# worm-privacy/proof-of-burn

Measured on AMD Instinct MI355X. Metric: proof_of_burn witnesses/sec, higher is better.
Workload: dtype u64 bit-sliced lanes + BN254 Fr (8x32-bit Montgomery)

## Files before the change

### include/pob_hip.h

```cpp
#ifndef POB_HIP_H
#define POB_HIP_H
#include <stdint.h>
#ifdef __cplusplus
extern "C" {
#endif

typedef struct pob_ctx* pob_handle;

enum { POB_CIRCUIT_PROOF_OF_BURN = 0, POB_CIRCUIT_SPEND = 1, POB_CIRCUIT_GADGET = 2 };
enum { POB_OK = 0, POB_E_ARG = -1, POB_E_HIP = -2, POB_E_NOMEM = -3, POB_E_STATE = -4, POB_E_IO = -5, POB_E_RANGE = -6 };

typedef struct {
    uint64_t n_witness;
    uint64_t n_bit, n_sm, n_fr;
    uint32_t n_fr_inputs, n_sm_inputs, n_outputs;
    uint32_t n_units, n_sponges, n_perms, n_stages, max_batch;
    uint64_t group_bytes;
    uint64_t keccak_bit_wires;
    uint64_t n_derived;
    uint64_t n_alias;
    uint32_t kchk_rounds;
    uint32_t kgc_rounds;
} pob_info_t;

int pob_open(int device, int circuit, const uint64_t* params, int nparams, uint32_t max_batch, pob_handle* out);
void pob_close(pob_handle h);
int pob_get_info(pob_handle h, pob_info_t* info);
int pob_plan_info(int circuit, const uint64_t* params, int nparams, pob_info_t* info);
const char* pob_strerror(pob_handle h);
int pob_gadget_template(const char* name, int* nparams);

int pob_upload_inputs(pob_handle h, const uint8_t* fr_inputs, const int32_t* sm_inputs, uint32_t n);
int pob_upload_inputs_async(pob_handle h, const uint8_t* fr_inputs, const int32_t* sm_inputs, uint32_t n, void* stream);
int pob_pack_json(int circuit, const uint64_t* params, int nparams, const char* json, uint64_t len, uint8_t* fr_row, int32_t* sm_row,
                  uint32_t* forced, char* err, uint32_t errcap);
int pob_pack_json_batch(int circuit, const uint64_t* params, int nparams, const char* const* json, const uint64_t* len, uint32_t n, int threads,
                        uint8_t* fr, int32_t* sm, uint32_t* forced, char* err, uint32_t errcap);
#define POB_EXC_CAP 32
#define POB_EXC_NONE 0xFFFFFFFFu
typedef struct { uint32_t k; int32_t v; } pob_sm_exc_t;
int pob_upload_inputs8(pob_handle h, const uint8_t* fr_inputs, const uint8_t* sm8, const pob_sm_exc_t* exc, uint32_t n);
int pob_upload_inputs8_async(pob_handle h, const uint8_t* fr_inputs, const uint8_t* sm8, const pob_sm_exc_t* exc, uint32_t n, void* stream);
int pob_narrow_inputs(const int32_t* sm, uint32_t n, uint32_t n_sm_inputs, uint8_t* sm8, pob_sm_exc_t* exc);
int pob_pack_json_batch8(int circuit, const uint64_t* params, int nparams, const char* const* json, const uint64_t* len, uint32_t n, int threads,
                         uint8_t* fr, uint8_t* sm8, pob_sm_exc_t* exc, uint32_t* forced, char* err, uint32_t errcap);
int pob_host_alloc(void** p, uint64_t bytes);
void pob_host_free(void* p);

int pob_generate(pob_handle h, void* stream);
int pob_constraint_check(pob_handle h, void* stream);
int pob_sync(pob_handle h);
int pob_set_partner(pob_handle h, pob_handle partner);

int pob_set_inorder(pob_handle h, int on);
int pob_set_audit(pob_handle h, uint32_t groups, uint32_t period);
int pob_audit_last(pob_handle h, uint32_t* first_group, uint32_t* n_groups, uint64_t* audited_batches, uint64_t* audited_groups);

int pob_results(pob_handle h, uint32_t* status, uint8_t* outputs, uint32_t* check_status, uint32_t* bad_wire);
int pob_results_device(pob_handle h, void** d_status, void** d_outputs);
#define POB_RECORD_BYTES 44
#define POB_NOT_EVALUATED 0xFFFFFFFEu
int pob_results_records_device(pob_handle h, void** d_records);
int pob_gather_records(pob_handle h, void* comm, void* stream, void* d_out, uint32_t n_per_rank);
int pob_results_fetch(pob_handle h);
int pob_results_wait(pob_handle h, const uint8_t** records, uint32_t* n);

int pob_emit_witness(pob_handle h, uint32_t idx, uint8_t* dst, uint64_t cap);
int pob_write_wtns(pob_handle h, uint32_t idx, const char* path);
int pob_write_wtns_reduced(pob_handle h, uint32_t idx, const uint32_t* keep, uint64_t n_keep, const char* path);
int pob_emit_begin(pob_handle h, uint32_t idx, uint64_t window_wires);
int pob_emit_begin_reduced(pob_handle h, uint32_t idx, const uint32_t* keep, uint64_t n_keep, uint64_t window_wires);
int pob_reduced_map_pin(pob_handle h, const uint32_t* keep, uint64_t n_keep);
int pob_emit_next(pob_handle h, const uint8_t** data, uint64_t* first_wire, uint64_t* n_wires);
int pob_emit_queue(pob_handle h, uint32_t next_idx);
int pob_emit_selfcheck(pob_handle h, int enable);
int pob_emit_selfcheck_alias(pob_handle h, const int32_t* alias, uint64_t n_wires);
int pob_emit_selfcheck_result(pob_handle h, uint64_t* checked, uint64_t* skipped, uint32_t* first_bad_wire);
int pob_emit_measure(pob_handle h, uint32_t first_idx, uint32_t count, uint64_t window_wires, double* seconds, uint64_t* bytes);
int pob_emit_measure_ex(pob_handle h, uint32_t first_idx, uint32_t count, uint64_t window_wires, const uint32_t* keep, uint64_t n_keep, double* seconds, uint64_t* bytes);

int pob_emit_begin_packed(pob_handle h, uint32_t idx, const uint32_t* keep, uint64_t n_keep, uint64_t window_wires);
int pob_emit_next_packed(pob_handle h, const uint8_t** data, uint64_t* bytes, uint64_t* first_wire, uint64_t* n_wires);
int pob_unpack_window(const uint8_t* packed, uint64_t packed_bytes, uint8_t* dst, uint64_t dst_cap, int threads);
int pob_write_wtns_packed(pob_handle h, uint32_t idx, const uint32_t* keep, uint64_t n_keep, const char* path);
int pob_emit_measure_packed(pob_handle h, uint32_t first_idx, uint32_t count, uint64_t window_wires, const uint32_t* keep, uint64_t n_keep, uint8_t* dst, uint64_t dst_cap, int threads,
                            double* seconds_pinned, double* seconds_expanded, uint64_t* d2h_bytes);

int pob_emit_begin_group_packed(pob_handle h, uint32_t group, uint64_t lanes, const uint32_t* keep, uint64_t n_keep, uint64_t window_wires, uint64_t* lanes_out);
int pob_emit_next_group_packed(pob_handle h, const uint8_t* data[64], uint64_t bytes[64], uint64_t* first_wire, uint64_t* n_wires);
int pob_write_wtns_group(pob_handle h, uint32_t group, uint64_t lanes, const uint32_t* keep, uint64_t n_keep, const char* const paths[64]);
int pob_emit_measure_group(pob_handle h, uint32_t first_group, uint32_t count, uint64_t lanes, uint64_t window_wires, const uint32_t* keep, uint64_t n_keep, uint8_t* dst, uint64_t dst_cap, int threads,
                           double* seconds_pinned, double* seconds_expanded, uint64_t* d2h_bytes);
int pob_emit_group_selfcheck(pob_handle h, int enable);
int pob_emit_group_selfcheck_result(pob_handle h, uint64_t* lanes, uint64_t* checked, uint64_t* skipped, uint32_t first_bad_wire[64]);

int pob_time_kernel(pob_handle h, int which, int iters, void* stream, float* avg_ms);
int pob_probe_check_kernel(pob_handle h, int enable, float* ms);

int pob_debug_xor_bits(pob_handle h, uint32_t group, uint64_t bit_index, uint64_t mask);
int pob_debug_store_fault(pob_handle h, int cls, uint32_t group, uint64_t index, uint64_t mask, uint32_t* wire);
int pob_debug_value_fault(pob_handle h, int cls, uint32_t group, uint64_t index, uint64_t mask, uint32_t* wire);
int pob_debug_stream_create(int device, const uint32_t* cu_mask, uint32_t words, void** stream);
void pob_debug_stream_destroy(int device, void* stream);
enum { POB_CLASS_BIT = 0, POB_CLASS_SM = 1, POB_CLASS_FR = 2 };
int pob_debug_poke(pob_handle h, int cls, uint32_t group, uint64_t index, uint32_t sub, uint32_t lane, uint32_t xor_mask);
// ... 18 lines not shown
```

### proof_of_burn_amd/csrc/circuits.hpp

```cpp
#pragma once
#include <string.h>
#include "gadgets.hpp"
#include "poseidon_consts.h"

#define KECCAKF_ROUND_WIRES 102656u
#define KECCAKF_WIRES (43200u + 24u * KECCAKF_ROUND_WIRES)
#define ABSORB_OWN 5888u
#define ABSORB_WIRES (ABSORB_OWN + 17u * 384u + KECCAKF_WIRES)
#define KR_STORED 76u
#define KR_BITS (KR_STORED * 64u)
#define AB_ROUNDS_W (ABSORB_OWN + 17u * 384u + 43200u)
#define AB_MID 0u
#define AB_DIRECT (25u * 1600u)
#define ABSORB_BITS (AB_DIRECT + 24u * KR_BITS)
#define ABSORB_ALIAS (ABSORB_WIRES - ABSORB_BITS)

enum UnitKind : uint32_t {
    U_POB_INPUT = 1, U_POB_RANGE, U_POB_LAYER_ASSERT, U_POB_HDR_ASSERT, U_POB_POSEIDONS, U_BAH_PRE, U_BAH_POST,
    U_KB_HEAD, U_KB_RANGE, U_KB_SELROW, U_KB_POST, U_POB_N2B, U_PC_PRE, U_PC_POST, U_POB_LASTLAYER, U_POB_LASTLAYER_RANGE,
    U_POB_LASTLEN, U_POB_LEAF, U_POB_LAYER_POST, U_SC_M, U_SC_RANGE, U_SC_SUMS, U_POB_LASTLEAF,
    U_RL_A, U_RL_SLROW, U_RL_ACC, U_RL_B, U_POW_PRE, U_POW_POST, U_POB_FINAL, U_ABS_RANGE, U_LD_HEAD, U_LD_SELR, U_LD_TAIL, U_POB_INPUT_FR, U_RL_ACC_B, U_RL_ACC_C,
    U_SP_INPUT, U_SP_HEAD,
    U_SC_MI,
    CK_POS_SEG,
// ... 14 lines not shown
#define FAM_LIGHT (FAM_BIT(F_MISC) | FAM_BIT(F_RANGE) | FAM_BIT(F_SELROW) | FAM_BIT(F_LD) | FAM_BIT(F_RL))
#define FAM_HEAVY (FAM_BIT(F_POS) | FAM_BIT(F_N2B))
#define FAM_ALL ((1u << F_COUNT) - 1)
HD constexpr uint32_t fam_of(uint32_t k) {
    return (k == U_KB_RANGE || k == U_ABS_RANGE) ? F_RANGE
         : k == U_KB_SELROW ? F_SELROW
         : (k == U_LD_HEAD || k == U_LD_SELR || k == U_LD_TAIL || k == U_LD_COPY || k == U_POB_LASTLAYER_RANGE || k == U_SC_SUMS) ? F_LD
         : (k == U_RL_A || k == U_RL_SLROW || k == U_RL_ACC_B || k == U_RL_ACC_C || k == U_RL_B || k == CK_SR_COLS || k == CK_SL_ROWS || k == CK_RL_B2 || k == CK_RL_B3 || k == CK_CAT) ? F_RL
         : (k == U_POB_LAYER_POST || k == U_SC_M || k == U_SC_RANGE) ? F_SC
         : (k == U_POB_POSEIDONS || k == U_BAH_PRE || k == U_SP_HEAD || k == CK_POS_SEG || k == U_POS_WIDE) ? F_POS
         : (k == U_GM || k == U_GM_INPUT) ? F_GM
         : (k == U_POB_INPUT_FR || k == U_POB_RANGE || k == U_POB_N2B || k == U_PC_POST || k == U_RL_ACC || k == U_POW_PRE || k == U_SP_INPUT || k == CK_N2BE) ? F_N2B
         : F_MISC;
}
HD constexpr uint32_t gen_fam_of(uint32_t k) { return k == U_PC_PRE ? (uint32_t)F_N2B : fam_of(k); }
HD constexpr bool ride_keeps_evaluation(uint32_t kind) { return fam_of(kind) == F_RL; }
#define UCASE(K) case K: if constexpr ((((MASK) >> (P::is_gen ? gen_fam_of(K) : fam_of(K))) & 1u) && !(P::ride && ride_keeps_evaluation(K)))

struct PobParams { int L, NB, HB, minNib, amountBytes, powZero; Fr maxIntended, maxActual; };
struct SpendParams { int maxAmountBytes; };

#define FP_ISEQ_S (Cur{6, 2, 0, 0, 4})
#define FP_ISEQ_F (Cur{6, 2, 0, 0, 4})
#define FP_N2B8 (Cur{9, 0, 0, 0, 9})
#define FP_ISEQ_D (Cur{6, 0, 0, 0, 6})

struct PobMain {
    FrRef commitment, burnKey, actualBalance, intendedBalance, revealAmount, burnExtraCommitment;
    SmRef numLeafAddressNibbles, layers, layerLens, numLayers, blockHeader, blockHeaderLen, byteSecurityRelax;
    FrRef proofExtraCommitment, remainingCoin, nullifier;
    SmRef addressHashNibbles, blockRoot, stateRoot, nullifierBytes, remainingCoinBytes, revealAmountBytes, burnExtraCommitmentBytes,
        extraCommitmentBytes, lastLayer, lastLayerLen;
    BitRef layerExists, substringCheckers;
    SmRef layerKeccaks, reducedLayerKeccaks;
    BitRef isLeaf, isLastLayerLeaf;
    SmRef leaf, leafLen;
};
struct SpendMain {
    FrRef commitment, burnKey, balance, withdrawnBalance, extraCommitment, coin, remainingCoin;
    SmRef coinBytes, withdrawnBalanceBytes, remainingCoinBytes, extraCommitmentBytes;
};
struct KBRefs {
    SmRef out, in, inLen, numBlocks; BitRef inBitsArray, inBits, inBlocks, outBits, outBytes;
    uint32_t padded_w, pad_o_w, pad_in_w;
    SmRef pad_nb, pad_il, pad_dv, pad_rm; BitRef pad_flt, pad_isEq, pad_isLast;
    Cur c_loop;
    Cur c_div;
    BitRef k_out, k_in; SmRef k_blocks; BitRef k_finalState, f_out, f_in; SmRef f_blocks; BitRef f_s;
    uint32_t abs_w, abs_b;
    BitRef sel_out, sel_arrays; SmRef sel_select; BitRef sel_T;
    Cur c_post;
    SmRef dst; uint32_t has_dst;
    uint32_t mb, index;
};
struct ScRefs {
    BitRef out; uint32_t mi_w; SmRef ml, si; FrRef num; uint32_t M_w; BitRef ex, isl, alw; SmRef sums; BitRef dne;
    Cur c_abs_sub, c_abs_main, c_after_abs, c_loop, c_tail;
    SmRef abs_main_in;
};
struct RlRefs {
    SmRef o, ol, in, inl; FrRef bal; SmRef key, keyLen, acc, accLen, pk, pkLen, val, valLen;
    SmRef t_o, t_ol, t_in, t_il, t_dv, t_rm, t_shf, t_on, t_tmp;
    SmRef s_o, s_in, s_cn; BitRef s_isEq; SmRef s_temp;
    Cur c_sl_iseq, c_mux, c_age, c_acc, c_concat;
};
struct LdRefs {
    BitRef isLeaf; SmRef layer, ll;
    BitRef leafPrefixIsF8; SmRef totalLength; BitRef isConsistentWithLayerLen; SmRef keyPrefix; BitRef keyPrefixIsValid, keyIsMultiByte;
    SmRef keyExtraLen, keyLen, valueWrapperPrefix; BitRef valueWrapperPrefixIsB8; SmRef valueWrapperLen, valuePrefix; BitRef valuePrefixIsF8;
    SmRef valueLen; BitRef isValueWrapperLenConsistent, isKeyValueLenEqualWithLayerLen;
    Cur c_sel[4], c_eq[4], c_mand, c_end;
    SmRef src, len_src; BitRef dst;
};
struct RaRefs {
    SmRef ea_o, ea_ol; FrRef ea_ib; SmRef pn, pnl, br, brl, nbl, sc;
    SmRef ri_o, ri_ol; FrRef ri_i; SmRef by, len, be; BitRef isb, isz; SmRef frb;
    Cur c_cb, c_sl, c_lt, c_concat, c_end;
};
struct SpongeDesc { uint32_t n, stage, src_b, abs_b, kin_w, fin_w, fs_w, abs_w, src_w; };
struct UnitDesc { uint32_t kind, stage; Cur cur; uint32_t a[8]; uint32_t cost, flags; };

#define SC_RANGE_POS 32
#define MAX_KB 72
#define MAX_SC 64
struct CircuitLayout {
    int circuit;
    struct { uint32_t tid, nfr_in, nsm_in, nout; } gm;
    uint32_t decl_order;
    PobParams pob; SpendParams spend;
    PobMain pm; SpendMain sm;
    Fr prefix[3];
    struct { SmRef nibbles; FrRef in; SmRef addressBytes, block, hash; uint32_t kb; } bah;
    struct { FrRef out; SmRef in, flat, block, hash, reduced; uint32_t kb; int N, nb; SmRef fl_o, fl_i, fit_o, fit_i; Cur c_abs; } pc;
    struct { FrRef in; SmRef mzb, keyBytes, raBytes, becBytes, eip, hin, block, keccak; BitRef sbz; uint32_t kb; } pw;
    struct { SmRef out; uint32_t arr_w, sel_w, T_w; Cur c_sel0; } ll;
    RlRefs rl;
    RaRefs ra;
    uint32_t kb_hdr, kb_layer0, nkb, nsc;
    Cur fp_n2be32, fp_n2beN;
    KBRefs kbs[MAX_KB];
    ScRefs scs[MAX_SC];
    LdRefs lds[MAX_SC + 1];
};

HD PosOff pos_off(int t) {
    PosOff k;
    if (t == 3) { k.C = POS_OFF_C_3; k.S = POS_OFF_S_3; k.M = POS_OFF_M_3; k.Pm = POS_OFF_P_3; k.rp = POS_RP_3; }
    else if (t == 4) { k.C = POS_OFF_C_4; k.S = POS_OFF_S_4; k.M = POS_OFF_M_4; k.Pm = POS_OFF_P_4; k.rp = POS_RP_4; }
    else { k.C = POS_OFF_C_5; k.S = POS_OFF_S_5; k.M = POS_OFF_M_5; k.Pm = POS_OFF_P_5; k.rp = POS_RP_5; }
    return k;
}

HD bool posw_value_fault_covers(int T, uint32_t rel) {
    const uint32_t t = (uint32_t)T, rp = (uint32_t)pos_off(T).rp, full = 8 * t, part = 4 + 2 * t;
    if (rel < 4 * t + 1) return rel >= 2 * t + 1 && rel <= 3 * t;
    rel -= 4 * t + 1;
    if (rel >= 4 * full && rel < 4 * full + rp * part) { const uint32_t q = (rel - 4 * full) % part; return q >= 4 && q < 4 + t; }
    if (rel >= 4 * full) rel -= rp * part;
    if (rel >= 7 * full) return false;
    const uint32_t q = rel % full;
    return (q >= 4 * t && q < 5 * t) || (q >= 6 * t && q < 7 * t);
}

#define NO_RANK 0xFFFFFFFFu
template <class P> HD BitRef dbits(P& p, uint32_t n) { BitRef r = {p.dvs(n), NO_RANK}; return r; }
template <class P> GD void kb_head(P& p, int mb, S inLen, KBRefs& r) {
    const uint32_t m = 136 * mb;
    r.mb = mb;
    r.out = p.sms(32); r.in = p.sms(m); r.inLen = p.sms(1); r.padded_w = p.dvs(m); r.numBlocks = p.sms(1);
    r.inBitsArray = dbits(p, 8 * m); r.inBits = dbits(p, 8 * m); r.inBlocks = p.bits(8 * m); r.outBits = dbits(p, 256); r.outBytes = dbits(p, 256);
    inLen = p.put(r.inLen, inLen);
    gAssertLessThanS(p, 16, inLen, (S)m);
    r.pad_o_w = p.dvs(m); r.pad_nb = p.sms(1); r.pad_in_w = p.dvs(m); r.pad_il = p.sms(1); r.pad_dv = p.sms(1); r.pad_rm = p.sms(1);
    r.pad_flt = p.bits(m + 1); r.pad_isEq = p.bits(m); r.pad_isLast = p.bits(m);
    inLen = p.put(r.pad_il, inLen);
    S q, rem;
    r.c_div = p.cur;
    gDivide(p, 16, inLen, (S)136, q, rem);
    q = p.put(r.pad_dv, q); p.put(r.pad_rm, rem);
    S nb = p.put(r.pad_nb, q + 1);
    gAssertLessEqThanS(p, 16, nb, (S)mb);
    p.put(r.numBlocks, nb);
    p.put(r.pad_flt, ~(B)0);
    r.c_loop = p.cur;
    p.cur = cur_add(cur_add(cur_add(p.cur, FP_ISEQ_D, 2 * m), FP_N2B8, m), Cur{16u * m, 0, 0, 0, 16u * m}, 1);
}
template <class P> HD void iseq_derived(P& p, Cur c, S a, S b) {
    p.derived(c.w + 1, a); p.derived(c.w + 2, b);
    const S x = (S)((uint32_t)b - (uint32_t)a);
    p.derived(c.w + 4, x); p.derived_inv(c.w + 5, x, true);
}
template <class P> GD void kb_range(P& p, const KBRefs& r, SmRef src, uint32_t lo, uint32_t hi, bool assert_src = false, SmRef also = SmRef{0, 0}) {
    const uint32_t m = 136 * r.mb, cnt = hi - lo, ln = p.lane_id();
    const S inLen = p.get(r.inLen), nb = p.get(r.numBlocks);
    const S last = (S)((uint32_t)nb * 136u - 1u);
    const Cur cE = r.c_loop, cL = cur_add(cE, FP_ISEQ_D, m), cN = cur_add(cL, FP_ISEQ_D, m), cF = cur_add(cN, FP_N2B8, m);
    const uint32_t flat_o_w = cF.w, flat_i_w = cF.w + 8 * m;
    bool fl = P::is_gen ? ((uint32_t)inLen >= lo) : p.bit(p.get(r.pad_flt + lo));
    uint32_t wE = 0, wL = 0, wF = 0, wPE = 0, wPL = 0;
    B wb0 = 0, wb1 = 0;
    S vs[16];
    if constexpr (P::is_count) { for (uint32_t t = 0; t < cnt; t++) p.put(r.in + (lo + t), (S)0); for (int q = 0; q < 16; q++) vs[q] = 0; }
    else {
        SmRef rr[16]; S sv[16];
#pragma unroll
        for (int q = 0; q < 16; q++) rr[q] = r.in + (lo + ((uint32_t)q < cnt ? (uint32_t)q : cnt - 1));
        const SmLoaded<16> h = sm_load(p, rr);
#pragma unroll
        for (int q = 0; q < 16; q++) sv[q] = p.get(src + (lo + ((uint32_t)q < cnt ? (uint32_t)q : cnt - 1)));
        sm_commit(p, rr, h, sv);
#pragma unroll
        for (int q = 0; q < 16; q++) vs[q] = P::is_check ? h.s[q] : sv[q];
        if (assert_src) {
#pragma unroll
            for (int q = 0; q < 16; q++) p.require_lane((uint32_t)sv[q] < 256u, FAILCODE(T_NUM2BITS, 38));
        }
        if (also.w) {
            SmRef ar[16];
#pragma unroll
            for (int q = 0; q < 16; q++) ar[q] = also + (lo + ((uint32_t)q < cnt ? (uint32_t)q : cnt - 1));
            const SmLoaded<16> ha = sm_load(p, ar);
            sm_commit(p, ar, ha, sv);
        }
    }
#pragma unroll
    for (uint32_t t = 0; t < 16; t++) if (t < cnt) {
        const uint32_t i = lo + t;
        const Cur ce = cur_add(cE, FP_ISEQ_D, i), cl = cur_add(cL, FP_ISEQ_D, i);
        const S v = vs[t];
        iseq_derived(p, ce, (S)i, inLen); iseq_derived(p, cl, (S)i, last);
        const bool e = (uint32_t)inLen == i, l = (uint32_t)last == i;
        fl = fl && !e;
        const S pv = (fl ? v : 0) + (S)e + (l ? 0x80 : 0);
        p.derived(r.pad_in_w + i, v); p.derived(r.pad_o_w + i, pv); p.derived(r.padded_w + i, pv); p.derived(cN.w + 9 * i + 8, pv);
        p.require_lane((uint32_t)pv < 256u, FAILCODE(T_NUM2BITS, 38));
        wE |= (uint32_t)e << t; wL |= (uint32_t)l << t; wF |= (uint32_t)fl << t;
        wPE |= (e ? 3u : 0u) << (2 * t); wPL |= (l ? 3u : 0u) << (2 * t);
        if (t < 8) wb0 |= (B)((uint32_t)pv & 0xffu) << (8 * t); else wb1 |= (B)((uint32_t)pv & 0xffu) << (8 * (t - 8));
    }
    const B runE = p.xpose64(wE, 0, cnt), runL = p.xpose64(wL, 0, cnt), runF = p.xpose64(wF, 0, cnt);
    const B runPairE = p.xpose64(wPE, 0, 2 * cnt), runPairL = p.xpose64(wPL, 0, 2 * cnt);
    const B bits0 = p.xpose(wb0, 64), bits1 = cnt > 8 ? p.xpose(wb1, 64) : 0;
    p.run_put(cnt, r.pad_isEq.w + lo + ln, r.pad_isEq.i + lo + ln, runE);
    p.run_put(cnt, r.pad_flt.w + lo + 1 + ln, r.pad_flt.i + lo + 1 + ln, runF);
    p.run_put(cnt, r.pad_isLast.w + lo + ln, r.pad_isLast.i + lo + ln, runL);
    {
        const uint32_t i = lo + (ln >> 1), wh = ln & 1;
        p.run_derived(2 * cnt, cE.w + 6 * i + 3 * wh, runPairE);
        p.run_derived(2 * cnt, cL.w + 6 * i + 3 * wh, runPairL);
        if constexpr (P::is_emit) { if (ln < 2 * cnt) { p.site_c(cE.w + 6 * i + 3 * wh, r.pad_isEq.w + i); p.site_c(cL.w + 6 * i + 3 * wh, r.pad_isLast.w + i); } }
    }
    for (uint32_t h2 = 0; h2 < 2 && 8 * h2 < cnt; h2++) {
        const uint32_t n = (cnt - 8 * h2 < 8 ? cnt - 8 * h2 : 8) * 8;
        const B x = h2 ? bits1 : bits0;
        const uint32_t j = 8 * (lo + 8 * h2) + ln, i = lo + 8 * h2 + (ln >> 3);
        p.run_put(n, r.inBlocks.w + j, r.inBlocks.i + j, x);
        p.run_derived(n, cN.w + 9 * i + (ln & 7), x);
        p.run_derived(n, r.inBitsArray.w + j, x);
        p.run_derived(n, flat_i_w + j, x);
        p.run_derived(n, flat_o_w + j, x);
        p.run_derived(n, r.inBits.w + j, x);
    }
}
template <class P> GD void kb_declare_keccak(P& p, KBRefs& r) {
    const uint32_t n = r.mb;
    r.k_out = dbits(p, 256); r.k_in = dbits(p, n * 1088); r.k_blocks = p.sms(1); r.k_finalState = dbits(p, 1600);
    r.f_out = dbits(p, 1600); r.f_in = dbits(p, n * 1088); r.f_blocks = p.sms(1); r.f_s = dbits(p, (n + 1) * 1600);
    r.abs_w = p.cur.w; r.abs_b = p.cur.b;
    p.skip_alias(n * ABSORB_WIRES, n * ABSORB_BITS);
    r.sel_out = dbits(p, 1600); r.sel_arrays = dbits(p, (n + 1) * 1600); r.sel_select = p.sms(1); r.sel_T = dbits(p, 1600 * (n + 1));
}
template <class P, int N1> GD void kb_selrow_n(P& p, const KBRefs& r, uint32_t row, uint32_t j0, uint32_t j1) {
    const uint32_t n1 = N1 ? (uint32_t)N1 : r.mb + 1, n = j1 - j0, ln = p.lane_id();
    const uint32_t fw = 9 * n1 + 3, fb = 1, fq = 9 * n1 + 2;
    const Cur c0 = p.cur;
    const uint32_t idx = row * 64 + j0 + ln;
    const S blocks = p.get(r.numBlocks);
    p.require(p.ballot((uint32_t)blocks < n1), FAILCODE(T_SELECTOR, 43));
    const uint32_t bw = c0.w + ln * fw, bb = c0.b + ln * fb;
    B acc = 0;
    p.run_derived(n, bw + 2 * n1 + 2, 0);
#pragma unroll
    for (uint32_t k = 0; k < n1; k++) {
        const B v = k == 0 ? (B)0 : p.run_get(n, r.abs_b + (k - 1) * ABSORB_BITS + AB_MID + 24u * 1600u + idx);
        const B e = p.ballot((uint32_t)blocks == k);
        acc |= e & v;
        if constexpr (P::is_emit) {
            p.run_derived(n, r.sel_arrays.w + k * 1600 + idx, v);
            p.run_derived(n, r.sel_T.w + idx * n1 + k, v);
            p.run_derived(n, bw + 1 + k, v);
            p.run_derived(n, bw + n1 + 2 + k, e);
            p.run_derived(n, bw + 2 * n1 + 3 + k, acc);
            const uint32_t cw = bw + 3 * n1 + 3 + 6 * k;
            p.run_derived(n, cw, e);
            p.run_derived(n, cw + 3, e);
        }
    }
    p.run_put(n, bw, bb, acc);
    p.run_derived(n, r.sel_out.w + idx, acc);
    p.run_derived(n, r.f_out.w + idx, acc);
    p.run_derived(n, r.k_finalState.w + idx, acc);
    if (row < 4) {
        const uint32_t pw = r.c_post.w;
        p.run_derived(n, r.k_out.w + idx, acc);
        p.run_derived(n, r.outBits.w + idx, acc);
        p.run_derived(n, pw + 256 + idx, acc);
        p.run_derived(n, pw + idx, acc);
        p.run_derived(n, r.outBytes.w + idx, acc);
        p.run_derived(n, pw + 512 + 9 * (idx >> 3) + 1 + (idx & 7), acc);
        for (uint32_t jj = 0; jj < n; jj += 8) {
            S by = 0;
#pragma unroll
            for (uint32_t b = 0; b < 8; b++) by |= (S)p.bit(p.run_bcast(acc, jj + b)) << b;
            const uint32_t i = (row * 64 + j0 + jj) >> 3;
            const SmRef b2n_o = {pw + 512 + 9 * i, r.c_post.s + i};
            const S o = p.put(r.out + i, p.put(b2n_o, by));
            if (r.has_dst) p.put(r.dst + i, o);
        }
    }
    derived_rows_same(p, c0.w + n1 + 1, fw, n, blocks);
    for (uint32_t k = 0; k < n1; k++) {
        const uint32_t cw = c0.w + 3 * n1 + 3 + 6 * k;
        const S x = (S)(k - (uint32_t)blocks);
        derived_rows_same(p, cw + 1, fw, n, blocks);
        derived_rows_same(p, cw + 2, fw, n, (S)k);
        derived_rows_same(p, cw + 4, fw, n, x);
        derived_rows_same(p, cw + 5, fw, n, x, true);
    }
    p.cur = cur_add(c0, Cur{fw, fb, 0, 0, fq}, n);
}
template <class P> GD void kb_selrow(P& p, const KBRefs& r, uint32_t row, uint32_t j0, uint32_t j1) { kb_selrow_n<P, 0>(p, r, row, j0, j1); }
template <class P> GD void kb_post(P& p, const KBRefs& r) {
    S nb = p.get(r.numBlocks);
    p.put(r.k_blocks, nb); p.put(r.f_blocks, nb); p.put(r.sel_select, nb);
    p.cur = cur_add(r.c_post, Cur{512 + 32 * 9, 0, 32, 0, 512 + 32 * 8}, 1);
}

#include "gadget_mains.hpp"

template <class P> GD void rl_b_prefixes(P& p, const RlRefs& R, const PobParams& prm, S kl, S& pl, S& vl) {
    const int ab = 32, bb = prm.amountBytes, maxAcc = 4 + bb + 66, maxKey = 1 + ab;
    const S al = p.get(R.accLen);
    p.put(R.val, 0xb8); p.put(R.val + 1, al);
    copy_n(p, R.val + 2, R.acc, maxAcc);
    vl = p.put(R.valLen, 2 + al);
    p.put(R.pk, 0xf8); p.put(R.pk + 1, (kl + 1) + vl); p.put(R.pk + 2, 0x80 + kl);
    copy_n(p, R.pk + 3, R.key, maxKey);
    pl = p.put(R.pkLen, 3 + kl);
}
template <class P, class MR> GD void rl_b_concat(P& p, const RlRefs& R, const MR& M, const PobParams& prm, S pl, S vl) {
// ... 537 lines not shown
        for (uint32_t k = lo; k < hi; k++) {
            Fr b1 = {{(uint32_t)p.get(src + k), 0, 0, 0, 0, 0, 0, 0}};
            acc = fr_add(fr_mul(b1, p.k256r(k)), acc);
            p.derived_fr(sc.M_w + k + 1, acc);
            p.site_m(sc.M_w + k + 1, sc.mi_w + k, k);
        }
    } break;
    UCASE(U_SC_RANGE) {
        const ScRefs& sc = L.scs[d.a[0]];
        const uint32_t lo = d.a[1], hi = d.a[2], sl = 31;
        const S mainLen = p.get(sc.ml);
        const F subNum = p.get(sc.num);
        const Fr subC = fr_from_mont(subNum);
        const SmRef src = M.layers + ((d.a[0] - 1) * LB);
        const uint32_t lastIdx = (uint32_t)(mainLen - (S)sl + 1);
        const uint32_t ln = p.lane_id(), cnt = hi - lo;
        bool allowed = P::is_gen ? (lastIdx >= lo) : p.bit(p.get(sc.alw + lo));
        uint32_t wIsl = 0, wAlw = 0, wEx = 0;
        B wC0 = 0, wC1 = 0;
        F ddL = fr_zero();
        Fr win = sc_window(p, src, lo, sl);
        for (uint32_t t = 0; t < cnt; t++) {
            const uint32_t i = lo + t;
            const S nxt = i + sl < (uint32_t)LB ? p.get(src + (i + sl)) : 0;
            const bool e = fr_eq(win, subC), last = i == lastIdx;
            allowed = allowed && !last;
            wIsl |= (uint32_t)last << t; wAlw |= (uint32_t)allowed << t; wEx |= (uint32_t)e << t;
            const B four = (B)((last ? 3u : 0u) | (e ? 12u : 0u)) << (4 * (t & 15));
            if (t < 16) wC0 |= four; else wC1 |= four;
            if constexpr (P::is_emit) {
                const Cur c = cur_add(cur_add(sc.c_loop, FP_ISEQ_S, i), FP_ISEQ_F, i);
                iseq_derived(p, c, (S)i, (S)lastIdx);
                const F t1 = fr_mul(subNum, p.k256(i)), t2 = fr_mul(fr_to_mont(win), p.k256(i)), dd = fr_sub(t2, t1);
                p.derived_fr(c.w + 7, t1); p.derived_fr(c.w + 8, t2); p.derived_fr(c.w + 10, dd);
                if constexpr (P::is_group) p.derived_fr_inv(c.w + 11, dd, true);
                else { const F ds = p.bcast_sel(dd); if (ln == t) ddL = ds; }
            }
            sc_window_step(win, sl, (uint32_t)nxt);
        }
        if constexpr (P::is_emit) if constexpr (!P::is_group) {
            const F inv = fr_is_zero(ddL) ? fr_zero() : fr_inv(ddL);
            if (ln < cnt) p.w32(cur_add(cur_add(sc.c_loop, FP_ISEQ_S, lo + ln), FP_ISEQ_F, lo + ln).w + 11, fr_from_mont(inv), (fr_is_zero(ddL) ? 3 : 2) | 4);
        }
        const B runIsl = p.xpose64(wIsl, 0, cnt), runAlw = p.xpose64(wAlw, 0, cnt), runEx = p.xpose64(wEx, 0, cnt);
        const B runC0 = p.xpose(wC0, 64), runC1 = cnt > 16 ? p.xpose(wC1, 64) : 0;
        p.run_put(cnt, sc.isl.w + lo + ln, sc.isl.i + lo + ln, runIsl);
        p.run_put(cnt, sc.alw.w + lo + 1 + ln, sc.alw.i + lo + 1 + ln, runAlw);
        p.run_put(cnt, sc.ex.w + lo + ln, sc.ex.i + lo + ln, runEx);
        for (uint32_t h2 = 0; h2 < 2 && 16 * h2 < cnt; h2++) {
            const uint32_t n = (cnt - 16 * h2 < 16 ? cnt - 16 * h2 : 16) * 4, i = lo + 16 * h2 + (ln >> 2), wh = ln & 3;
            p.run_put(n, sc.c_loop.w + 12 * i + 3 * wh, sc.c_loop.b + 4 * i + wh, h2 ? runC1 : runC0);
        }
    } break;
    UCASE(CK_POS_SEG) {
        if constexpr (!(P::is_check || P::is_count)) { (void)d; }
        else if (d.a[0] == 3) gPoseidonSegStored<P, 3>(p, pos_off(3), d.cur, d.a[1]);
        else if (d.a[0] == 4) gPoseidonSegStored<P, 4>(p, pos_off(4), d.cur, d.a[1]);
        else gPoseidonSegStored<P, 5>(p, pos_off(5), d.cur, d.a[1]);
    } break;
    UCASE(CK_SL_ROWS) {
        if constexpr (P::is_check || P::is_count) gShiftLeftRows(p, (int)d.a[0], d.cur, Cur{d.a[3], d.a[4], d.a[5], d.cur.f, d.cur.q}, d.a[1], d.a[2]);
    } break;
    UCASE(CK_N2BE) {
        if constexpr (P::is_check || P::is_count || P::is_gen) {
            const FrRef src = P::is_gen ? FrRef{d.a[6], d.a[7]} : FrRef{d.a[1], d.a[2]}; const SmRef also = {d.a[3], d.a[4]};
            gNum2BigEndianBytesFv(p, (int)d.a[0], p.get(src), also, d.a[5] != 0);
        }
    } break;
    default: break;
    }
}
template <class P> GD void unit_run_all(P& p, const UnitDesc& d, CircuitLayout& L) { unit_run<P, FAM_ALL>(p, d, L); }

#include <stdlib.h>
#include <algorithm>
#include <stdexcept>
#include <string>
#include <vector>
struct Plan {
    CircuitLayout L;
    std::vector<UnitDesc> units;
    std::vector<SpongeDesc> sponges;
    Cur total;
    uint32_t nfr_in, nsm_in, max_stage;
    enum { TRACK_STRIDE = 32, MAX_TRACKS = 7 };
    uint32_t ntracks, track_fork[MAX_TRACKS], track_join[MAX_TRACKS];
    uint32_t wide_tracks = 0;
    CountP p;

    static bool same(Cur a, Cur b) { return a.w == b.w && a.b == b.b && a.s == b.s && a.f == b.f && a.q == b.q; }
    void expect_cursor(const char* what, Cur got, Cur want) {
        if (!same(got, want)) throw std::runtime_error(std::string("layout planner: split units disagree with the monolithic template: ") + what);
    }
    void record(uint32_t kind, uint32_t stage, Cur cur, uint32_t a0 = 0, uint32_t a1 = 0, uint32_t a2 = 0, uint32_t a3 = 0, uint32_t a4 = 0, uint32_t a5 = 0, uint32_t a6 = 0, uint32_t a7 = 0) {
        UnitDesc d; d.kind = kind; d.stage = stage; d.cur = cur; d.cost = 0; d.a[0] = a0; d.a[1] = a1; d.a[2] = a2; d.a[3] = a3; d.a[4] = a4; d.a[5] = a5; d.a[6] = a6; d.a[7] = a7;
        d.flags = (kind == CK_POS_SEG || kind == CK_SR_COLS || kind == CK_SL_ROWS || kind == CK_RL_B2 || kind == CK_RL_B3 || kind == CK_CAT) ? UNIT_CHECK
                : kind == CK_N2BE ? (UNIT_GEN | UNIT_CHECK)
                : kind == U_POS_WIDE ? UNIT_GEN
                : kind == U_SC_M ? UNIT_EMIT
                : kind == U_POB_POSEIDONS ? (UNIT_CHECK | UNIT_EMIT)
                : kind == U_GM_INPUT ? (UNIT_GEN | UNIT_CHECK)
                : kind == U_POB_INPUT ? UNIT_EMIT
                : (UNIT_GEN | UNIT_CHECK | UNIT_EMIT);
        units.push_back(d);
        if (stage > max_stage) max_stage = stage;
    }
    void unit(uint32_t kind, uint32_t stage, uint32_t a0 = 0, uint32_t a1 = 0, uint32_t a2 = 0, uint32_t a3 = 0, uint32_t a4 = 0) {
        record(kind, stage, p.cur, a0, a1, a2, a3, a4);
        const UnitDesc d = units.back();
        p.nnotes = 0;
        unit_run_all(p, d, L);
        take_notes(p, stage);
    }
    void take_notes(CountP& q, uint32_t stage) {
        if (q.notes_overflow) throw std::runtime_error("layout planner: a composite unit has more split sub-blocks than PLAN_MAX_NOTES");
        for (uint32_t k = 0; k < q.nnotes; k++) {
            const PlanNote& nt = q.notes[k];
            if (nt.what == NOTE_POSEIDON) {
                const uint32_t ns = pos_nseg(pos_off((int)nt.n).rp);
                for (uint32_t seg = 1; seg < ns; seg++) record(CK_POS_SEG, stage, nt.cur, nt.n, seg);
                if (stage % TRACK_STRIDE == 0) throw std::runtime_error("layout planner: a Poseidon composite needs a stage before it");
                record(U_POS_WIDE, stage - 1, nt.cur, nt.n, nt.a[0], nt.a[1], nt.a[2], nt.a[3], nt.a[4], nt.a[5]);
            } else if (nt.what == NOTE_N2BE) record(CK_N2BE, stage, nt.cur, nt.n, nt.a[0], nt.a[1], nt.a[2], nt.a[3], nt.a[4], nt.a[5], nt.a[6]);
            else if (nt.what == NOTE_SHIFTLEFT) { for (uint32_t i = 0; i < nt.n; i += 2) record(CK_SL_ROWS, stage, nt.cur, nt.n, i, std::min(i + 2, nt.n), nt.a[0], nt.a[1], nt.a[2]); }
        }
        q.nnotes = 0;
    }
    void record_composite(uint32_t kind, uint32_t stage, Cur cur) {
        record(kind, stage, cur);
        const UnitDesc d = units.back();
        CountP q; q.nnotes = 0;
        unit_run_all(q, d, L);
        take_notes(q, stage);
    }
    void cat_units(uint32_t stage, Cur c0, int La, int Lb) {
        Cur cc[3]; concat_cursors(p, c0, La, Lb, cc);
        for (uint32_t part = 0; part < 4; part++) record(CK_CAT, stage, cc[part < 3 ? part : 2], part, (uint32_t)La, (uint32_t)Lb, c0.w, c0.s);
    }
    void abs_units(uint32_t stage, uint32_t N, SmRef src, uint32_t chunk = 32, bool emit_only = false) {
        CountP chk; chk.cur = p.cur; gAssertByteString(chk, (int)N, src);
        const uint32_t own_w = p.dvs(N);
        const Cur c0 = p.cur;
        for (uint32_t lo = 0; lo < N; lo += chunk) { record(U_ABS_RANGE, stage, c0, own_w, 0, src.w, src.i, lo, std::min(lo + chunk, N)); if (emit_only) units.back().flags = UNIT_EMIT; }
        p.cur = cur_add(c0, FP_ABITS8, N);
        expect_cursor("AssertByteString", p.cur, chk.cur);
    }
    void keccak_tail(uint32_t kb, uint32_t range_stage, SmRef dst, bool has_dst) {
        KBRefs& r = L.kbs[kb];
        r.index = kb;
        kb_declare_keccak(p, r);
        SpongeDesc s; s.n = r.mb; s.stage = range_stage + 1; s.src_b = r.inBlocks.i; s.src_w = r.inBlocks.w;
        s.kin_w = r.k_in.w; s.fin_w = r.f_in.w; s.fs_w = r.f_s.w; s.abs_b = r.abs_b; s.abs_w = r.abs_w;
        sponges.push_back(s);
        r.dst = dst; r.has_dst = has_dst ? 1 : 0;
        {
            CountP q; q.cur = p.cur; r.c_post = Cur{0, 0, 0, 0}; r.has_dst = 0; kb_selrow(q, r, 24, 0, 1);
            const Cur fp1 = {q.cur.w - p.cur.w, q.cur.b - p.cur.b, q.cur.s - p.cur.s, 0, q.cur.q - p.cur.q};
            r.c_post = cur_add(p.cur, fp1, 1600); r.has_dst = has_dst ? 1 : 0;
        }
        const uint32_t split = r.mb >= 8 ? 4 : r.mb >= 3 ? 2 : 1;
        for (uint32_t row = 0; row < 25; row++) {
            const Cur c0 = p.cur;
            CountP q; q.cur = c0; kb_selrow(q, r, row, 0, 64);
            const Cur fp = {(q.cur.w - c0.w) / 64, (q.cur.b - c0.b) / 64, (q.cur.s - c0.s) / 64, 0, (q.cur.q - c0.q) / 64};
            for (uint32_t k = 0; k < split; k++) record(U_KB_SELROW, range_stage + 2, cur_add(c0, fp, k * (64 / split)), kb, row, k * (64 / split), (k + 1) * (64 / split));
            p.cur = q.cur;
        }
        if (!same(p.cur, r.c_post)) throw std::runtime_error("layout planner: selector footprint");
        unit(U_KB_POST, range_stage + 2, kb);
        if (range_stage + 1 > max_stage) max_stage = range_stage + 1;
    }
    void keccak_bytes(uint32_t kb, int mb, uint32_t stage, SmRef src, SmRef len, SmRef dst, uint32_t len_input = 0, bool has_dst = true, bool assert_src = false, SmRef also = SmRef{0, 0}) {
        L.kbs[kb].mb = mb;
        const Cur start = p.cur;
        unit(U_KB_HEAD, stage, kb, len.w, len.i, len_input);
        const uint32_t m = 136 * mb;
        for (uint32_t lo = 0; lo < m; lo += 16) record(U_KB_RANGE, stage + 1, start, kb, src.w, src.i, lo, std::min(lo + 16, m), assert_src ? 1u : 0u, also.w, also.i);
        keccak_tail(kb, stage + 1, dst, has_dst);
    }
    void kb_ranges(uint32_t kb, uint32_t stage, SmRef src) {
        const uint32_t m = 136 * L.kbs[kb].mb;
        for (uint32_t lo = 0; lo < m; lo += 16) record(U_KB_RANGE, stage, p.cur, kb, src.w, src.i, lo, std::min(lo + 16, m));
    }
    void leaf_detector(uint32_t inst, uint32_t stage, SmRef src, SmRef len, BitRef dst, bool copy_units = true) {
        const uint32_t N = 136 * L.pob.NB;
        CountP chk; chk.cur = p.cur; gLeafDetector(chk, (int)N, src, 0);
        L.lds[inst].src = src; L.lds[inst].len_src = len; L.lds[inst].dst = dst;
        unit(U_LD_HEAD, stage, inst);
        expect_cursor("LeafDetector", p.cur, chk.cur);
        if (copy_units) for (uint32_t lo = 0; lo < N; lo += 32) record(U_LD_COPY, stage, p.cur, inst, lo, std::min(lo + 32, N));
        for (uint32_t k = 0; k < 4; k++) for (uint32_t lo = 0; lo < N; lo += 34) record(U_LD_SELR, stage + 1, p.cur, inst, k, lo, std::min(lo + 34, N));
        record(U_LD_TAIL, stage + 2, p.cur, inst);
    }
    void burn_address_hash(uint32_t pre_stage) {
        L.bah.nibbles = p.sms(64); L.bah.in = p.frs(3); L.bah.addressBytes = p.sms(20); L.bah.block = p.sms(136); L.bah.hash = p.sms(32);
        L.bah.kb = L.nkb++;
        if (L.circuit == 2) { L.pm.burnKey = L.bah.in; L.pm.revealAmount = L.bah.in + 1; L.pm.burnExtraCommitment = L.bah.in + 2; L.pm.addressHashNibbles = L.bah.nibbles; }
        unit(U_BAH_PRE, pre_stage);
        kb_ranges(L.bah.kb, pre_stage + 1, L.bah.block);
        keccak_tail(L.bah.kb, pre_stage + 1, L.bah.hash, true);
        unit(U_BAH_POST, pre_stage + 4);
    }
    void proof_of_work_checker(uint32_t pre_stage) {
        L.pw.in = p.frs(3); L.pw.mzb = p.sms(1); L.pw.keyBytes = p.sms(32); L.pw.raBytes = p.sms(32); L.pw.becBytes = p.sms(32); L.pw.eip = p.sms(8);
        L.pw.hin = p.sms(104); L.pw.block = p.sms(136); L.pw.keccak = p.sms(32); L.pw.sbz = p.bits(32);
        L.pw.kb = L.nkb++;
        if (L.circuit == 2) { L.pm.burnKey = L.pw.in; L.pm.revealAmount = L.pw.in + 1; L.pm.burnExtraCommitment = L.pw.in + 2; L.pm.byteSecurityRelax = L.pw.mzb; }
        unit(U_POW_PRE, pre_stage);
        kb_ranges(L.pw.kb, pre_stage + 1, L.pw.block);
        keccak_tail(L.pw.kb, pre_stage + 1, L.pw.keccak, true);
        unit(U_POW_POST, pre_stage + 4);
    }
    void public_commitment(int N, uint32_t pre_stage) {
        L.pc.N = N; L.pc.nb = N * 32 / 136 + ((N * 32) % 136 != 0);
        L.pc.out = p.frs(1); L.pc.in = p.sms(32 * N); L.pc.flat = p.sms(32 * N); L.pc.block = p.sms(136 * L.pc.nb); L.pc.hash = p.sms(32); L.pc.reduced = p.sms(31);
        L.pc.kb = L.nkb++; L.kbs[L.pc.kb].mb = L.pc.nb;
        {
            CountP chk; chk.cur = p.cur; chk.decl_order = p.decl_order;
            for (int j = 0; j < N; j++) gAssertByteString(chk, 32, L.pc.in + 32 * j);
            gFlattenS(chk, 32 * N, L.pc.in); gFitS(chk, 32 * N, 136 * L.pc.nb, L.pc.flat);
            unit(U_PC_PRE, pre_stage);
            for (int j = 0; j <= N; j++) record(U_PC_COPY, pre_stage, p.cur, (uint32_t)j);
            KBRefs r2 = L.kbs[L.pc.kb]; kb_head(chk, L.pc.nb, (S)(32 * N), r2);
            expect_cursor("PublicCommitment", p.cur, chk.cur);
        }
        kb_ranges(L.pc.kb, pre_stage + 1, L.pc.block);
        keccak_tail(L.pc.kb, pre_stage + 1, L.pc.hash, true);
        unit(U_PC_POST, pre_stage + 4);
    }

    void estimate_costs() {
        for (UnitDesc& d : units) {
            if (d.kind == U_POS_WIDE) { d.cost = 8 * pos_wires((int)d.a[0], pos_off((int)d.a[0]).rp); continue; }
            CountP q; const UnitDesc dd = d; unit_run_all(q, dd, L); d.cost = q.nput * (unit_is_heavy(d.kind) ? 4 : 1);
        }
    }
    void plan_pob(const PobParams& prm) {
        memset(&L, 0, sizeof L);
        L.circuit = 0; L.pob = prm; L.nkb = 0; max_stage = 0; L.decl_order = p.decl_order;
        L.fp_n2be32 = n2be_footprint(32); L.fp_n2beN = n2be_footprint(prm.amountBytes);
        const uint32_t TB = TRACK_STRIDE, TR = 2 * TRACK_STRIDE, TC = 3 * TRACK_STRIDE, TN = 4 * TRACK_STRIDE;
        ntracks = 6; track_fork[1] = 0; track_join[1] = 5; track_fork[2] = TB + 6; track_join[2] = 10; track_fork[3] = 0; track_join[3] = TR + 2;
        track_fork[4] = TB + 1; track_join[4] = 4;
        const uint32_t TP = 5 * TRACK_STRIDE;
        track_fork[5] = 0; track_join[5] = 5; wide_tracks = 1u << 5;
        const uint32_t TQ = 6 * TRACK_STRIDE;
        ntracks = 7; track_fork[6] = 4; track_join[6] = 10;
        PobMain& M = L.pm;
        const int Ln = prm.L, LB = 136 * prm.NB, HBy = 136 * prm.HB;
        p.cur = Cur{1, 0, 0, 0};
        M.commitment = p.frs(1);
        M.burnKey = p.frs(1); M.actualBalance = p.frs(1); M.intendedBalance = p.frs(1); M.revealAmount = p.frs(1); M.burnExtraCommitment = p.frs(1);
        M.numLeafAddressNibbles = p.sms(1); M.layers = p.sms(Ln * LB); M.layerLens = p.sms(Ln); M.numLayers = p.sms(1);
        M.blockHeader = p.sms(HBy); M.blockHeaderLen = p.sms(1); M.byteSecurityRelax = p.sms(1); M.proofExtraCommitment = p.frs(1);
        M.remainingCoin = p.frs(1); M.nullifier = p.frs(1); M.addressHashNibbles = p.sms(64); M.blockRoot = p.sms(32); M.stateRoot = p.sms(32);
        M.nullifierBytes = p.sms(32); M.remainingCoinBytes = p.sms(32); M.revealAmountBytes = p.sms(32); M.burnExtraCommitmentBytes = p.sms(32);
        M.extraCommitmentBytes = p.sms(32); M.lastLayer = p.sms(LB); M.lastLayerLen = p.sms(1); M.layerExists = p.bits(Ln);
        M.substringCheckers = p.bits(Ln - 1); M.layerKeccaks = p.sms(32 * Ln); M.reducedLayerKeccaks = p.sms(31 * Ln); M.isLeaf = p.bits(Ln);
        M.isLastLayerLeaf = p.bits(1); M.leaf = p.sms(139); M.leafLen = p.sms(1);
        nfr_in = 6; nsm_in = 1 + Ln * LB + Ln + 1 + HBy + 2;

        unit(U_POB_INPUT_FR, 0);
        for (uint32_t k = 0; k < nsm_in; k += 256) unit(U_POB_INPUT, 0, k, std::min(k + 256, nsm_in));
        for (int k = 0; k < 5; k++) unit(U_POB_RANGE, TB + 1, k);
        for (int i = 0; i < Ln; i++) { unit(U_POB_LAYER_ASSERT, TP + 1, i); abs_units(TP + 1, LB, M.layers + i * LB, 32, true); }
        unit(U_POB_HDR_ASSERT, TP + 1); abs_units(TP + 1, HBy, M.blockHeader, 32, true);
        unit(U_POB_POSEIDONS, TB + 2, 0);
        unit(U_POB_POSEIDONS, TB + 2, 1);
        burn_address_hash(TB + 2);
        L.kb_hdr = L.nkb++;
        keccak_bytes(L.kb_hdr, prm.HB, 0, M.blockHeader, M.blockHeaderLen, M.blockRoot, 0, true, true);
        for (int j = 0; j < 5; j++) unit(U_POB_N2B, TN + 1, j);
        public_commitment(6, TQ + 1);
        {
            CountP chk; chk.cur = p.cur; gSelectorArray1D(chk, Ln, LB, M.layers, 0);
            L.ll.out = p.sms(LB); L.ll.arr_w = p.dvs(Ln * LB); L.ll.sel_w = p.dvs(1); L.ll.T_w = p.dvs(LB * Ln);
            unit(U_POB_LASTLAYER, TP + 1);
            L.ll.c_sel0 = p.cur;
            const Cur fp = sel_fp((uint32_t)Ln);
            for (uint32_t j = 0; j < (uint32_t)LB; j += 4) record(U_POB_LASTLAYER_RANGE, TP + 1, p.cur, j, std::min<uint32_t>(j + 4, LB));
            p.cur = cur_add(p.cur, fp, LB);
            expect_cursor("SelectorArray1D", p.cur, chk.cur);
        }
        unit(U_POB_LASTLEN, TP + 1);
        L.kb_layer0 = L.nkb; L.nkb += Ln;
        L.nsc = Ln;
        for (int i = 0; i < Ln; i++) {
            leaf_detector(i, TP + 1, M.layers + i * LB, M.layerLens + i, M.isLeaf + i, false);
            keccak_bytes(L.kb_layer0 + i, prm.NB, 0, M.layers + i * LB, M.layerLens + i, M.layerKeccaks + 32 * i, 0, true, true, L.lds[i].layer);
            const Cur start = p.cur;
            unit(U_POB_LAYER_POST, 5, i);
            if (i > 0) {
                const ScRefs sc = L.scs[i];
                CountP chk; chk.cur = start; { gFitS(chk, 32, 31, M.layerKeccaks); gSubstringCheck(chk, LB, 31, M.layers, 0, M.reducedLayerKeccaks); }
                expect_cursor("SubstringCheck", p.cur, chk.cur);
                const SmRef src = M.layers + (i - 1) * LB;
                for (uint32_t lo = 0; lo < (uint32_t)LB; lo += 32) {
                    record(U_ABS_RANGE, TP + 1, sc.c_abs_main, sc.abs_main_in.w, sc.abs_main_in.i, src.w, src.i, lo, std::min<uint32_t>(lo + 32, LB));
                    units.back().flags = UNIT_EMIT;
                }
                for (uint32_t lo = 0; lo < (uint32_t)LB; lo += 32) record(U_SC_M, TP + 1, start, i, lo, std::min<uint32_t>(lo + 32, LB));
                const uint32_t kk = LB - 31 + 1;
                record(U_SC_MI, TP + 1, start, i);
                for (uint32_t lo = 0; lo < kk; lo += SC_RANGE_POS) record(U_SC_RANGE, 6, sc.c_loop, i, lo, std::min<uint32_t>(lo + SC_RANGE_POS, kk));
                const uint32_t sums_step = 64;
                for (uint32_t lo = 0; lo < kk; lo += sums_step) record(U_SC_SUMS, 7, sc.c_tail, i, lo, std::min<uint32_t>(lo + sums_step, kk));
            }
        }
        leaf_detector(Ln, TP + 2, M.lastLayer, M.lastLayerLen, M.isLastLayerLeaf);
        {
            const Cur start = p.cur;
            CountP chk; chk.cur = start; { S ll; gRlpMptLeaf(chk, 32, prm.amountBytes, M.addressHashNibbles, 0, fr_zero(), ll); }
            unit(U_RL_A, TR + 1);
            RlRefs& R = L.rl;
            for (uint32_t i = 0; i < 64; i += 4) record(U_RL_SLROW, TR + 1, R.c_sl_iseq, i, i + 4);
            CountP q; q.cur = R.c_mux;
            for (int i = 0; i < 63; i++) gMux1S(q, 0, 0, 0);
            gNibbles2Bytes(q, 33, R.t_on);
            R.c_age = q.cur;
            gAssertGreaterEqThanS(q, 16, 0, 2);
            R.c_acc = q.cur;
            { S al; gRlpEmptyAccount(q, prm.amountBytes, fr_zero(), al); }
            R.c_concat = q.cur;
            { S cl; gConcat(q, 2 + 1 + 33, 2 + 4 + prm.amountBytes + 66, R.pk, 0, R.val, 0, cl); }
            expect_cursor("RlpMerklePatriciaTrieLeaf", q.cur, chk.cur);
            {
                const Cur keep = p.cur;
                p.cur = R.c_acc;
                CountP qa; qa.cur = R.c_acc; { S al; gRlpEmptyAccount(qa, prm.amountBytes, fr_zero(), al); }
                unit(U_RL_ACC, TC + 1);
                expect_cursor("RlpEmptyAccount", p.cur, qa.cur);
                p.cur = keep;
                record_composite(U_RL_ACC_B, TC + 2, L.ra.c_cb);
                record_composite(U_RL_ACC_C, TC + 3, L.ra.c_concat);
                cat_units(TC + 3, L.ra.c_concat, 4 + prm.amountBytes, 66);
            }
            record_composite(U_RL_B, TR + 2, R.c_mux);
            record(CK_RL_B2, TR + 2, R.c_mux); record(CK_RL_B3, TR + 2, R.c_concat);
            cat_units(TR + 2, R.c_concat, 2 + 1 + 33, 2 + 4 + prm.amountBytes + 66);
            p.cur = chk.cur;
        }
        proof_of_work_checker(TB + 2);
        unit(U_POB_FINAL, 10);
        total = p.cur;
        estimate_costs();
    }
    const char* plan_gadget(uint32_t tid, const int* prm, int nprm) {
        memset(&L, 0, sizeof L);
        L.circuit = 2; L.nkb = 0; max_stage = 0; ntracks = 1; L.decl_order = p.decl_order;
        L.pob = PobParams{1, 1, 1, 0, 31, 0, fr_zero(), fr_zero()};
        L.fp_n2be32 = n2be_footprint(32); L.fp_n2beN = n2be_footprint(31);
        L.gm.tid = tid;
        const GmName* nm = nullptr;
        for (const GmName& g : GM_NAMES) if (g.id == tid) nm = &g;
        if (!nm) return "unknown gadget template";
        if (nprm != nm->nparams) return "wrong number of template parameters";
        const int a = nprm > 0 ? prm[0] : 0, b = nprm > 1 ? prm[1] : 0, c = nprm > 2 ? prm[2] : 0, d = nprm > 3 ? prm[3] : 0;
        auto in = [](long v, long lo, long hi) { return v >= lo && v <= hi; };
        bool ok = true;
        switch (tid) {
        case GM_CONCAT_FIXED4: ok = in(a, 0, 4096) && in(b, 0, 4096) && in(c, 0, 4096) && in(d, 0, 4096) && a + b + c + d >= 1; break;
        case GM_PUBLIC_COMMITMENT: ok = in(a, 1, 16); break;
        case GM_POSEIDON: ok = in(a, 2, 4); break;
        case GM_DIVIDE: case GM_ASSERT_LESS_EQ_THAN: case GM_ASSERT_LESS_THAN: case GM_ASSERT_GREATER_EQ_THAN: case GM_IS_IN_RANGE: ok = in(a, 1, 30); break;
        case GM_SUBSTRING_CHECK: ok = in(b, 1, 31) && in(a, b, 4096); break;
        case GM_SHIFT_LEFT: ok = in(a, 1, 256); break;
        case GM_SHIFT_RIGHT: ok = in(a, 1, 4096) && in(b, 0, 4096) && in((long)a * (b + 1), 1, 1 << 20); break;
        case GM_MASK: case GM_SELECTOR: case GM_BYTES2NIBBLES: case GM_NIBBLES2BYTES: case GM_ASSERT_BYTE_STRING: case GM_FILTER: case GM_REVERSE:
        case GM_COUNT_BYTES: ok = in(a, 1, 4096); break;
        case GM_CONCAT: ok = in(a, 1, 2048) && in(b, 1, 2048); break;
        case GM_SELECTOR_ARRAY_1D: ok = in(a, 1, 4096) && in(b, 1, 4096) && in((long)a * b, 1, 1 << 16); break;
        case GM_SELECTOR_ARRAY_2D: ok = in(a, 1, 4096) && in(b, 1, 4096) && in(c, 1, 4096) && in((long)a * b * c, 1, 1 << 16); break;
        case GM_BIG_ENDIAN_BYTES2NUM: case GM_LITTLE_ENDIAN_BYTES2NUM: case GM_RLP_INTEGER: case GM_RLP_EMPTY_ACCOUNT: ok = in(a, 1, 31); break;
        case GM_NUM2BIG_ENDIAN_BYTES: case GM_NUM2LITTLE_ENDIAN_BYTES: ok = in(a, 1, 32); break;
        case GM_NUM2BITS_SAFE: ok = in(a, 1, 256); break;
        case GM_PAD: ok = in(a, 1, 4096) && in(b, 1, 4096) && in((long)a * b, 1, 4096); break;
        case GM_KECCAK_BYTES: ok = in(a, 1, 32); break;
        case GM_ASSERT_BITS: ok = in(a, 1, 253); break;
        case GM_FIT: ok = in(a, 1, 4096) && in(b, 1, 4096); break;
        case GM_FLATTEN: case GM_RESHAPE: ok = in(a, 1, 4096) && in(b, 1, 4096) && in((long)a * b, 1, 1 << 16); break;
        case GM_TRUNCATED_ADDRESS_HASH: ok = in(a, 1, 32); break;
        case GM_LEAF_DETECTOR: ok = in(a, 3, 4096); break;
        case GM_RLP_MPT_LEAF: ok = in(a, 1, 32) && in(b, 1, 31); break;
        default: break;
        }
        if (!ok) return "template parameters outside the range the gadget-main path supports";
        p.cur = Cur{1, 0, 0, 0, 0};
        nfr_in = nsm_in = 0;
        if (tid == GM_KECCAK_BYTES) {
            const uint32_t m = 136u * (uint32_t)a;
            const SmRef own_in = {1 + 32, 32}, own_len = own_in + m;
            L.nkb = 1;
            keccak_bytes(0, a, 1, own_in, own_len, SmRef{0, 0}, m + 1, false);
            const KBRefs& r = L.kbs[0];
            if (r.in.w != own_in.w || r.in.i != own_in.i || r.inLen.w != own_len.w || r.inLen.i != own_len.i) throw std::runtime_error("layout planner: KeccakBytes main inputs");
            record(U_GM_INPUT, 1, Cur{1, 0, 0, 0, 0}, 0, 0, 0, own_in.w, own_in.i, m + 1);
            L.gm.nfr_in = 0; L.gm.nsm_in = m + 1; L.gm.nout = 32;
        } else if (tid == GM_PUBLIC_COMMITMENT) {
            public_commitment(a, 2);
            record(U_GM_INPUT, 1, Cur{1, 0, 0, 0, 0}, 0, 0, 0, L.pc.in.w, L.pc.in.i, 32u * (uint32_t)a);
            L.gm.nfr_in = 0; L.gm.nsm_in = 32u * (uint32_t)a; L.gm.nout = 1;
        } else if (tid == GM_BURN_ADDRESS_HASH) {
            burn_address_hash(2);
            record(U_GM_INPUT, 0, Cur{1, 0, 0, 0, 0}, L.bah.in.w, L.bah.in.i, 3, 0, 0, 0);
            L.gm.nfr_in = 3; L.gm.nsm_in = 0; L.gm.nout = 64;
        } else if (tid == GM_PROOF_OF_WORK_CHECKER) {
            proof_of_work_checker(2);
            record(U_GM_INPUT, 0, Cur{1, 0, 0, 0, 0}, L.pw.in.w, L.pw.in.i, 3, L.pw.mzb.w, L.pw.mzb.i, 1);
            L.gm.nfr_in = 3; L.gm.nsm_in = 1; L.gm.nout = 0;
        } else unit(U_GM, 1, tid, (uint32_t)a, (uint32_t)b, (uint32_t)c, (uint32_t)d);
        nfr_in = L.gm.nfr_in; nsm_in = L.gm.nsm_in;
        total = p.cur;
        estimate_costs();
        return nullptr;
    }
    void plan_spend(const SpendParams& prm) {
        memset(&L, 0, sizeof L);
        L.circuit = 1; L.spend = prm; L.nkb = 0; max_stage = 0; ntracks = 1; L.decl_order = p.decl_order;
        L.fp_n2be32 = n2be_footprint(32); L.fp_n2beN = n2be_footprint(prm.maxAmountBytes);
        L.pob = PobParams{1, 1, 1, 0, prm.maxAmountBytes, 0, fr_zero(), fr_zero()};
        SpendMain& M = L.sm;
        p.cur = Cur{1, 0, 0, 0};
        M.commitment = p.frs(1); M.burnKey = p.frs(1); M.balance = p.frs(1); M.withdrawnBalance = p.frs(1); M.extraCommitment = p.frs(1);
        M.coin = p.frs(1); M.remainingCoin = p.frs(1); M.coinBytes = p.sms(32); M.withdrawnBalanceBytes = p.sms(32); M.remainingCoinBytes = p.sms(32);
        M.extraCommitmentBytes = p.sms(32);
        nfr_in = 4; nsm_in = 0;
        unit(U_SP_INPUT, 0);
        unit(U_SP_HEAD, 2);
        public_commitment(4, 3);
        total = p.cur;
        estimate_costs();
    }
};
```

### proof_of_burn_amd/csrc/pob_emit.hip

```cpp
#include "pob_ctx.hpp"

static void group_free_device(EmitGroup& Gr) {
    for (void* p : {(void*)Gr.d_win, (void*)Gr.d_pk[0], (void*)Gr.d_pk[1], (void*)Gr.d_hdr[0], (void*)Gr.d_hdr[1], (void*)Gr.d_blk, (void*)Gr.d_tot}) if (p) (void)hipFree(p);
    for (uint8_t* p : {Gr.h_hdr[0], Gr.h_hdr[1]}) if (p) (void)hipHostFree(p);
    Gr.d_win = Gr.d_pk[0] = Gr.d_pk[1] = Gr.d_hdr[0] = Gr.d_hdr[1] = Gr.h_hdr[0] = Gr.h_hdr[1] = nullptr; Gr.d_blk = Gr.d_tot = nullptr; Gr.alloc_wires = 0;
}
void pob_detail::emit_release(pob_ctx* h) {
    EmitState& E = h->em;
    void* ptrs[] = {E.d_win[0], E.d_win[1], E.d_win[2], E.d_order, E.d_probe, E.d_rbits, E.d_rpre, E.d_sc_res, E.d_sc_zr, E.d_sc_mr, E.d_gsc_res, E.d_pk[0], E.d_pk[1], E.d_pk[2], E.d_pk_blk, E.d_pk_tot};
    for (void* p : ptrs) if (p) hipFree(p);
    E.sc.free(); E.gsc.free();
    {
        EmitGroup& Gr = E.grp;
        group_free_device(Gr);
        for (int k = 0; k < 3; k++) if (Gr.h_pin[k]) hipHostFree(Gr.h_pin[k]);
        for (hipEvent_t e : {Gr.ev_made[0], Gr.ev_made[1], Gr.ev_hdr[0], Gr.ev_hdr[1], Gr.ev_free[0], Gr.ev_free[1], Gr.ev_copied[0], Gr.ev_copied[1], Gr.ev_copied[2]}) if (e) hipEventDestroy(e);
    }
    for (int k = 0; k < EmitState::NSLOT; k++) {
        if (E.h_pin[k]) hipHostFree(E.h_pin[k]);
        for (hipEvent_t e : {E.ev_made[k], E.ev_copied[k], E.ev_free[k]}) if (e) hipEventDestroy(e);
    }
}
void pob_detail::emit_release_streams(pob_ctx* h) {
    if (h->em.s_copy) hipStreamDestroy(h->em.s_copy);
    if (h->em.s_val) hipStreamDestroy(h->em.s_val);
}

#define EMIT_ALL_UNITS (~0ull)
static void emit_units(pob_ctx* h, GArgs A, uint64_t k, void (*launch)(const GArgs&, uint32_t, uint32_t, hipStream_t)) {
    const EmitState& E = h->em;
    hipStream_t st = own_stream(h);
    if (E.probe_win == E.win_wires && E.probe_map == E.map_id && k < E.wsegs.size()) {
        A.order = E.d_order;
        for (const EmitState::WSeg& sg : E.wsegs[k]) { A.first = sg.first; launch(A, sg.cls, sg.count, st); }
    } else {
        for (const pob_ctx::Seg& sg : h->emit_segs) { A.first = sg.first; launch(A, sg.lds, sg.count, st); }
    }
}
template <class F> static void for_each_run_piece(const EmitState& E, uint64_t w0, uint64_t wn, F f) {
    const uint64_t wire_lo = E.red ? E.keep[w0] : w0, wire_hi = E.red ? (uint64_t)E.keep[w0 + wn - 1] + 1 : w0 + wn;
    for (const EmitState::Run& r : E.runs) {
        uint64_t lo = std::max<uint64_t>(r.w, wire_lo), hi = std::min<uint64_t>((uint64_t)r.w + r.n, wire_hi);
        if (lo >= hi) continue;
        if (E.red) {
            const auto a = std::lower_bound(E.keep.begin() + w0, E.keep.begin() + w0 + wn, (uint32_t)lo), b = std::lower_bound(a, E.keep.begin() + w0 + wn, (uint32_t)hi);
            if (a == b) continue;
            lo = *a; hi = (uint64_t)*(b - 1) + 1;
        }
        f(r, lo, hi);
    }
}
hipError_t SiteTables::upload(const std::vector<std::array<uint32_t, 3>>& ms, const std::vector<std::array<uint32_t, 2>>& cs) {
    m_next.resize(ms.size()); c_hi.resize(cs.size());
    for (size_t i = 0; i < ms.size(); i++) m_next[i] = ms[i][0];
    for (size_t i = 0; i < cs.size(); i++) c_hi[i] = cs[i][0];
    hipError_t e = hipMalloc(&d_z, std::max<size_t>(z.size(), 1) * 4);
    if (e == hipSuccess) e = hipMalloc(&d_m, std::max<size_t>(ms.size(), 1) * 12);
    if (e == hipSuccess) e = hipMalloc(&d_c, std::max<size_t>(cs.size(), 1) * 8);
    if (e == hipSuccess && !z.empty()) e = hipMemcpy(d_z, z.data(), z.size() * 4, hipMemcpyHostToDevice);
    if (e == hipSuccess && !ms.empty()) e = hipMemcpy(d_m, ms.data(), ms.size() * 12, hipMemcpyHostToDevice);
    if (e == hipSuccess && !cs.empty()) e = hipMemcpy(d_c, cs.data(), cs.size() * 8, hipMemcpyHostToDevice);
    return e;
}
void SiteTables::free() {
    for (uint32_t** q : {&d_z, &d_m, &d_c}) { if (*q) (void)hipFree(*q); *q = nullptr; }
}
SiteTables::Window SiteTables::window(uint64_t wire_lo, uint64_t wire_hi) const {
    const auto zless = [](uint32_t s, uint32_t v) { return (s & 0x7FFFFFFFu) < v; };
    const auto za = std::lower_bound(z.begin(), z.end(), (uint32_t)wire_lo, zless), zb = std::lower_bound(za, z.end(), (uint32_t)wire_hi, zless);
    const auto ma = std::lower_bound(m_next.begin(), m_next.end(), (uint32_t)wire_lo), mb = std::lower_bound(ma, m_next.end(), (uint32_t)wire_hi);
    const auto ca = std::lower_bound(c_hi.begin(), c_hi.end(), (uint32_t)wire_lo), cb = std::lower_bound(ca, c_hi.end(), (uint32_t)wire_hi);
    return {{d_z + (za - z.begin()), (uint32_t)(zb - za)}, {d_m + 3 * (ma - m_next.begin()), (uint32_t)(mb - ma)}, {d_c + 2 * (ca - c_hi.begin()), (uint32_t)(cb - ca)}};
}

extern "C" {

static int emit_make_window(pob_ctx* h, uint32_t idx, uint64_t k, int slot) {
    EmitState& E = h->em;
    const uint64_t w0 = k * E.win_wires, wn = std::min(E.win_wires, E.total - w0);
    hipStream_t st = own_stream(h);
    HIPC(hipStreamWaitEvent(st, E.ev_free[slot], 0));
    hipLaunchKernelGGL(k_fill_ee, dim3(2048), dim3(256), 0, st, (uint4*)E.d_win[slot], wn * 2);
    if (w0 == 0) { const uint32_t one[8] = {1, 0, 0, 0, 0, 0, 0, 0}; HIPC(hipMemcpyAsync(E.d_win[slot], one, 32, hipMemcpyHostToDevice, st)); }
    GArgs A = gargs(h);
    A.emit_out = E.d_win[slot]; A.emit_sel = idx % 64; A.emit_group = idx / 64; A.emit_w0 = (uint32_t)w0; A.emit_wn = (uint32_t)wn;
    if (E.red) { A.emit_rbits = E.d_rbits; A.emit_rpre = E.d_rpre; }
    emit_units(h, A, k, launch_g_emit);
    const u64* Gp = (const u64*)h->d_bits + (uint64_t)(idx / 64) * h->plan.total.b;
    for_each_run_piece(E, w0, wn, [&](const EmitState::Run& r, uint64_t lo, uint64_t hi) {
        if (!E.red) {
            if (r.absorb) launch_k_emit_absorb(Gp, E.d_win[slot] + (lo - w0) * 32, AbsorbRef{r.b, r.prev, r.src}, r.o + (uint32_t)(lo - r.w), (uint32_t)(hi - lo), idx % 64, h->d_ktab, st);
            else launch_k_emit_bits(Gp, E.d_win[slot] + (lo - w0) * 32, 0, (uint32_t)(r.b + (lo - r.w)), (uint32_t)(hi - lo), idx % 64, st);
        } else {
            if (r.absorb) launch_k_emit_absorb_red(Gp, E.d_win[slot], (uint32_t)lo, AbsorbRef{r.b, r.prev, r.src}, r.o + (uint32_t)(lo - r.w), (uint32_t)(hi - lo), idx % 64, h->d_ktab, E.d_rbits, E.d_rpre, (uint32_t)w0, (uint32_t)wn, st);
            else launch_k_emit_bits_red(Gp, E.d_win[slot], (uint32_t)lo, (uint32_t)(r.b + (lo - r.w)), (uint32_t)(hi - lo), idx % 64, E.d_rbits, E.d_rpre, (uint32_t)w0, (uint32_t)wn, st);
        }
    });
    if (E.sc_on && E.red) {
        const ScWin W{E.d_win[slot], (uint32_t)w0, (uint32_t)wn, E.d_rbits, E.d_rpre};
        uint32_t* res = E.d_sc_res; const uint32_t* zr = E.d_sc_zr; const uint32_t* mr = E.d_sc_mr; const uint32_t* pw = h->d_pow256; const uint32_t nz = E.sc_red_nz, nm = E.sc_red_nm;
        if (nz) hipLaunchKernelGGL(k_selfcheck_zr, dim3((nz + 63) / 64), dim3(64), 0, st, W, zr, nz, res);
        if (nm) hipLaunchKernelGGL(k_selfcheck_mr, dim3((nm + 63) / 64), dim3(64), 0, st, W, mr, nm, pw, res);
    }
    if (E.sc_on && !E.red) {
        const ScWin W{E.d_win[slot], (uint32_t)w0, (uint32_t)wn, nullptr, nullptr};
        uint32_t* res = E.d_sc_res;
        const SiteTables::Window S = E.sc.window(w0, w0 + wn);
        const uint32_t nz = S.z.n, nm = S.m.n, ncs = S.c.n;
        const uint32_t *zs = S.z.p, *msites = S.m.p, *csites = S.c.p, *pw = h->d_pow256;
        if (nz) hipLaunchKernelGGL(k_selfcheck_z, dim3((nz + 63) / 64), dim3(64), 0, st, W, zs, nz, res);
        if (nm) hipLaunchKernelGGL(k_selfcheck_m, dim3((nm + 63) / 64), dim3(64), 0, st, W, msites, nm, pw, res);
        if (ncs) hipLaunchKernelGGL(k_selfcheck_c, dim3((ncs + 63) / 64), dim3(64), 0, st, W, csites, ncs, res);
        E.sc_checked += S.total();
    }
    HIPC(hipGetLastError());
    if (E.packed) {
        launch_pack_window(E.d_win[slot], w0, (uint32_t)wn, E.d_pk[slot], E.d_pk_blk, E.d_pk_tot, st);
        HIPC(hipGetLastError());
    }
    HIPC(hipEventRecord(E.ev_made[slot], st));
    HIPC(hipStreamWaitEvent(E.s_copy, E.ev_made[slot], 0));
    if (E.packed) { HIPC(hipMemcpyAsync(E.h_pin[slot], E.d_pk[slot], pack_fixed_bytes(wn), hipMemcpyDeviceToHost, E.s_copy)); E.pk_d2h += pack_fixed_bytes(wn); }
    else HIPC(hipMemcpyAsync(E.h_pin[slot], E.d_win[slot], wn * 32, hipMemcpyDeviceToHost, E.s_copy));
    HIPC(hipEventRecord(E.ev_copied[slot], E.s_copy));
    HIPC(hipEventRecord(E.ev_free[slot], E.s_copy));
    return POB_OK;
}

static uint64_t fnv64(const void* p, size_t n) {
    const uint8_t* q = (const uint8_t*)p; uint64_t hsh = 1469598103934665603ull;
    size_t i = 0;
    for (; i + 8 <= n; i += 8) { uint64_t v; memcpy(&v, q + i, 8); hsh = (hsh ^ v) * 1099511628211ull; }
    for (; i < n; i++) hsh = (hsh ^ q[i]) * 1099511628211ull;
    return hsh ? hsh : 1;
}

static int emit_statuses(pob_ctx* h) {
    EmitState& E = h->em;
    if (E.status_gen == h->gen_count && E.status_host.size() == h->n) return POB_OK;
    HIPC(hipEventSynchronize(h->ev_gen_done));
    E.status_host.resize(h->n);
    HIPC(hipMemcpyAsync(E.status_host.data(), h->d_status, (size_t)h->n * 4, hipMemcpyDeviceToHost, own_stream(h)));
    HIPC(hipStreamSynchronize(own_stream(h)));
    E.status_gen = h->gen_count;
    return POB_OK;
}

static int emit_prepare(pob_ctx* h, uint64_t total, uint64_t default_window, uint64_t* window_wires, uint64_t* nwin) {
    HIPC(hipEventSynchronize(h->ev_gen_done));
    if (h->evaluated) HIPC(hipEventSynchronize(h->ev_check_done));
    { int rc = emit_statuses(h); if (rc) return rc; }
    if (*window_wires == 0) *window_wires = default_window;
    *window_wires = std::min<uint64_t>(*window_wires, total);
    *nwin = (total + *window_wires - 1) / *window_wires;
    return POB_OK;
}

static int emit_streams_and_runs(pob_ctx* h) {
    EmitState& E = h->em;
    const int NS = EmitState::NSLOT;
    if (E.s_copy) HIPC(hipStreamSynchronize(E.s_copy));
    if (!E.s_copy) {
        HIPC(hipStreamCreateWithPriority(&E.s_copy, hipStreamNonBlocking, 0));
        for (int k = 0; k < NS; k++) {
            HIPC(hipEventCreateWithFlags(&E.ev_made[k], hipEventDisableTiming)); HIPC(hipEventCreateWithFlags(&E.ev_copied[k], hipEventDisableTiming));
            HIPC(hipEventCreateWithFlags(&E.ev_free[k], hipEventDisableTiming));
        }
        for (const SpongeDesc& sp : h->plan.sponges) {
            E.runs.push_back({sp.kin_w, sp.src_b, sp.n * 1088, 0, 0, 0, 0}); E.runs.push_back({sp.fin_w, sp.src_b, sp.n * 1088, 0, 0, 0, 0});
            E.runs.push_back({sp.fs_w, sp.abs_b, 1600, 1, 1600, NO_RANK, sp.src_b});
            for (uint32_t b = 0; b < sp.n; b++) {
// ... 227 lines not shown
        std::vector<unsigned long long> bits(nwords, 0); std::vector<uint32_t> pre(nwords, 0);
        for (uint64_t i = 0; i < n_keep; i++) {
            if (i && keep[i] <= keep[i - 1]) { h->err = "reduced map: wire indices must be strictly increasing"; return POB_E_ARG; }
            if (keep[i] >= W) { h->err = "reduced map: every index must be < nWitness"; return POB_E_ARG; }
            bits[keep[i] >> 6] |= 1ull << (keep[i] & 63);
        }
        uint32_t acc = 0;
        for (uint64_t i = 0; i < nwords; i++) { pre[i] = acc; acc += (uint32_t)__builtin_popcountll(bits[i]); }
        if (E.s_copy) HIPC(hipStreamSynchronize(E.s_copy));
        HIPC(hipStreamSynchronize(own_stream(h)));
        if (E.d_rbits) { HIPC(hipFree(E.d_rbits)); E.d_rbits = nullptr; }
        if (E.d_rpre) { HIPC(hipFree(E.d_rpre)); E.d_rpre = nullptr; }
        HIPC(hipMalloc(&E.d_rbits, nwords * 8)); HIPC(hipMalloc(&E.d_rpre, nwords * 4));
        HIPC(hipMemcpy(E.d_rbits, bits.data(), nwords * 8, hipMemcpyHostToDevice));
        HIPC(hipMemcpy(E.d_rpre, pre.data(), nwords * 4, hipMemcpyHostToDevice));
        E.keep.assign(keep, keep + n_keep);
        E.queued_idx = -1; E.pre_made = false;
    }
    E.red = true; E.map_id = id; E.total = n_keep;
    return POB_OK;
}

int pob_reduced_map_pin(pob_handle h, const uint32_t* keep, uint64_t n_keep) {
    if (!h) return POB_E_ARG;
    EmitState& E = h->em;
    if (!keep || n_keep == 0) { E.pin_ptr = nullptr; E.pin_n = 0; E.pin_id = 0; return POB_OK; }
    E.pin_ptr = keep; E.pin_n = n_keep; E.pin_id = fnv64(keep, n_keep * 4) ^ (n_keep << 1);
    return POB_OK;
}

static bool packed_counts_ok(const uint8_t* hdr, uint64_t wn, pob_ctx* h, uint32_t cnt[2]) {
    memcpy(cnt, hdr + 20, 8);
    if ((uint64_t)cnt[0] + cnt[1] > wn) { h->err = "internal: packed window counts more values than wires"; return false; }
    return true;
}
static int emit_next(pob_handle h, bool packed, const uint8_t** data, uint64_t* bytes, uint64_t* first_wire, uint64_t* n_wires) {
    if (!h || !data || !first_wire || !n_wires) return POB_E_ARG;
    EmitState& E = h->em;
    if (!E.active) { h->err = "pob_emit_next without pob_emit_begin"; return POB_E_STATE; }
    if (E.grp.on) { h->err = "pob_emit_next / pob_emit_next_packed: the emission was begun with pob_emit_begin_group_packed"; return POB_E_STATE; }
    if (E.packed != packed) { h->err = packed ? "pob_emit_next_packed: the emission was not begun with pob_emit_begin_packed" : "pob_emit_next: the emission was begun with pob_emit_begin_packed"; return POB_E_STATE; }
    if (E.next_take == E.nwin) { E.active = false; *data = nullptr; *first_wire = E.total; *n_wires = 0; return POB_OK; }
    HIPC(hipSetDevice(h->device));
    const int NS = EmitState::NSLOT;
    while (E.next_make < E.nwin && E.next_make <= E.next_take + 2) {
        int rc = emit_make_window(h, E.idx, E.next_make, (int)((E.first_slot + E.next_make) % NS)); if (rc) return rc;
        E.next_make++;
    }
    if (E.next_make == E.nwin && E.nwin - E.next_take <= 2 && E.queued_idx >= 0 && !E.pre_made) {
        int rc = emit_make_window(h, (uint32_t)E.queued_idx, 0, (int)((E.first_slot + E.nwin) % NS)); if (rc) return rc;
        E.pre_made = true; E.pre_made_gen = h->gen_count; E.pre_made_packed = E.packed;
    }
    const uint64_t k = E.next_take++;
    const int slot = (int)((E.first_slot + k) % NS);
    HIPC(hipEventSynchronize(E.ev_copied[slot]));
    *data = E.h_pin[slot]; *first_wire = k * E.win_wires; *n_wires = std::min(E.win_wires, E.total - k * E.win_wires);
    if (packed) {
        uint32_t cnt[2];
        if (!packed_counts_ok(E.h_pin[slot], *n_wires, h, cnt)) return POB_E_STATE;
        const uint64_t fixed = pack_fixed_bytes(*n_wires), vb = pack_value_bytes(cnt[0], cnt[1]);
        if (vb) {
            HIPC(hipMemcpyAsync(E.h_pin[slot] + fixed, E.d_pk[slot] + fixed, vb, hipMemcpyDeviceToHost, E.s_val));
            HIPC(hipStreamSynchronize(E.s_val));
            E.pk_d2h += vb;
        }
        if (bytes) *bytes = fixed + vb;
    }
    return POB_OK;
}
int pob_emit_next(pob_handle h, const uint8_t** data, uint64_t* first_wire, uint64_t* n_wires) { return emit_next(h, false, data, nullptr, first_wire, n_wires); }
int pob_emit_next_packed(pob_handle h, const uint8_t** data, uint64_t* bytes, uint64_t* first_wire, uint64_t* n_wires) {
    if (!bytes) return POB_E_ARG;
    return emit_next(h, true, data, bytes, first_wire, n_wires);
}

#define GROUP_DEFAULT_WINDOW (4ull << 20)
static int group_make_window(pob_ctx* h, uint64_t k) {
    EmitState& E = h->em; EmitGroup& Gr = E.grp;
    const int ps = (int)(k % 2);
    const uint64_t w0 = k * E.win_wires, wn = std::min(E.win_wires, E.total - w0);
    const uint32_t nblk = (uint32_t)((wn + 63) / 64);
    hipStream_t st = own_stream(h);
    HIPC(hipStreamWaitEvent(st, Gr.ev_free[ps], 0));
    const u64* Gp = (const u64*)h->d_bits + (uint64_t)Gr.group * h->plan.total.b;
    const GroupWin GW{Gr.d_win, Gr.plane, Gr.lanes, (uint32_t)w0, (uint32_t)wn, E.red ? E.d_rbits : nullptr, E.red ? E.d_rpre : nullptr};
    struct Piece { const EmitState::Run* r; uint64_t lo, hi; };
    std::vector<Piece> canon;
    std::vector<std::pair<uint32_t, uint32_t>> ranges;
    uint32_t covered = 0;
    for_each_run_piece(E, w0, wn, [&](const EmitState::Run& r, uint64_t lo, uint64_t hi) {
        if (E.red) { canon.push_back({&r, lo, hi}); return; }
        const uint64_t bA = (lo - w0 + 63) / 64, bB = (hi - w0) / 64;
        if (bB > bA) {
            const uint64_t wa = w0 + 64 * bA, wb = w0 + 64 * bB;
            if ((uint32_t)bA > covered) ranges.push_back({covered, (uint32_t)bA});
            covered = (uint32_t)bB;
            launch_k_emit_group_direct(Gp, Gr.d_pk[ps], Gr.pk_stride, Gr.lanes, (uint32_t)bA, (uint32_t)(bB - bA), AbsorbRef{r.b, r.prev, r.src},
                                       (r.absorb ? r.o : r.b) + (uint32_t)(wa - r.w), r.absorb ? h->d_ktab : nullptr, st);
            if (lo < wa) canon.push_back({&r, lo, wa});
            if (wb < hi) canon.push_back({&r, wb, hi});
        } else canon.push_back({&r, lo, hi});
    });
    if (covered < nblk) ranges.push_back({covered, nblk});
    const PackGroup PG{Gr.d_win, Gr.plane, Gr.d_pk[ps], Gr.pk_stride, Gr.lanes, Gr.d_blk, Gr.d_tot, Gr.d_hdr[ps]};
    launch_group_fill(PG, (uint32_t)wn, w0 == 0, ranges, st);
    GArgs A = gargs(h);
    A.emit_out = Gr.d_win; A.emit_plane = Gr.plane; A.emit_lanes = Gr.lanes; A.emit_sel = 0; A.emit_group = Gr.group; A.emit_w0 = (uint32_t)w0; A.emit_wn = (uint32_t)wn;
    if (E.red) { A.emit_rbits = E.d_rbits; A.emit_rpre = E.d_rpre; }
    emit_units(h, A, k, launch_g_emit_group);
    for (const Piece& c : canon) {
        const EmitState::Run& r = *c.r;
        launch_k_emit_group_canon(Gp, GW, (uint32_t)c.lo, AbsorbRef{r.b, r.prev, r.src}, (r.absorb ? r.o : r.b) + (uint32_t)(c.lo - r.w), (uint32_t)(c.hi - c.lo), r.absorb ? h->d_ktab : nullptr, st);
    }
    for (const EmitState::GXor& x : E.xor_now) {
        if (!((Gr.lanes >> x.lane) & 1)) continue;
        uint64_t pos = x.wire;
        if (E.red) { const auto it = std::lower_bound(E.keep.begin(), E.keep.end(), x.wire); if (it == E.keep.end() || *it != x.wire) continue; pos = (uint64_t)(it - E.keep.begin()); }
        if (pos < w0 || pos >= w0 + wn) continue;
        launch_group_xor_byte(Gr.d_win + (uint64_t)x.lane * Gr.plane + (pos - w0) * 32 + x.byte, x.mask, st);
    }
    if (Gr.checked) {
        const ScGroup SG{Gr.d_win, Gr.plane, Gr.lanes, (uint32_t)w0, (uint32_t)wn, E.red ? E.d_rbits : nullptr, E.red ? E.d_rpre : nullptr, E.d_gsc_res, E.d_gsc_res + 64};
        if (E.red) {
            launch_selfcheck_group_zr(SG, E.d_sc_zr, E.sc_red_nz, st);
            launch_selfcheck_group_mr(SG, E.d_sc_mr, E.sc_red_nm, h->d_pow256, st);
        } else {
            const SiteTables::Window S = E.gsc.window(w0, w0 + wn);
            launch_selfcheck_group_z(SG, S.z.p, S.z.n, st);
            launch_selfcheck_group_m(SG, S.m.p, S.m.n, h->d_pow256, st);
            launch_selfcheck_group_c(SG, S.c.p, S.c.n, st);
            E.gsc_launched += S.total();
        }
    }
    launch_pack_group(PG, w0, (uint32_t)wn, ranges, st);
    HIPC(hipGetLastError());
    HIPC(hipEventRecord(Gr.ev_made[ps], st));
    HIPC(hipStreamWaitEvent(E.s_copy, Gr.ev_made[ps], 0));
    HIPC(hipMemcpyAsync(Gr.h_hdr[ps], Gr.d_hdr[ps], (size_t)Gr.nsel * 32, hipMemcpyDeviceToHost, E.s_copy));
    HIPC(hipEventRecord(Gr.ev_hdr[ps], E.s_copy));
    return POB_OK;
}

static int group_copy_window(pob_ctx* h, uint64_t k) {
    EmitState& E = h->em; EmitGroup& Gr = E.grp;
    const int ps = (int)(k % 2), hs = (int)(k % 3);
    const uint64_t wn = std::min(E.win_wires, E.total - k * E.win_wires), fixed = pack_fixed_bytes(wn);
    HIPC(hipEventSynchronize(Gr.ev_hdr[ps]));
    uint64_t total = 0; uint32_t r = 0;
    for (uint32_t l = 0; l < 64; l++) {
        Gr.off[hs][l] = Gr.len[hs][l] = 0;
        if (!((Gr.lanes >> l) & 1)) continue;
        uint32_t cnt[2];
        if (!packed_counts_ok(Gr.h_hdr[ps] + 32 * (size_t)r++, wn, h, cnt)) return POB_E_STATE;
        Gr.off[hs][l] = total; Gr.len[hs][l] = fixed + pack_value_bytes(cnt[0], cnt[1]); total += Gr.len[hs][l];
    }
    if (Gr.pin_cap[hs] < total) {
        if (Gr.h_pin[hs]) { HIPC(hipHostFree(Gr.h_pin[hs])); Gr.h_pin[hs] = nullptr; Gr.pin_cap[hs] = 0; }
        const uint64_t cap = total + total / 8 + 4096;
        if (hipHostMalloc((void**)&Gr.h_pin[hs], cap, hipHostMallocDefault) != hipSuccess) { Gr.h_pin[hs] = nullptr; (void)hipGetLastError(); h->err = "group emission: out of pinned host memory"; E.active = false; return POB_E_NOMEM; }
        Gr.pin_cap[hs] = cap;
    }
    r = 0;
    for (uint32_t l = 0; l < 64; l++) {
        if (!Gr.len[hs][l]) continue;
        uint8_t* dst = Gr.h_pin[hs] + Gr.off[hs][l];
        memcpy(dst, Gr.h_hdr[ps] + 32 * (size_t)r++, 32);
        HIPC(hipMemcpyAsync(dst + 32, Gr.d_pk[ps] + (uint64_t)l * Gr.pk_stride + 32, Gr.len[hs][l] - 32, hipMemcpyDeviceToHost, E.s_copy));
// ... 387 lines not shown
```

### proof_of_burn_amd/csrc/pob_host.hip

```cpp
#include "pob_ctx.hpp"


__global__ void k_init_invlut(uint32_t* lut) {
    int t = blockIdx.x * blockDim.x + threadIdx.x;
    if (t > 8192) return;
    Fr c = fr_from_mont(fr_inv(fr_from_i64((int64_t)t - 4096)));
    for (int j = 0; j < 8; j++) lut[t * 8 + j] = c.l[j];
}
__global__ void k_collect(const uint32_t* fr, uint64_t fr_stride, uint32_t out_idx, uint32_t* status_raw, uint32_t* status, uint8_t* outputs, uint32_t* records,
                          uint32_t* host_records, uint32_t* chk, uint32_t* bad, uint32_t n) {
    uint32_t w = blockIdx.x * blockDim.x + threadIdx.x;
    if (w >= n) return;
    const uint32_t g = w / 64, lane = w % 64;
    Fr m = fr_zero();
    if (out_idx != 0xFFFFFFFFu) for (int k = 0; k < 8; k++) m.l[k] = fr[(uint64_t)g * fr_stride + (uint64_t)out_idx * 512 + k * 64 + lane];
    Fr c = fr_from_mont(m);
    uint32_t s, cs = POB_NOT_EVALUATED, bw = POB_NOT_EVALUATED;
    if (!chk) {
        s = status_raw[w]; status_raw[w] = 0xFFFFFFFFu;
        s = s == 0xFFFFFFFFu ? 0 : s;
        status[w] = s;
        for (int k = 0; k < 8; k++) ((uint32_t*)(outputs + (uint64_t)w * 32))[k] = c.l[k];
    } else {
        s = status[w];
// ... 190 lines not shown
            for (int x = 0; x < 5; x++) a[y + x] = b[y + x] ^ (~b[y + (x + 1) % 5] & b[y + (x + 2) % 5]);
        a[0] ^= RC[r];
    }
    if ((a[0] & mask) == 0) atomicMin(found, (unsigned long long)off);
}


hipStream_t pob_detail::own_stream(pob_ctx* h) {
    if (!h->stream) {
        int lo = 0, hi = 0;
        hipSetDevice(h->device);
        if (hipDeviceGetStreamPriorityRange(&lo, &hi) != hipSuccess) hi = 0;
        if (hipStreamCreateWithPriority(&h->stream, hipStreamNonBlocking, hi) != hipSuccess) h->stream = nullptr;
    }
    return h->stream;
}

struct StreamPool { int device = 0, refs = 0; hipStream_t stream2 = nullptr, stream_k = nullptr, track1 = nullptr, track2 = nullptr, chk1 = nullptr, chk2 = nullptr, s_in = nullptr; };
static std::mutex g_pool_mu;
static std::vector<StreamPool*> g_pools;

#define POB_PIPELINE_HW_QUEUES 12
static int hw_queues_env() { const char* e = getenv("GPU_MAX_HW_QUEUES"); return e ? atoi(e) : 4; }
__attribute__((constructor)) static void pob_default_hw_queues() { setenv("GPU_MAX_HW_QUEUES", "16", 0); }


#define N_GEN_CLASSES 6
#define CLS_ALL 6
static uint32_t unit_class(uint32_t kind, bool gen = false) { return fam_of(kind) == F_GM ? 5 : kind == U_POS_WIDE ? 4 : fam_of(kind) == F_SC ? 3 : (gen ? unit_gen_is_heavy(kind) : unit_is_heavy(kind)) ? 1 : 0; }
static void launch_g_gen(const GArgs& A, uint32_t cls, uint32_t nunits, uint32_t ngroups, hipStream_t st, bool ride = false, bool fault = false) {
    if (cls == 5) launch_g_gen_gm(A, nunits, ngroups, st);
    else if (cls == 4) launch_pos_wide(A, nunits, ngroups, st, ride, fault);
    else if (cls == CLS_ALL && ride && fault) launch_g_gen_all_ride_fault(A, nunits, ngroups, st);
    else if (cls == CLS_ALL && ride) launch_g_gen_all_ride(A, nunits, ngroups, st);
    else if (cls == 3) launch_g_gen_sc(A, nunits, ngroups, st);
    else if (cls == 1) launch_g_gen_n2b(A, nunits, ngroups, st);
    else if (cls == CLS_ALL) launch_g_gen_all(A, nunits, ngroups, st);
    else launch_g_gen_light(A, nunits, ngroups, st);
}
static void launch_g_check(const GArgs& A, uint32_t fam, uint32_t nunits, uint32_t ngroups, hipStream_t st) {
    switch (fam) {
    case F_MISC: launch_g_check_misc(A, nunits, ngroups, st); break;
    case F_RANGE: launch_g_check_range(A, nunits, ngroups, st); break;
    case F_SELROW: launch_g_check_selrow(A, nunits, ngroups, st); break;
    case F_LD: launch_g_check_ld(A, nunits, ngroups, st); break;
    case F_RL: launch_g_check_rl(A, nunits, ngroups, st); break;
    case F_SC: launch_g_check_sc(A, nunits, ngroups, st); break;
    case F_POS: launch_g_check_pos(A, nunits, ngroups, st); break;
    case F_GM: launch_g_check_gm(A, nunits, ngroups, st); break;
    default: launch_g_check_n2b(A, nunits, ngroups, st); break;
    }
}
void pob_detail::launch_g_emit_group(const GArgs& A, uint32_t cls, uint32_t nunits, hipStream_t st) {
    if (cls == 3) launch_g_emit_group_sc(A, nunits, 1, st); else if (cls) launch_g_emit_group_heavy(A, nunits, 1, st); else launch_g_emit_group_light(A, nunits, 1, st);
}
void pob_detail::launch_g_emit(const GArgs& A, uint32_t cls, uint32_t nunits, hipStream_t st) {
    if (cls == 5) launch_g_emit_gm(A, nunits, 1, st); else if (cls == 3) launch_g_emit_sc(A, nunits, 1, st); else if (cls) launch_g_emit_heavy(A, nunits, 1, st); else launch_g_emit_light(A, nunits, 1, st);
}

static void launch_inputs(pob_ctx* h, int mode, uint32_t G, hipStream_t st, uint32_t group0) {
    if (h->circuit != POB_CIRCUIT_PROOF_OF_BURN || !h->plan.nsm_in) return;
    const SmRef r0 = h->plan.L.pm.numLeafAddressNibbles;
    const uint32_t fk = (mode == 2 && h->fault_armed && !h->fault_g && h->fault_cls == POB_CLASS_SM) ? (uint32_t)h->fault_word - r0.i : 0xFFFFFFFFu;
    if (h->in_bytes[h->in_cur]) {
        const dim3 grid8((h->plan.nsm_in + IN8_K - 1) / IN8_K, G);
        const size_t lds = 64 * (IN8_K + 1) * 4;
        auto go = [&](auto kern) { hipLaunchKernelGGL(kern, grid8, dim3(256), lds, st, h->d_in_sm8[h->in_cur], h->d_in_exc[h->in_cur], h->plan.nsm_in, h->n, h->d_sm, (uint64_t)h->plan.total.s * 64, r0.i, r0.w, h->d_bad, fk, h->fault_group, h->fault_mask, mode == 1 ? group0 : 0u); };
        if (mode == 1) go(k_inputs8<1>); else if (mode == 2) go(k_inputs8<2>); else go(k_inputs8<0>);
        return;
    }
    const dim3 grid((h->plan.nsm_in + 63) / 64, G);
    auto go = [&](auto kern) { hipLaunchKernelGGL(kern, grid, dim3(64), 64 * 65 * 4, st, h->d_in_sm[h->in_cur], h->plan.nsm_in, h->d_sm, (uint64_t)h->plan.total.s * 64, r0.i, r0.w, h->d_bad, fk, h->fault_group, h->fault_mask, mode == 1 ? group0 : 0u); };
    if (mode == 1) go(k_inputs<1>); else if (mode == 2) go(k_inputs<2>); else go(k_inputs<0>);
}
static Fr limbs_to_mont(const uint64_t* l) {
    Fr c; for (int i = 0; i < 4; i++) { c.l[2 * i] = (uint32_t)l[i]; c.l[2 * i + 1] = (uint32_t)(l[i] >> 32); }
    return fr_to_mont(c);
}

GArgs pob_detail::gargs(pob_ctx* h) {
    GArgs A; memset(&A, 0, sizeof A);
    A.units = h->d_units; A.order = h->d_order; A.L = h->d_L;
    A.bits = h->d_bits; A.sm = h->d_sm; A.fr = h->d_fr;
    A.bits_stride = h->plan.total.b; A.sm_stride = (uint64_t)h->plan.total.s * 64; A.fr_stride = (uint64_t)h->plan.total.f * 512;
    A.pos_tab = h->d_pos; A.inv_lut = h->d_inv; A.pow256 = h->d_pow256; A.npow256 = h->npow256; A.in_fr = h->d_in_fr[h->in_cur]; A.in_sm = h->d_in_sm[h->in_cur];
    A.nfr_in = h->plan.nfr_in; A.nsm_in = h->plan.nsm_in;
    A.status = h->d_status_raw; A.chk_status = h->d_chk; A.bad_wire = h->d_bad; A.emit_counters = h->d_emit_ctr;
    A.fault_cls = 0xFFFFFFFFu;
    return A;
}
static KArgs kargs(pob_ctx* h) {
    KArgs K; memset(&K, 0, sizeof K);
    K.bits = (u64*)h->d_bits; K.group_stride = h->plan.total.b; K.sponges = h->d_sponges;
    K.perm_sponge = h->d_perm_sponge; K.perm_block = h->d_perm_block; K.bad_wire = h->d_bad;
    return K;
}

static bool small_param(const uint64_t* l, uint64_t lo, uint64_t hi, int* out) {
    if (l[1] | l[2] | l[3]) return false;
    if (l[0] < lo || l[0] > hi) return false;
    *out = (int)l[0];
    return true;
}
static Fr field_param(const uint64_t* l) {
    Fr c; for (int i = 0; i < 4; i++) { c.l[2 * i] = (uint32_t)l[i]; c.l[2 * i + 1] = (uint32_t)(l[i] >> 32); }
    for (int k = 0; k < 6 && fr_geq_p(c); k++) c = fr_sub_p(c);
    return fr_to_mont(c);
}
static int make_plan(Plan& plan, std::string& err, int circuit, const uint64_t* params, int nparams) {
    if (circuit == POB_CIRCUIT_PROOF_OF_BURN) {
        if (nparams != 8) { err = "ProofOfBurn takes 8 template parameters"; return POB_E_ARG; }
        PobParams prm;
        if (!small_param(params + 0, 2, 64, &prm.L) || !small_param(params + 4, 1, 16, &prm.NB) || !small_param(params + 8, 1, 32, &prm.HB) ||
            !small_param(params + 12, 0, 64, &prm.minNib) || !small_param(params + 16, 1, 31, &prm.amountBytes) || !small_param(params + 20, 0, 32, &prm.powZero) ||
            4 + prm.L > MAX_KB || prm.L > MAX_SC) {
            err = "unsupported ProofOfBurn parameters (maxNumLayers 2..64, maxNodeBlocks 1..16, maxHeaderBlocks 1..32, minLeafAddressNibbles 0..64, "
                  "amountBytes 1..31, powMinimumZeroBytes 0..32)";
            return POB_E_ARG;
        }
        prm.maxIntended = field_param(params + 24); prm.maxActual = field_param(params + 28);
        const uint64_t perms = (uint64_t)prm.L * prm.NB + prm.HB + 2 + 1 + 1;
        if (perms * 2600000ull >= (1ull << 29)) { err = "instantiation too large for the 32-bit layout offsets (more than 206 Keccak-f permutations)"; return POB_E_ARG; }
        plan.plan_pob(prm);
    } else if (circuit == POB_CIRCUIT_SPEND) {
        int mab = 0;
        if (nparams != 1 || !small_param(params, 1, 31, &mab)) { err = "Spend takes maxAmountBytes in 1..31"; return POB_E_ARG; }
        SpendParams sp; sp.maxAmountBytes = mab;
        plan.plan_spend(sp);
    } else if (circuit == POB_CIRCUIT_GADGET) {
        int tid = 0, prm[4] = {0, 0, 0, 0};
        if (nparams < 1 || nparams > 5 || !small_param(params, 1, GM_TEMPLATE_COUNT - 1, &tid)) { err = "gadget main: params[0] must be a template id (pob_gadget_template)"; return POB_E_ARG; }
        for (int k = 1; k < nparams; k++) if (!small_param(params + 4 * k, 0, 1 << 20, &prm[k - 1])) { err = "gadget main: template parameter out of range"; return POB_E_ARG; }
        const char* why = plan.plan_gadget((uint32_t)tid, prm, nparams - 1);
        if (why) { err = std::string("gadget main: ") + why; return POB_E_ARG; }
    } else { err = "unknown circuit"; return POB_E_ARG; }
    const Cur t = plan.total;
    if (t.b >= (1u << 29) || t.s >= (1u << 24) || t.f >= (1u << 21) || t.q >= (1u << 30)) {
        err = "instantiation exceeds the layout's offset limits (BIT < 2^29, SM < 2^24, FR < 2^21 wires)"; return POB_E_ARG;
    }
    return POB_OK;
}
static void fill_info(const Plan& pl, uint32_t nperms, uint32_t max_batch, pob_info_t* info) {
    info->n_witness = pl.total.w; info->n_bit = pl.total.b; info->n_sm = pl.total.s; info->n_fr = pl.total.f;
    info->n_fr_inputs = pl.nfr_in; info->n_sm_inputs = pl.nsm_in; info->n_outputs = pl.L.circuit == 2 ? pl.L.gm.nout : 1;
    info->n_units = (uint32_t)pl.units.size(); info->n_sponges = (uint32_t)pl.sponges.size(); info->n_perms = nperms;
    { std::vector<char> used(pl.max_stage + 1, 0); for (const UnitDesc& u : pl.units) if (u.flags & UNIT_GEN) used[u.stage] = 1; for (const SpongeDesc& s : pl.sponges) used[s.stage] = 1;
      info->n_stages = 0; for (char c : used) info->n_stages += c; }
    info->max_batch = max_batch;
    info->group_bytes = (uint64_t)pl.total.b * 8 + (uint64_t)pl.total.s * 256 + (uint64_t)pl.total.f * 2048;
    info->n_derived = pl.total.q;
    info->n_alias = (uint64_t)nperms * ABSORB_ALIAS;
    info->kchk_rounds = (uint32_t)pob_kchk_rounds(); info->kgc_rounds = (uint32_t)pob_kgc_rounds();
    info->keccak_bit_wires = 0;
    for (const SpongeDesc& s : pl.sponges) info->keccak_bit_wires += (uint64_t)s.n * (ABSORB_WIRES + 2 * 1088) + (uint64_t)(s.n + 1) * 1600;
}

extern "C" {

int pob_plan_info(int circuit, const uint64_t* params, int nparams, pob_info_t* info) {
    if (!info) return POB_E_ARG;
    Plan* plan = new Plan(); std::string err;
    int rc;
    try { rc = make_plan(*plan, err, circuit, params, nparams); } catch (const std::exception& e) { fprintf(stderr, "%s\n", e.what()); rc = POB_E_STATE; }
    if (rc == POB_OK) { uint32_t np = 0; for (const SpongeDesc& sd : plan->sponges) np += sd.n; fill_info(*plan, np, 0, info); }
    delete plan;
    return rc;
}

int pob_gadget_template(const char* name, int* nparams) {
    if (!name) return -1;
    for (const GmName& g : GM_NAMES) if (!strcmp(g.name, name)) { if (nparams) *nparams = g.nparams; return (int)g.id; }
    return -1;
}

const char* pob_strerror(pob_handle h) { return h ? h->err.c_str() : "null handle"; }

int pob_open(int device, int circuit, const uint64_t* params, int nparams, uint32_t max_batch, pob_handle* out) {
    if (!out || max_batch == 0) return POB_E_ARG;
    pob_ctx* h = new pob_ctx();
    *out = h;
    h->device = device; h->circuit = circuit; h->max_batch = max_batch; h->groups = (max_batch + 63) / 64;
    try { int prc = make_plan(h->plan, h->err, circuit, params, nparams); if (prc) return prc; }
    catch (const std::exception& e) { h->err = e.what(); return POB_E_STATE; }
    Plan& pl = h->plan;
    {
        const uint64_t pre[4] = {0xf0363f983d892f7eULL, 0xd115b780980a6b46ULL, 0x007d2482cd46cec2ULL, 0x0ba44186ee7876b8ULL};
        Fr base = limbs_to_mont(pre);
        pl.L.prefix[0] = base; pl.L.prefix[1] = fr_add(base, fr_one_mont()); pl.L.prefix[2] = fr_add(pl.L.prefix[1], fr_one_mont());
    }
    std::stable_sort(pl.sponges.begin(), pl.sponges.end(), [&](const SpongeDesc& a, const SpongeDesc& b) { return a.stage < b.stage; });
    std::vector<uint32_t> perm_sponge, perm_block;
    for (uint32_t s = 0; s <= pl.max_stage; s++) {
        for (uint32_t lds = N_GEN_CLASSES; lds-- > 0;) {
            pob_ctx::Seg sg{s, lds, (uint32_t)h->order.size(), 0};
            for (uint32_t u = 0; u < pl.units.size(); u++) {
                if (!(pl.units[u].flags & UNIT_GEN)) continue;
                if (pl.units[u].stage == s && unit_class(pl.units[u].kind, true) == lds) h->order.push_back(u);
            }
            sg.count = (uint32_t)h->order.size() - sg.first;
            std::stable_sort(h->order.begin() + sg.first, h->order.end(), [&](uint32_t a, uint32_t b) { return pl.units[a].cost > pl.units[b].cost; });
            if (sg.count) h->segs.push_back(sg);
        }
        {
            pob_ctx::KSeg ks{s, 0, 0, (uint32_t)perm_sponge.size(), 0, nullptr};
            bool first = true;
            for (uint32_t i = 0; i < pl.sponges.size(); i++) if (pl.sponges[i].stage == s) {
                if (first) { ks.sp_first = i; first = false; }
                ks.sp_count++;
                for (uint32_t b = 0; b < pl.sponges[i].n; b++) { perm_sponge.push_back(i); perm_block.push_back(b); }
            }
            ks.perm_count = (uint32_t)perm_sponge.size() - ks.perm_first;
            if (ks.sp_count) h->ksegs.push_back(ks);
        }
    }
    h->nperms = (uint32_t)perm_sponge.size();
    for (uint32_t cls = 0; cls < N_GEN_CLASSES; cls++) {
        pob_ctx::Seg sg{0, cls, (uint32_t)h->order.size(), 0};
        for (uint32_t u = 0; u < pl.units.size(); u++) if ((pl.units[u].flags & UNIT_EMIT) && unit_class(pl.units[u].kind) == cls) h->order.push_back(u);
        sg.count = (uint32_t)h->order.size() - sg.first;
        if (sg.count) h->emit_segs.push_back(sg);
    }
    for (uint32_t fam = 0; fam < F_COUNT; fam++) {
        pob_ctx::Seg sg{0, fam, (uint32_t)h->order.size(), 0};
        for (uint32_t u = 0; u < pl.units.size(); u++) if ((pl.units[u].flags & UNIT_CHECK) && fam_of(pl.units[u].kind) == fam) h->order.push_back(u);
        sg.count = (uint32_t)h->order.size() - sg.first;
        std::stable_sort(h->order.begin() + sg.first, h->order.end(), [&](uint32_t a, uint32_t b) { return pl.units[a].cost > pl.units[b].cost; });
        if (sg.count) h->chk_segs.push_back(sg);
    }

    for (int variant = 0; variant < 2; variant++) {
        const bool fused = variant == 1;
        const uint32_t NS = (pl.max_stage / Plan::TRACK_STRIDE + 1) * Plan::TRACK_STRIDE;
// ... 31 lines not shown
                pob_ctx::GenLaunch gl{pob_ctx::GL_UNITS, cls, (uint32_t)h->order.size(), 0, 0, 0};
                for (const pob_ctx::Seg& sg : h->segs) if ((cls == CLS_ALL ? (sg.lds == 0 || sg.lds == 1 || sg.lds == 3) : sg.lds == cls) && has_g[sg.stage] && lvl_g[sg.stage] == lv)
                    for (uint32_t j2 = 0; j2 < sg.count; j2++) h->order.push_back(h->order[sg.first + j2]);
                gl.count = (uint32_t)h->order.size() - gl.first;
                std::stable_sort(h->order.begin() + gl.first, h->order.end(), [&](uint32_t a, uint32_t b) { return pl.units[a].cost > pl.units[b].cost; });
                if (!gl.count) continue;
                if (cls == 4 && fused) pos = gl;
                else plan.push_back(gl);
            }
            for (const pob_ctx::KSeg& ks : h->ksegs) if (lvl_end[ks.stage] == lv) {
                if (pos.count) { plan.push_back({pob_ctx::GL_POS_CHAIN, 4, pos.first, pos.count, ks.sp_first, ks.sp_count}); pos.count = 0; }
                else plan.push_back({pob_ctx::GL_CHAIN, 0, 0, 0, ks.sp_first, ks.sp_count});
            }
            if (pos.count) plan.push_back(pos);
        }
        if (h->nperms) plan.push_back({pob_ctx::GL_ROUNDS, 0, 0, 0, 0, h->nperms});
        if (getenv("POB_DEBUG_LEVELS")) {
            fprintf(stderr, "---- in-order launch plan %d (%s), %d levels\n", variant, fused ? "fused" : "one launch per kernel", nlev);
            for (const pob_ctx::GenLaunch& gl : plan) {
                fprintf(stderr, "kind %u class %u: %5u units, sponges / permutations [%u, +%u)", gl.kind, gl.cls, gl.count, gl.k_first, gl.k_count);
                if (gl.count && gl.kind != pob_ctx::GL_CHAIN && gl.kind != pob_ctx::GL_ROUNDS) {
                    fprintf(stderr, " longest unit cost %u:", pl.units[h->order[gl.first]].cost);
                    std::vector<uint32_t> kinds(U_KIND_COUNT, 0);
                    for (uint32_t j2 = 0; j2 < gl.count; j2++) kinds[pl.units[h->order[gl.first + j2]].kind]++;
                    for (uint32_t k = 0; k < U_KIND_COUNT; k++) if (kinds[k]) fprintf(stderr, " %u x kind %u", kinds[k], k);
                }
                fprintf(stderr, "\n");
            }
        }
    }

    {
        h->chk_narrow = pob_ctx::Seg{0, 0, (uint32_t)h->order.size(), 0};
        for (uint32_t u = 0; u < pl.units.size(); u++) {
            const uint32_t f = fam_of(pl.units[u].kind);
            if ((pl.units[u].flags & UNIT_CHECK) && (f == F_MISC || f == F_RL || f == F_POS || f == F_N2B)) h->order.push_back(u);
        }
        h->chk_narrow.count = (uint32_t)h->order.size() - h->chk_narrow.first;
        std::stable_sort(h->order.begin() + h->chk_narrow.first, h->order.end(), [&](uint32_t a, uint32_t b) { return pl.units[a].cost > pl.units[b].cost; });
        h->chk_ride_kept.first = (uint32_t)h->order.size();
        for (uint32_t u = 0; u < pl.units.size(); u++) if ((pl.units[u].flags & UNIT_CHECK) && ride_keeps_evaluation(pl.units[u].kind)) h->order.push_back(u);
        h->chk_ride_kept.count = (uint32_t)h->order.size() - h->chk_ride_kept.first;
    }

    HIPC(hipSetDevice(device));
    int prio_lo = 0, prio_hi = 0;
    HIPC(hipDeviceGetStreamPriorityRange(&prio_lo, &prio_hi));
    {
        std::lock_guard<std::mutex> lk(g_pool_mu);
        StreamPool* P = nullptr;
        for (StreamPool* q : g_pools) if (q->device == device) P = q;
        if (!P) {
            P = new StreamPool(); P->device = device;
            hipStream_t* want[7] = {&P->stream2, &P->stream_k, &P->track1, &P->track2, &P->chk1, &P->chk2, &P->s_in};
            hipError_t e = hipSuccess;
            for (int k = 0; k < 7 && e == hipSuccess; k++) e = hipStreamCreateWithPriority(want[k], hipStreamNonBlocking, (k == 1 || k == 4 || k == 5) ? prio_lo : prio_hi);
            if (e != hipSuccess) {
                for (hipStream_t* q : want) if (*q) hipStreamDestroy(*q);
                delete P;
                h->err = std::string("hipStreamCreateWithPriority: ") + hipGetErrorString(e);
                return POB_E_HIP;
            }
            g_pools.push_back(P);
        }
        P->refs++; h->pool = P;
    }
    h->stream2 = h->pool->stream2; h->stream_k = h->pool->stream_k;
    hipStream_t p_track1 = h->pool->track1, p_track2 = h->pool->track2;
    HIPC(hipEventCreateWithFlags(&h->ev_join3, hipEventDisableTiming));
    HIPC(hipEventCreateWithFlags(&h->ev_rounds_fork, hipEventDisableTiming));
    HIPC(hipEventCreateWithFlags(&h->ev_g_done, hipEventDisableTiming)); HIPC(hipEventCreateWithFlags(&h->ev_k_done, hipEventDisableTiming));
    HIPC(hipEventCreateWithFlags(&h->ev_gen_done, hipEventDisableTiming)); HIPC(hipEventCreateWithFlags(&h->ev_check_done, hipEventDisableTiming));
    for (pob_ctx::KSeg& ks : h->ksegs) HIPC(hipEventCreateWithFlags(&ks.ev_done, hipEventDisableTiming));
    HIPC(hipEventCreateWithFlags(&h->ev_fork, hipEventDisableTiming)); HIPC(hipEventCreateWithFlags(&h->ev_join, hipEventDisableTiming));
    for (uint32_t t = 1; t < Plan::MAX_TRACKS; t++) {
        pob_ctx::Track& T = h->tracks[t];
        T.s_main = t == 1 ? p_track1 : t == 2 ? p_track2 : t == 3 ? p_track2 : t == 6 ? p_track1 : h->stream2;
        T.s_heavy = T.s_main;
        HIPC(hipEventCreateWithFlags(&T.ev_fork, hipEventDisableTiming)); HIPC(hipEventCreateWithFlags(&T.ev_join, hipEventDisableTiming));
        HIPC(hipEventCreateWithFlags(&T.ev_start, hipEventDisableTiming)); HIPC(hipEventCreateWithFlags(&T.ev_end, hipEventDisableTiming));
    }
    h->stream3 = p_track1;
    const uint64_t G = h->groups, npad = G * 64;
    HIPC(hipMalloc(&h->d_bits, G * (uint64_t)std::max(pl.total.b, 1u) * 8));
    HIPC(hipMalloc(&h->d_sm, G * (uint64_t)std::max(pl.total.s, 1u) * 256));
    HIPC(hipMalloc(&h->d_fr, G * (uint64_t)std::max(pl.total.f, 1u) * 2048));
    HIPC(hipMalloc(&h->d_units, pl.units.size() * sizeof(UnitDesc)));
    HIPC(hipMalloc(&h->d_order, h->order.size() * sizeof(uint32_t)));
    HIPC(hipMalloc(&h->d_L, sizeof(CircuitLayout)));
    HIPC(hipMalloc(&h->d_sponges, std::max<size_t>(pl.sponges.size(), 1) * sizeof(SpongeDesc)));
    HIPC(hipMalloc(&h->d_perm_sponge, std::max<size_t>(h->nperms, 1) * 4));
    HIPC(hipMalloc(&h->d_perm_block, std::max<size_t>(h->nperms, 1) * 4));
    HIPC(hipMalloc(&h->d_pos, sizeof(POS_TABLE_MONT)));
    HIPC(hipMalloc(&h->d_inv, 8193 * 32));
    HIPC(hipMalloc(&h->d_emit_ctr, 4 * 4)); HIPC(hipMemset(h->d_emit_ctr, 0, 4 * 4));
    {
        h->npow256 = 136u * (uint32_t)std::max(pl.L.pob.NB, 1);
        std::vector<Fr> tab(2 * (size_t)h->npow256);
        const Fr c256 = fr_from_i64(256);
        Fr pw = fr_one_mont();
        for (uint32_t i = 0; i < h->npow256; i++) { tab[i] = pw; tab[h->npow256 + i] = fr_to_mont(pw); pw = fr_mul(pw, c256); }
        HIPC(hipMalloc(&h->d_pow256, tab.size() * sizeof(Fr)));
        HIPC(hipMemcpy(h->d_pow256, tab.data(), tab.size() * sizeof(Fr), hipMemcpyHostToDevice));
    }
    for (int k = 0; k < 2; k++) {
        HIPC(hipMalloc(&h->d_in_fr[k], std::max<uint64_t>(npad * (uint64_t)pl.nfr_in * 32, 32)));
        HIPC(hipMalloc(&h->d_in_sm[k], std::max<uint64_t>(npad * (uint64_t)pl.nsm_in * 4, 4)));
        HIPC(hipMemset(h->d_in_fr[k], 0, std::max<uint64_t>(npad * (uint64_t)pl.nfr_in * 32, 32)));
        HIPC(hipMemset(h->d_in_sm[k], 0, std::max<uint64_t>(npad * (uint64_t)pl.nsm_in * 4, 4)));
        if (pl.nsm_in) {
            HIPC(hipMalloc(&h->d_in_sm8[k], npad * (uint64_t)pl.nsm_in + 16));
            HIPC(hipMalloc(&h->d_in_exc[k], npad * POB_EXC_CAP * sizeof(pob_sm_exc_t)));
        }
        HIPC(hipEventCreateWithFlags(&h->ev_in_done[k], hipEventDisableTiming));
    }
    HIPC(hipMalloc(&h->d_status_raw, npad * 4)); HIPC(hipMalloc(&h->d_status, npad * 4));
    HIPC(hipMalloc(&h->d_chk, npad * 4)); HIPC(hipMalloc(&h->d_bad, npad * 4));
    HIPC(hipMalloc(&h->d_outputs, npad * 32));
    HIPC(hipMalloc(&h->d_records, npad * POB_RECORD_BYTES));
    for (int k = 0; k < 2; k++) {
        HIPC(hipHostMalloc((void**)&h->h_records[k], npad * POB_RECORD_BYTES, hipHostMallocDefault));
        HIPC(hipEventCreateWithFlags(&h->ev_rec[k], hipEventDisableTiming));
    }

    HIPC(hipMemcpy(h->d_units, pl.units.data(), pl.units.size() * sizeof(UnitDesc), hipMemcpyHostToDevice));
    HIPC(hipMemcpy(h->d_order, h->order.data(), h->order.size() * 4, hipMemcpyHostToDevice));
    HIPC(hipMemcpy(h->d_L, &pl.L, sizeof(CircuitLayout), hipMemcpyHostToDevice));
    if (!pl.sponges.empty()) HIPC(hipMemcpy(h->d_sponges, pl.sponges.data(), pl.sponges.size() * sizeof(SpongeDesc), hipMemcpyHostToDevice));
    if (h->nperms) {
        HIPC(hipMemcpy(h->d_perm_sponge, perm_sponge.data(), h->nperms * 4, hipMemcpyHostToDevice));
        HIPC(hipMemcpy(h->d_perm_block, perm_block.data(), h->nperms * 4, hipMemcpyHostToDevice));
    }
    HIPC(hipMemcpy(h->d_pos, POS_TABLE_MONT, sizeof(POS_TABLE_MONT), hipMemcpyHostToDevice));
    if (h->nperms) {
        std::vector<uint16_t> tab(KECCAKF_ROUND_WIRES);
        if (!keccak_alias_table_host(tab.data())) { h->err = "internal: the KeccakfRound walk does not name every wire of the block exactly once"; return POB_E_STATE; }
        HIPC(hipMalloc(&h->d_ktab, tab.size() * 2));
        HIPC(hipMemcpy(h->d_ktab, tab.data(), tab.size() * 2, hipMemcpyHostToDevice));
    }
    HIPC(hipMemset(h->d_status_raw, 0xFF, npad * 4)); HIPC(hipMemset(h->d_chk, 0xFF, npad * 4)); HIPC(hipMemset(h->d_bad, 0xFF, npad * 4));
    hipLaunchKernelGGL(k_init_invlut, dim3((8193 + 63) / 64), dim3(64), 0, h->stream2, h->d_inv);
    HIPC(hipGetLastError());
    HIPC(hipStreamSynchronize(h->stream2));
    return POB_OK;
}

void pob_close(pob_handle h) {
    if (!h) return;
    hipSetDevice(h->device);
    void* ptrs[] = {h->d_bits, h->d_sm, h->d_fr, h->d_units, h->d_order, h->d_L, h->d_sponges, h->d_perm_sponge, h->d_perm_block, h->d_pos,
                    h->d_inv, h->d_pow256, h->d_ktab, h->d_emit_ctr, h->d_in_fr[0], h->d_in_fr[1], h->d_in_sm[0], h->d_in_sm[1], h->d_in_sm8[0], h->d_in_sm8[1], h->d_in_exc[0], h->d_in_exc[1], h->d_status_raw, h->d_status, h->d_chk, h->d_bad, h->d_outputs, h->d_records};
    for (void* p : ptrs) if (p) hipFree(p);
    emit_release(h);
    hipDeviceSynchronize();
    for (int k = 0; k < 2; k++) { if (h->h_records[k]) hipHostFree(h->h_records[k]); if (h->ev_rec[k]) hipEventDestroy(h->ev_rec[k]); }
    if (h->ev_upload) hipEventDestroy(h->ev_upload);
    for (hipEvent_t e : h->ev_in_done) if (e) hipEventDestroy(e);
    for (auto& pr : h->ev_kchk) for (hipEvent_t e : pr) if (e) hipEventDestroy(e);
    if (h->partner && h->partner->partner == h) h->partner->partner = nullptr;
    emit_release_streams(h);
    if (h->pool) {
        std::lock_guard<std::mutex> lk(g_pool_mu);
        StreamPool* P = h->pool;
        if (--P->refs == 0) {
            for (hipStream_t q : {P->stream2, P->stream_k, P->track1, P->track2, P->chk1, P->chk2, P->s_in}) if (q) hipStreamDestroy(q);
            g_pools.erase(std::find(g_pools.begin(), g_pools.end(), P));
            delete P;
// ... 402 lines not shown
    return POB_OK;
}

int pob_results_records_device(pob_handle h, void** d_records) {
    if (!h || !d_records) return POB_E_ARG;
    *d_records = h->d_records;
    return POB_OK;
}

int pob_probe_check_kernel(pob_handle h, int enable, float* ms) {
    if (!h) return POB_E_ARG;
    HIPC(hipSetDevice(h->device));
    if (ms) {
        uint32_t sl = h->rec_slot;
        if (!h->kchk_rec[sl] || hipEventQuery(h->ev_kchk[sl][1]) != hipSuccess) sl ^= 1;
        if (!h->ev_kchk[sl][0] || !h->kchk_rec[sl]) { h->err = "no timed evaluation yet"; return POB_E_STATE; }
        HIPC(hipEventSynchronize(h->ev_kchk[sl][1]));
        HIPC(hipEventElapsedTime(ms, h->ev_kchk[sl][0], h->ev_kchk[sl][1]));
    }
    if (enable && !h->ev_kchk[0][0]) for (auto& pr : h->ev_kchk) for (hipEvent_t& e : pr) HIPC(hipEventCreate(&e));
    if (!enable) { for (auto& pr : h->ev_kchk) for (hipEvent_t& e : pr) if (e) { hipEventDestroy(e); e = nullptr; } h->kchk_rec[0] = h->kchk_rec[1] = false; }
    return POB_OK;
}

int pob_time_kernel(pob_handle h, int which, int iters, void* stream_, float* avg_ms) {
    if (!h || !h->generated || iters < 1 || !avg_ms) return POB_E_STATE;
    HIPC(hipSetDevice(h->device));
    hipStream_t st = stream_ ? (hipStream_t)stream_ : own_stream(h);
    const uint32_t G = (h->n + 63) / 64;
    hipEvent_t e0, e1;
    HIPC(hipEventCreate(&e0)); HIPC(hipEventCreate(&e1));
    KArgs K = kargs(h); K.first = 0;
    GArgs A = gargs(h);
    uint32_t* d_sel = nullptr; uint32_t nsel = 0, sel_cls = 0, sel_fam = 0;
    if (which >= 100 && which < 300) {
        const uint32_t kind = (uint32_t)which % 100, need = which >= 200 ? UNIT_GEN : UNIT_CHECK;
        std::vector<uint32_t> sel;
        for (uint32_t u = 0; u < h->plan.units.size(); u++) if (h->plan.units[u].kind == kind && (h->plan.units[u].flags & need)) sel.push_back(u);
        if (sel.empty()) { *avg_ms = 0; hipEventDestroy(e0); hipEventDestroy(e1); return POB_OK; }
        nsel = (uint32_t)sel.size(); sel_cls = unit_class(kind, which >= 200); sel_fam = fam_of(kind);
        HIPC(hipMalloc(&d_sel, nsel * 4)); HIPC(hipMemcpy(d_sel, sel.data(), nsel * 4, hipMemcpyHostToDevice));
        A.order = d_sel; A.first = 0;
    }
    HIPC(hipEventRecord(e0, st));
    for (int it = 0; it < iters; it++) {
        if (which >= 300) {
            for (const pob_ctx::Seg& sg : h->chk_segs) if (sg.lds == (uint32_t)which - 300) { A.first = sg.first; launch_g_check(A, sg.lds, sg.count, G, st); }
        } else if (which >= 200) launch_g_gen(A, sel_cls, nsel, G, st);
        else if (which >= 100) launch_g_check(A, sel_fam, nsel, G, st);
        else if (which == 0) launch_k_rounds(K, false, h->nperms, G, st);
        else if (which == 1) launch_k_rounds(K, true, h->nperms, G, st);
        else if (which == 6) launch_k_rounds_gc(K, h->nperms, G, false, st);
        else if (which == 2) {
            for (const pob_ctx::Seg& sg : h->chk_segs) {
                A.first = sg.first;
                launch_g_check(A, sg.lds, sg.count, G, st);
            }
        } else launch_k_chain(K, false, (uint32_t)h->plan.sponges.size(), G, st);
    }
    HIPC(hipEventRecord(e1, st));
    HIPC(hipEventSynchronize(e1));
    float ms = 0; HIPC(hipEventElapsedTime(&ms, e0, e1));
    *avg_ms = ms / iters;
    hipEventDestroy(e0); hipEventDestroy(e1);
    if (d_sel) hipFree(d_sel);
    return POB_OK;
}

int pob_debug_stream_create(int device, const uint32_t* cu_mask, uint32_t words, void** stream) {
    if (!cu_mask || !words || !stream) return POB_E_ARG;
    if (hipSetDevice(device) != hipSuccess) return POB_E_HIP;
    hipStream_t st = nullptr;
    if (hipExtStreamCreateWithCUMask(&st, words, cu_mask) != hipSuccess) return POB_E_HIP;
    *stream = (void*)st;
    return POB_OK;
}
void pob_debug_stream_destroy(int device, void* stream) { if (stream && hipSetDevice(device) == hipSuccess) hipStreamDestroy((hipStream_t)stream); }

int pob_debug_store_fault(pob_handle h, int cls, uint32_t group, uint64_t index, uint64_t mask, uint32_t* wire) {
    if (!h || group >= h->groups) return POB_E_ARG;
    if (!h->inorder || !h->gc) { h->err = "pob_debug_store_fault: the calculator's generation carries no evaluation (pob_set_inorder bit 2)"; return POB_E_STATE; }
    bool found = false;
    if (cls == POB_CLASS_BIT) {
        if (index >= h->plan.total.b) return POB_E_ARG;
        for (const SpongeDesc& sp : h->plan.sponges) {
            if (index < sp.abs_b || index >= sp.abs_b + (uint64_t)sp.n * ABSORB_BITS) continue;
            const uint32_t b = (uint32_t)((index - sp.abs_b) / ABSORB_BITS), o = (uint32_t)((index - sp.abs_b) % ABSORB_BITS);
            if (o < AB_DIRECT) break;
            if (wire) *wire = sp.abs_w + b * ABSORB_WIRES + AB_ROUNDS_W + (o - AB_DIRECT) / KR_BITS * KECCAKF_ROUND_WIRES;
            found = true; break;
        }
    } else if (cls == POB_CLASS_SM && h->circuit == POB_CIRCUIT_PROOF_OF_BURN) {
        const SmRef r0 = h->plan.L.pm.numLeafAddressNibbles;
        if (index >= r0.i && index < r0.i + h->plan.nsm_in) { found = true; if (wire) *wire = r0.w + (uint32_t)(index - r0.i); }
    }
    h->fault_g = !found;
    if (!found) {
        const Cur t = h->plan.total;
        if (!(h->circuit == POB_CIRCUIT_PROOF_OF_BURN || h->circuit == POB_CIRCUIT_SPEND) || (cls == POB_CLASS_BIT ? index >= t.b : cls == POB_CLASS_SM ? index >= t.s : cls == POB_CLASS_FR ? index >= t.f : true)) {
            h->err = "pob_debug_store_fault: not a stored word whose evaluation rides with its generation"; return POB_E_ARG;
        }
        if (wire) *wire = 0xFFFFFFFFu;
    }
    h->fault_armed = true; h->fault_value = false; h->fault_cls = cls; h->fault_group = group; h->fault_word = index; h->fault_mask = mask;
    return POB_OK;
}

int pob_debug_value_fault(pob_handle h, int cls, uint32_t group, uint64_t index, uint64_t mask, uint32_t* wire) {
    if (!h || group >= h->groups) return POB_E_ARG;
    if (!h->inorder || !h->gc) { h->err = "pob_debug_value_fault: the calculator's generation carries no evaluation (pob_set_inorder bit 2)"; return POB_E_STATE; }
    const Cur t = h->plan.total;
    if (!(cls == POB_CLASS_BIT ? index < t.b : cls == POB_CLASS_SM ? index < t.s : cls == POB_CLASS_FR ? index < t.f : false)) { h->err = "pob_debug_value_fault: no such word"; return POB_E_ARG; }
    auto refuse = [&](const char* why) { h->err = std::string("pob_debug_value_fault: not covered: ") + why; return POB_E_ARG; };
    if (!(h->circuit == POB_CIRCUIT_PROOF_OF_BURN || h->circuit == POB_CIRCUIT_SPEND)) return refuse("the G units of a gadget-level main do not ride");
    if (cls == POB_CLASS_BIT) return refuse("BIT words (round blocks, sponge chains, the G units' bit runs)");
    if (cls == POB_CLASS_SM && h->circuit == POB_CIRCUIT_PROOF_OF_BURN) {
        const SmRef r0 = h->plan.L.pm.numLeafAddressNibbles;
        if (index >= r0.i && index < r0.i + h->plan.nsm_in) return refuse("an input row (stored from the packed inputs, no unit computes it)");
    }
    uint32_t w = 0xFFFFFFFFu;
    bool in_block = false;
    if (cls == POB_CLASS_FR) for (const UnitDesc& d : h->plan.units) if (d.kind == U_POS_WIDE) {
        const int T = (int)d.a[0];
        if (index < d.cur.f || index >= (uint64_t)d.cur.f + pos_wires(T, pos_off(T).rp)) continue;
        if (!posw_value_fault_covers(T, (uint32_t)(index - d.cur.f))) return refuse("an element of a Poseidon block that does not carry the running state (Sigma internals, operand copies)");
        w = d.cur.w + (uint32_t)(index - d.cur.f); in_block = true;
    }
    if (!in_block) {
        uint64_t best = 0; bool any = false, rl = false;
        for (const UnitDesc& d : h->plan.units) if ((d.flags & UNIT_GEN) && d.kind != U_POS_WIDE) {
            const uint64_t s = cls == POB_CLASS_SM ? d.cur.s : d.cur.f;
            if (s > index) continue;
            if (!any || s > best) { best = s; any = true; rl = false; }
            if (s == best && ride_keeps_evaluation(d.kind)) rl = true;
        }
        if (rl) return refuse("a wire of the RLP units, which generate on the plain policy");
    }
    if (wire) *wire = w;
    if (mask == 0) { if (h->fault_value) h->fault_armed = false; return POB_OK; }
    h->fault_g = true; h->fault_armed = true; h->fault_value = true; h->fault_cls = cls; h->fault_group = group; h->fault_word = index; h->fault_mask = mask;
    return POB_OK;
}

int pob_debug_xor_bits(pob_handle h, uint32_t group, uint64_t bit_index, uint64_t mask) {
    if (!h || group >= h->groups || bit_index >= h->plan.total.b) return POB_E_ARG;
    HIPC(hipSetDevice(h->device));
    h->rode = false;
    hipLaunchKernelGGL(k_xor_word, dim3(1), dim3(1), 0, own_stream(h), h->d_bits + (uint64_t)group * h->plan.total.b + bit_index, mask);
    HIPC(hipStreamSynchronize(own_stream(h)));
    return POB_OK;
}

int pob_debug_poke(pob_handle h, int cls, uint32_t group, uint64_t index, uint32_t sub, uint32_t lane, uint32_t xor_mask) {
    if (!h || group >= h->groups || lane >= 64) return POB_E_ARG;
    HIPC(hipSetDevice(h->device));
    h->rode = false;
    const Cur t = h->plan.total;
    if (cls == POB_CLASS_BIT) {
        if (index >= t.b) return POB_E_ARG;
        hipLaunchKernelGGL(k_xor_word, dim3(1), dim3(1), 0, own_stream(h), h->d_bits + (uint64_t)group * t.b + index, (uint64_t)(xor_mask & 1u) << lane);
    } else if (cls == POB_CLASS_SM) {
        if (index >= t.s) return POB_E_ARG;
        hipLaunchKernelGGL(k_xor_u32, dim3(1), dim3(1), 0, own_stream(h), (uint32_t*)h->d_sm + ((uint64_t)group * t.s + index) * 64 + lane, xor_mask);
    } else if (cls == POB_CLASS_FR) {
        if (index >= t.f || sub >= 8) return POB_E_ARG;
        hipLaunchKernelGGL(k_xor_u32, dim3(1), dim3(1), 0, own_stream(h), h->d_fr + ((uint64_t)group * t.f + index) * 512 + sub * 64 + lane, xor_mask);
    } else return POB_E_ARG;
    HIPC(hipStreamSynchronize(own_stream(h)));
    return POB_OK;
}

int pob_debug_fr_inv(int device, const uint8_t* in, uint32_t n, uint8_t* out_kaliski, uint8_t* out_fermat) {
    if (!in || !out_kaliski || !out_fermat || n == 0) return POB_E_ARG;
    if (hipSetDevice(device) != hipSuccess) return POB_E_HIP;
    uint32_t *d_in = nullptr, *d_a = nullptr, *d_b = nullptr;
    const size_t bytes = (size_t)n * 32;
    int rc = POB_E_HIP;
    if (hipMalloc(&d_in, bytes) == hipSuccess && hipMalloc(&d_a, bytes) == hipSuccess && hipMalloc(&d_b, bytes) == hipSuccess &&
        hipMemcpy(d_in, in, bytes, hipMemcpyHostToDevice) == hipSuccess) {
        hipLaunchKernelGGL(k_fr_inv_test, dim3((n + 63) / 64), dim3(64), 0, 0, d_in, d_a, d_b, n);
        if (hipMemcpy(out_kaliski, d_a, bytes, hipMemcpyDeviceToHost) == hipSuccess && hipMemcpy(out_fermat, d_b, bytes, hipMemcpyDeviceToHost) == hipSuccess) rc = POB_OK;
    }
    if (d_in) hipFree(d_in); if (d_a) hipFree(d_a); if (d_b) hipFree(d_b);
    return rc;
}

int pob_debug_fr_sqr(int device, const uint8_t* in, uint32_t n, uint8_t* out_sqr, uint8_t* out_mul) {
    if (!in || !out_sqr || !out_mul || n == 0) return POB_E_ARG;
    if (hipSetDevice(device) != hipSuccess) return POB_E_HIP;
    uint32_t *d_in = nullptr, *d_a = nullptr, *d_b = nullptr;
    const size_t bytes = (size_t)n * 32;
    int rc = POB_E_HIP;
    if (hipMalloc(&d_in, bytes) == hipSuccess && hipMalloc(&d_a, bytes) == hipSuccess && hipMalloc(&d_b, bytes) == hipSuccess &&
        hipMemcpy(d_in, in, bytes, hipMemcpyHostToDevice) == hipSuccess) {
        hipLaunchKernelGGL(k_fr_sqr_test, dim3((n + 63) / 64), dim3(64), 0, 0, d_in, d_a, d_b, n);
        if (hipMemcpy(out_sqr, d_a, bytes, hipMemcpyDeviceToHost) == hipSuccess && hipMemcpy(out_mul, d_b, bytes, hipMemcpyDeviceToHost) == hipSuccess) rc = POB_OK;
    }
    if (d_in) hipFree(d_in); if (d_a) hipFree(d_a); if (d_b) hipFree(d_b);
    return rc;
}

int pob_debug_ref(pob_handle h, const char* name, uint32_t k, int* cls, uint64_t* index, uint64_t* wire) {
    if (!h || !name || !cls || !index || !wire) return POB_E_ARG;
    const Plan& pl = h->plan; const CircuitLayout& L = pl.L;
    const std::string n = name;
    auto set = [&](int c, uint64_t i, uint64_t w) { *cls = c; *index = i; *wire = w; return POB_OK; };
    if (n == "poseidon" || n == "poseidon.t3" || n == "poseidon.t4" || n == "poseidon.t5") {
        const uint32_t want_t = n.size() > 8 ? (uint32_t)(n[10] - '0') : 0;
        for (const UnitDesc& u : pl.units) if (u.kind == CK_POS_SEG && (want_t == 0 || u.a[0] == want_t)) {
            if (k >= pos_wires((int)u.a[0], pos_off((int)u.a[0]).rp)) return POB_E_ARG;
            return set(POB_CLASS_FR, u.cur.f + k, u.cur.w + k);
        }
        return POB_E_ARG;
    }
    if (n == "commitment") { const FrRef r = h->circuit == POB_CIRCUIT_PROOF_OF_BURN ? L.pm.commitment : L.sm.commitment; return set(POB_CLASS_FR, r.i, r.w); }
    if (n == "kb.inLen") { if (k >= L.nkb) return POB_E_ARG; return set(POB_CLASS_SM, L.kbs[k].inLen.i, L.kbs[k].inLen.w); }
    if (n == "kb.inBlocks" || n == "kb.absorb") {
        if (k >= L.nkb) return POB_E_ARG;
        const KBRefs& r = L.kbs[k];
        return n == "kb.inBlocks" ? set(POB_CLASS_BIT, r.inBlocks.i, r.inBlocks.w) : set(POB_CLASS_BIT, r.abs_b + AB_MID, r.abs_w);
    }
    if (n == "pad.div.out" || n == "pad.div.rem") {
        if (k >= L.nkb) return POB_E_ARG;
        const KBRefs& r = L.kbs[k];
        const uint32_t o = n == "pad.div.rem" ? 1 : 0;
        return set(POB_CLASS_SM, r.c_div.s + o, r.c_div.w + o);
    }
    if (h->circuit == POB_CIRCUIT_PROOF_OF_BURN && L.nsc > 1) {
        const ScRefs& sc = L.scs[1];
        const uint32_t mm = 136u * (uint32_t)L.pob.NB, kk = mm - 31 + 1;
        if (n == "sc.exists" && k < kk) return set(POB_CLASS_BIT, sc.ex.i + k, sc.ex.w + k);
    }
    return POB_E_ARG;
}

static const int KROT_H[25] = {1, 10, 7, 11, 17, 18, 3, 5, 16, 8, 21, 24, 4, 15, 23, 19, 13, 12, 2, 20, 14, 22, 9, 6, 1};
static uint64_t rotl64h(uint64_t v, int n) { return n ? (v << n) | (v >> (64 - n)) : v; }
static void keccak_f_host(uint64_t a[25]) {
    static const uint64_t RC[24] = {
        0x0000000000000001ULL, 0x0000000000008082ULL, 0x800000000000808AULL, 0x8000000080008000ULL, 0x000000000000808BULL,
        0x0000000080000001ULL, 0x8000000080008081ULL, 0x8000000000008009ULL, 0x000000000000008AULL, 0x0000000000000088ULL,
        0x0000000080008009ULL, 0x000000008000000AULL, 0x000000008000808BULL, 0x800000000000008BULL, 0x8000000000008089ULL,
        0x8000000000008003ULL, 0x8000000000008002ULL, 0x8000000000000080ULL, 0x000000000000800AULL, 0x800000008000000AULL,
        0x8000000080008081ULL, 0x8000000000008080ULL, 0x0000000080000001ULL, 0x8000000080008008ULL};
    for (int r = 0; r < 24; r++) {
        uint64_t c[5], b[25];
        for (int x = 0; x < 5; x++) c[x] = a[x] ^ a[x + 5] ^ a[x + 10] ^ a[x + 15] ^ a[x + 20];
        for (int x = 0; x < 5; x++) { uint64_t d = c[(x + 4) % 5] ^ rotl64h(c[(x + 1) % 5], 1); for (int y = 0; y < 25; y += 5) a[x + y] ^= d; }
        b[0] = a[0];
        for (int i = 0; i < 24; i++) b[KROT_H[i + 1]] = rotl64h(a[KROT_H[i]], ((i + 1) * (i + 2) / 2) % 64);
        for (int i = 0; i < 25; i++) { int y = i / 5 * 5; a[i] = b[i] ^ (~b[y + (i + 1) % 5] & b[y + (i + 2) % 5]); }
        a[0] ^= RC[r];
    }
}
void pob_keccak256(const uint8_t* msg, uint64_t len, uint8_t out[32]) {
    uint64_t st[25]; memset(st, 0, sizeof st);
    uint8_t blk[136];
    for (uint64_t off = 0;; off += 136) {
        uint64_t n = len - off < 136 ? len - off : 136;
        memset(blk, 0, 136); if (n) memcpy(blk, msg + off, n);
        const bool last = n < 136;
        if (last) { blk[n] ^= 0x01; blk[135] ^= 0x80; }
        for (int i = 0; i < 17; i++) { uint64_t v; memcpy(&v, blk + 8 * i, 8); st[i] ^= v; }
        keccak_f_host(st);
        if (last) break;
    }
    memcpy(out, st, 32);
}

int64_t pob_pow_search(const uint8_t start_key[32], const uint8_t* postfix, uint32_t postfix_len, uint32_t zero_bytes, uint64_t max_tries, uint8_t out_key[32]) {
    if (postfix_len > 100 || zero_bytes > 8) return -1;
    uint8_t msg[136];
    memcpy(msg, start_key, 32); memcpy(msg + 32, postfix, postfix_len);
    const uint32_t len = 32 + postfix_len;
    for (uint64_t t = 0; t < max_tries; t++) {
        uint8_t blk[136]; memset(blk, 0, 136); memcpy(blk, msg, len); blk[len] ^= 0x01; blk[135] ^= 0x80;
        uint64_t st[25]; memset(st, 0, sizeof st);
        for (int i = 0; i < 17; i++) { uint64_t v; memcpy(&v, blk + 8 * i, 8); st[i] = v; }
        keccak_f_host(st);
        const uint64_t mask = zero_bytes == 8 ? ~0ULL : ((1ULL << (8 * zero_bytes)) - 1);
        if ((st[0] & mask) == 0) { memcpy(out_key, msg, 32); return (int64_t)t; }
        for (int i = 31; i >= 0; i--) if (++msg[i]) break;
    }
    return -1;
}

int64_t pob_pow_search_gpu(int device, const uint8_t start_key[32], const uint8_t* postfix, uint32_t postfix_len, uint32_t zero_bytes,
                           uint64_t max_tries, uint8_t out_key[32]) {
    if (postfix_len > 100 || zero_bytes > 8 || zero_bytes == 0) return -1;
    if (hipSetDevice(device) != hipSuccess) return -2;
    uint8_t blk[136]; memset(blk, 0, 136);
    memcpy(blk + 32, postfix, postfix_len);
    const uint32_t len = 32 + postfix_len;
    blk[len] ^= 0x01; blk[135] ^= 0x80;
    uint64_t tail[13];
    for (int i = 0; i < 13; i++) memcpy(&tail[i], blk + 32 + 8 * i, 8);
    uint64_t kw[4];
    for (int i = 0; i < 4; i++) { uint64_t v = 0; for (int j = 0; j < 8; j++) v = (v << 8) | start_key[8 * i + j]; kw[i] = v; }
    uint64_t* d_tail = nullptr; unsigned long long* d_found = nullptr;
    if (hipMalloc(&d_tail, sizeof tail) != hipSuccess || hipMalloc(&d_found, 8) != hipSuccess) return -2;
    hipMemcpy(d_tail, tail, sizeof tail, hipMemcpyHostToDevice);
    const uint64_t mask = zero_bytes == 8 ? ~0ULL : ((1ULL << (8 * zero_bytes)) - 1);
    const uint64_t WIN = 1ULL << 24;
// ... 22 lines not shown
```

### proof_of_burn_amd/csrc/policy.hpp

```cpp
#pragma once
#include <stdint.h>
#include "fr_dev.hpp"

typedef uint64_t B;
typedef int32_t S;
typedef Fr F;

struct Cur { uint32_t w, b, s, f, q; };
HD Cur cur_add(Cur a, Cur d, uint32_t k) { Cur r = {a.w + d.w * k, a.b + d.b * k, a.s + d.s * k, a.f + d.f * k, a.q + d.q * k}; return r; }
struct BitRef { uint32_t w, i; HD BitRef operator+(uint32_t k) const { BitRef r = {w + k, i + k}; return r; } };
struct SmRef  { uint32_t w, i; HD SmRef  operator+(uint32_t k) const { SmRef  r = {w + k, i + k}; return r; } };
struct FrRef  { uint32_t w, i; HD FrRef  operator+(uint32_t k) const { FrRef  r = {w + k, i + k}; return r; } };

enum : uint32_t {
    T_NUM2BITS = 1, T_ISZERO, T_ALIASCHECK, T_ASSERT_LT, T_ASSERT_LE, T_ASSERT_GE, T_DIVIDE, T_SELECTOR,
    T_POW, T_POB, T_INPUT, T_COMPCONST, T_MISC
};
#define FAILCODE(tpl, line) (((uint32_t)(tpl) << 12) | (uint32_t)(line))

#if defined(__HIP_DEVICE_COMPILE__)
#define POB_DECL_ORDER_DEFAULT 0u
#else
#include <stdlib.h>
static inline uint32_t pob_decl_order_env() { static const uint32_t v = (getenv("POB_DECL_ORDER") && getenv("POB_DECL_ORDER")[0] == '1') ? 1u : 0u; return v; }
#define POB_DECL_ORDER_DEFAULT pob_decl_order_env()
#endif
struct PolBase {
    Cur cur;
    uint32_t decl_order = POB_DECL_ORDER_DEFAULT;
    HD BitRef bits(uint32_t n) { BitRef r = {cur.w, cur.b}; cur.w += n; cur.b += n; return r; }
    HD SmRef sms(uint32_t n) { SmRef r = {cur.w, cur.s}; cur.w += n; cur.s += n; return r; }
    HD uint32_t dvs(uint32_t n) { const uint32_t w = cur.w; cur.w += n; cur.q += n; return w; }
    HD FrRef frs(uint32_t n) { FrRef r = {cur.w, cur.f}; cur.w += n; cur.f += n; return r; }
    HD void skip_alias(uint32_t nw, uint32_t nb) { cur.w += nw; cur.b += nb; }
};

enum : uint32_t { NOTE_POSEIDON = 1, NOTE_N2BE = 2, NOTE_SHIFTRIGHT = 3, NOTE_SHIFTLEFT = 4 };
struct PlanNote { uint32_t what, n; Cur cur; uint32_t a[7]; };
#define PLAN_MAX_NOTES 8
struct CountP : PolBase {
    static constexpr bool is_gen = false, is_check = false, is_emit = false, is_count = true, ride = false;
    uint32_t nput = 0;
    uint32_t nb = 0, ns = 0, nf = 0;
    PlanNote notes[PLAN_MAX_NOTES]; uint32_t nnotes = 0;
    bool notes_overflow = false;
    HD void note(uint32_t what, uint32_t n, Cur c, uint32_t a0 = 0, uint32_t a1 = 0, uint32_t a2 = 0, uint32_t a3 = 0, uint32_t a4 = 0, uint32_t a5 = 0, uint32_t a6 = 0) {
        if (nnotes >= PLAN_MAX_NOTES) { notes_overflow = true; return; }
        PlanNote& x = notes[nnotes++]; x.what = what; x.n = n; x.cur = c;
        x.a[0] = a0; x.a[1] = a1; x.a[2] = a2; x.a[3] = a3; x.a[4] = a4; x.a[5] = a5; x.a[6] = a6;
    }
    HD B put(BitRef, B v) { nput++; nb++; return v; }
    HD S put(SmRef, S v) { nput++; ns++; return v; }
    HD F put(FrRef, const F& v) { nput += 8; nf++; return v; }
    HD B hint(BitRef, B v) { nput++; nb++; return v; }
    HD S hint(SmRef, S v) { nput++; ns++; return v; }
    HD F hint(FrRef, const F& v) { nput += 8; nf++; return v; }
    HD B get(BitRef) { return 0; }
    HD S get(SmRef) { return 0; }
    HD S get_lane(SmRef, uint32_t) { return 0; }
    HD void derived(uint32_t, S) {}
    HD void derived_inv(uint32_t, S, bool = false) {}
    HD void derived_fr(uint32_t, const F&) {}
    HD void derived_fr_inv(uint32_t, const F&, bool = true) {}
    HD void site_m(uint32_t, uint32_t, uint32_t) {}
    HD void site_c(uint32_t, uint32_t) {}
    HD F get(FrRef) { return fr_zero(); }
    HD void raw_put(FrRef, const F&) {}
    HD B ballot(bool) { return 0; }
    HD bool bit(B) { return false; }
    HD void require(B, uint32_t) {}
    HD void require_lane(bool, uint32_t) {}
    HD F kconst(uint32_t) { return fr_zero(); }
    HD F k256(uint32_t) { return fr_zero(); }
    HD F k256r(uint32_t) { return fr_zero(); }
    HD F input_fr(uint32_t) { return fr_zero(); }
    HD S input_sm(uint32_t) { return 0; }
    HD uint32_t lane_id() { return 0; }
    HD B run_get(uint32_t, uint32_t) { return 0; }
    HD void run_put(uint32_t n, uint32_t, uint32_t, B) { nput += n; nb += n; }
    HD void run_derived(uint32_t, uint32_t, B) {}
    HD B run_bcast(B, uint32_t) { return 0; }
    HD B xpose64(uint32_t, uint32_t, uint32_t) { return 0; }
    HD B xpose(B, uint32_t) { return 0; }
    HD B run_set(B run, uint32_t, B) { return run; }
    HD B run_perm(B run, uint32_t) { return run; }
};

template <int N> struct SmLoaded { S s[N]; };
template <class P, int N> HD __attribute__((always_inline)) SmLoaded<N> sm_load(P& p, const SmRef (&r)[N]) {
    SmLoaded<N> h;
    if constexpr (P::is_check) {
#pragma unroll
        for (int k = 0; k < N; k++) h.s[k] = p.get(r[k]);
    } else {
#pragma unroll
        for (int k = 0; k < N; k++) h.s[k] = 0;
    }
    return h;
}
template <class P, int N> HD __attribute__((always_inline)) void sm_commit(P& p, const SmRef (&r)[N], const SmLoaded<N>& h, const S (&v)[N]) {
    if constexpr (P::is_check) {
#pragma unroll
        for (int k = 0; k < N; k++) p.mark(h.s[k] != v[k], r[k].w);
        p.pin();
    } else {
#pragma unroll
        for (int k = 0; k < N; k++) p.put(r[k], v[k]);
    }
}
template <class P, int BATCH, class RefFn, class ValFn> HD __attribute__((always_inline)) void sm_puts_at(P& p, int n, RefFn ref, ValFn val) {
    for (int i0 = 0; i0 < n; i0 += BATCH) {
        SmRef rr[BATCH]; S vv[BATCH];
#pragma unroll
        for (int q = 0; q < BATCH; q++) rr[q] = ref(i0 + q < n ? i0 + q : n - 1);
        const SmLoaded<BATCH> h = sm_load(p, rr);
#pragma unroll
        for (int q = 0; q < BATCH; q++) vv[q] = val(i0 + q < n ? i0 + q : n - 1);
        sm_commit(p, rr, h, vv);
    }
}
template <class P, int BATCH, class ValFn> HD __attribute__((always_inline)) void sm_puts(P& p, SmRef base, int n, ValFn val) {
    sm_puts_at<P, BATCH>(p, n, [&](int i) { return base + (uint32_t)i; }, val);
}
struct BV { B r[4]; };
template <class P> HD __attribute__((always_inline)) BV bv_from_canon(P& p, const F& c, int n) {
    BV v;
#pragma unroll
    for (int q = 0; q < 4; q++) v.r[q] = (64 * q < n) ? p.xpose64(c.l[2 * q], c.l[2 * q + 1], (uint32_t)(n - 64 * q)) : 0;
// ... 434 lines not shown
```

### proof_of_burn_amd/witness.py

```python
from __future__ import annotations

import ctypes
import json
import os
import re
from dataclasses import dataclass
from typing import Iterable, Sequence

import numpy as np

P = 21888242871839275222246405745257275088548364400416034343698204186575808495617
_HERE = os.path.dirname(os.path.abspath(__file__))
LIB_PATH = os.environ.get("POB_LIB_PATH") or os.path.join(_HERE, "csrc", "libpob_hip.so")

POB_FR_INPUTS = ["burnKey", "actualBalance", "intendedBalance", "revealAmount", "burnExtraCommitment", "_proofExtraCommitment"]
POB_SM_INPUTS = ["numLeafAddressNibbles", "layers", "layerLens", "numLayers", "blockHeader", "blockHeaderLen", "byteSecurityRelax"]
SPEND_FR_INPUTS = ["burnKey", "balance", "withdrawnBalance", "extraCommitment"]

_TPL = {1: "Num2Bits", 2: "IsZero", 3: "AliasCheck", 4: "AssertLessThan", 5: "AssertLessEqThan", 6: "AssertGreaterEqThan",
        7: "Divide", 8: "Selector", 9: "ProofOfWorkChecker", 10: "ProofOfBurn", 11: "input", 12: "CompConstant", 13: "misc"}
FAIL_INPUT_RANGE = (11 << 12) | 1

GADGET_INPUTS = {
    "EIP7503": lambda p: [],
    "ConcatFixed4": lambda p: [("a", "s", p[0]), ("b", "s", p[1]), ("c", "s", p[2]), ("d", "s", p[3])],
    "ProofOfWorkChecker": lambda p: [("burnKey", "f", 1), ("revealAmount", "f", 1), ("burnExtraCommitment", "f", 1), ("minimumZeroBytes", "s", 1)],
    "PublicCommitment": lambda p: [("in", "s", 32 * p[0])],
    "Poseidon": lambda p: [("inputs", "f", p[0])],
    "Divide": lambda p: [("a", "s", 1), ("b", "s", 1)],
    "SubstringCheck": lambda p: [("mainInput", "s", p[0]), ("mainLen", "s", 1), ("subInput", "s", p[1])],
    "ShiftLeft": lambda p: [("in", "s", p[0]), ("count", "s", 1)],
    "ShiftRight": lambda p: [("in", "s", p[0]), ("count", "s", 1)],
    "Mask": lambda p: [("in", "s", p[0]), ("count", "s", 1)],
    "Concat": lambda p: [("a", "s", p[0]), ("aLen", "s", 1), ("b", "s", p[1]), ("bLen", "s", 1)],
    "Selector": lambda p: [("vals", "s", p[0]), ("select", "s", 1)],
    "SelectorArray1D": lambda p: [("arrays", "s", p[0] * p[1]), ("select", "s", 1)],
    "SelectorArray2D": lambda p: [("arrays", "s", p[0] * p[1] * p[2]), ("select", "s", 1)],
    "BigEndianBytes2Num": lambda p: [("in", "s", p[0])],
    "LittleEndianBytes2Num": lambda p: [("in", "s", p[0])],
    "Bytes2Nibbles": lambda p: [("in", "s", p[0])],
    "Nibbles2Bytes": lambda p: [("nibbles", "s", 2 * p[0])],
    "Num2BigEndianBytes": lambda p: [("in", "f", 1)],
    "Num2LittleEndianBytes": lambda p: [("in", "f", 1)],
    "Num2BitsSafe": lambda p: [("in", "f", 1)],
    "Pad": lambda p: [("in", "s", p[0] * p[1]), ("inLen", "s", 1)],
    "KeccakBytes": lambda p: [("in", "s", 136 * p[0]), ("inLen", "s", 1)],
    "BurnAddress": lambda p: [("burnKey", "f", 1), ("revealAmount", "f", 1), ("burnExtraCommitment", "f", 1)],
    "BurnAddressHash": lambda p: [("burnKey", "f", 1), ("revealAmount", "f", 1), ("burnExtraCommitment", "f", 1)],
    "AssertBits": lambda p: [("in", "f", 1)],
    "AssertByteString": lambda p: [("in", "s", p[0])],
    "AssertLessEqThan": lambda p: [("a", "s", 1), ("b", "s", 1)],
    "AssertLessThan": lambda p: [("a", "s", 1), ("b", "s", 1)],
    "AssertGreaterEqThan": lambda p: [("a", "s", 1), ("b", "s", 1)],
    "Filter": lambda p: [("in", "s", 1)],
    "Fit": lambda p: [("in", "s", p[0])],
    "Reverse": lambda p: [("in", "s", p[0])],
    "Flatten": lambda p: [("in", "s", p[0] * p[1])],
    "Reshape": lambda p: [("in", "s", p[0] * p[1])],
    "RlpInteger": lambda p: [("in", "f", 1)],
    "CountBytes": lambda p: [("bytes", "s", p[0])],
    "RlpEmptyAccount": lambda p: [("balance", "f", 1)],
    "TruncatedAddressHash": lambda p: [("addressHashNibbles", "s", 2 * p[0]), ("addressHashNibblesLen", "s", 1)],
    "IsInRange": lambda p: [("lower", "s", 1), ("value", "s", 1), ("upper", "s", 1)],
    "LeafDetector": lambda p: [("layer", "s", p[0]), ("layerLen", "s", 1)],
    "RlpMerklePatriciaTrieLeaf": lambda p: [("addressHashNibbles", "s", 2 * p[0]), ("addressHashNibblesLen", "s", 1), ("balance", "f", 1)],
}


def circuit_of(name: str, params):
    if name == "ProofOfBurn":
        return 0, list(params)
    if name == "Spend":
        return 1, list(params)
    if name not in GADGET_INPUTS:
        raise NotImplementedError(f"{name} is not a template of the reference's circuits")
    npar = ctypes.c_int()
    tid = load_library().pob_gadget_template(name.encode(), ctypes.byref(npar))
    if tid < 0:
        raise NotImplementedError(f"{name}: unknown to libpob_hip.so")
    if npar.value != len(params):
        raise ValueError(f"{name} takes {npar.value} template parameters, got {len(params)}")
    return 2, [tid] + list(params)


def _limbs(params):
    arr = (ctypes.c_uint64 * (4 * max(len(params), 1)))()
    for i, v in enumerate(params):
        for k in range(4):
            arr[4 * i + k] = (int(v) >> (64 * k)) & 0xFFFFFFFFFFFFFFFF
    return arr


class PobInfo(ctypes.Structure):
    _fields_ = [("n_witness", ctypes.c_uint64), ("n_bit", ctypes.c_uint64), ("n_sm", ctypes.c_uint64), ("n_fr", ctypes.c_uint64),
                ("n_fr_inputs", ctypes.c_uint32), ("n_sm_inputs", ctypes.c_uint32), ("n_outputs", ctypes.c_uint32),
                ("n_units", ctypes.c_uint32), ("n_sponges", ctypes.c_uint32), ("n_perms", ctypes.c_uint32),
                ("n_stages", ctypes.c_uint32), ("max_batch", ctypes.c_uint32),
                ("group_bytes", ctypes.c_uint64), ("keccak_bit_wires", ctypes.c_uint64), ("n_derived", ctypes.c_uint64), ("n_alias", ctypes.c_uint64),
                ("kchk_rounds", ctypes.c_uint32), ("kgc_rounds", ctypes.c_uint32)]


RECORD_DTYPE = np.dtype([("status", "<u4"), ("check_status", "<u4"), ("bad_wire", "<u4"), ("commitment", "u1", (32,))])
NOT_EVALUATED, CLEAN = 0xFFFFFFFE, 0xFFFFFFFF
EXC_CAP, EXC_NONE, E_RANGE, E_NOMEM = 32, 0xFFFFFFFF, -6, -3
EXC_DTYPE = np.dtype([("k", "<u4"), ("v", "<i4")])

_lib = None


def load_library() -> ctypes.CDLL:
    global _lib
    if _lib is not None:
        return _lib
    if not os.path.exists(LIB_PATH):
        raise RuntimeError(f"{LIB_PATH} is missing: run `python -c 'import __graft_entry__ as g; g.build()'` "
                           "(hipcc --offload-arch=gfx950).  There is no CPU fallback.")
    lib = ctypes.CDLL(LIB_PATH)
    vp, u32p, u8p = ctypes.c_void_p, ctypes.POINTER(ctypes.c_uint32), ctypes.POINTER(ctypes.c_uint8)
    lib.pob_open.argtypes = [ctypes.c_int, ctypes.c_int, ctypes.POINTER(ctypes.c_uint64), ctypes.c_int, ctypes.c_uint32, ctypes.POINTER(vp)]
    lib.pob_close.argtypes = [vp]
    lib.pob_close.restype = None
    lib.pob_get_info.argtypes = [vp, ctypes.POINTER(PobInfo)]
    lib.pob_plan_info.argtypes = [ctypes.c_int, ctypes.POINTER(ctypes.c_uint64), ctypes.c_int, ctypes.POINTER(PobInfo)]
    lib.pob_strerror.argtypes = [vp]
    lib.pob_strerror.restype = ctypes.c_char_p
    lib.pob_gadget_template.argtypes = [ctypes.c_char_p, ctypes.POINTER(ctypes.c_int)]
    lib.pob_gadget_template.restype = ctypes.c_int
    lib.pob_upload_inputs.argtypes = [vp, vp, vp, ctypes.c_uint32]
    lib.pob_upload_inputs_async.argtypes = [vp, vp, vp, ctypes.c_uint32, vp]
    lib.pob_upload_inputs8.argtypes = [vp, vp, vp, vp, ctypes.c_uint32]
    lib.pob_upload_inputs8_async.argtypes = [vp, vp, vp, vp, ctypes.c_uint32, vp]
    lib.pob_narrow_inputs.argtypes = [vp, ctypes.c_uint32, ctypes.c_uint32, vp, vp]
    lib.pob_pack_json_batch8.argtypes = [ctypes.c_int, ctypes.POINTER(ctypes.c_uint64), ctypes.c_int, ctypes.POINTER(ctypes.c_char_p), ctypes.POINTER(ctypes.c_uint64),
                                         ctypes.c_uint32, ctypes.c_int, vp, vp, vp, vp, ctypes.c_char_p, ctypes.c_uint32]
    lib.pob_host_alloc.argtypes = [ctypes.POINTER(vp), ctypes.c_uint64]
    lib.pob_pack_json.argtypes = [ctypes.c_int, ctypes.POINTER(ctypes.c_uint64), ctypes.c_int, ctypes.c_char_p, ctypes.c_uint64, vp, vp, vp, ctypes.c_char_p, ctypes.c_uint32]
    lib.pob_pack_json_batch.argtypes = [ctypes.c_int, ctypes.POINTER(ctypes.c_uint64), ctypes.c_int, ctypes.POINTER(ctypes.c_char_p), ctypes.POINTER(ctypes.c_uint64),
                                        ctypes.c_uint32, ctypes.c_int, vp, vp, vp, ctypes.c_char_p, ctypes.c_uint32]
    lib.pob_host_free.argtypes = [vp]
    lib.pob_host_free.restype = None
    lib.pob_results_fetch.argtypes = [vp]
    lib.pob_results_wait.argtypes = [vp, ctypes.POINTER(vp), u32p]
    lib.pob_emit_begin_reduced.argtypes = [vp, ctypes.c_uint32, vp, ctypes.c_uint64, ctypes.c_uint64]
    lib.pob_write_wtns_reduced.argtypes = [vp, ctypes.c_uint32, vp, ctypes.c_uint64, ctypes.c_char_p]
    lib.pob_reduced_map_pin.argtypes = [vp, vp, ctypes.c_uint64]
    lib.pob_emit_measure_ex.argtypes = [vp, ctypes.c_uint32, ctypes.c_uint32, ctypes.c_uint64, vp, ctypes.c_uint64, ctypes.POINTER(ctypes.c_double), ctypes.POINTER(ctypes.c_uint64)]
    lib.pob_generate.argtypes = [vp, vp]
    lib.pob_constraint_check.argtypes = [vp, vp]
    lib.pob_sync.argtypes = [vp]
    lib.pob_set_partner.argtypes = [vp, vp]
    lib.pob_results.argtypes = [vp, vp, vp, vp, vp]
    lib.pob_results_device.argtypes = [vp, ctypes.POINTER(vp), ctypes.POINTER(vp)]
    lib.pob_results_records_device.argtypes = [vp, ctypes.POINTER(vp)]
    lib.pob_gather_records.argtypes = [vp, vp, vp, vp, ctypes.c_uint32]
    lib.pob_emit_witness.argtypes = [vp, ctypes.c_uint32, vp, ctypes.c_uint64]
    lib.pob_write_wtns.argtypes = [vp, ctypes.c_uint32, ctypes.c_char_p]
    lib.pob_emit_begin.argtypes = [vp, ctypes.c_uint32, ctypes.c_uint64]
    lib.pob_emit_next.argtypes = [vp, ctypes.POINTER(ctypes.c_void_p), ctypes.POINTER(ctypes.c_uint64), ctypes.POINTER(ctypes.c_uint64)]
    lib.pob_emit_queue.argtypes = [vp, ctypes.c_uint32]
    lib.pob_emit_measure.argtypes = [vp, ctypes.c_uint32, ctypes.c_uint32, ctypes.c_uint64, ctypes.POINTER(ctypes.c_double), ctypes.POINTER(ctypes.c_uint64)]
    if hasattr(lib, "pob_emit_begin_packed"):
        lib.pob_emit_begin_packed.argtypes = [vp, ctypes.c_uint32, vp, ctypes.c_uint64, ctypes.c_uint64]
        lib.pob_emit_next_packed.argtypes = [vp, ctypes.POINTER(ctypes.c_void_p), ctypes.POINTER(ctypes.c_uint64), ctypes.POINTER(ctypes.c_uint64), ctypes.POINTER(ctypes.c_uint64)]
        lib.pob_unpack_window.argtypes = [vp, ctypes.c_uint64, vp, ctypes.c_uint64, ctypes.c_int]
        lib.pob_write_wtns_packed.argtypes = [vp, ctypes.c_uint32, vp, ctypes.c_uint64, ctypes.c_char_p]
        lib.pob_emit_measure_packed.argtypes = [vp, ctypes.c_uint32, ctypes.c_uint32, ctypes.c_uint64, vp, ctypes.c_uint64, vp, ctypes.c_uint64, ctypes.c_int,
                                                ctypes.POINTER(ctypes.c_double), ctypes.POINTER(ctypes.c_double), ctypes.POINTER(ctypes.c_uint64)]
    if hasattr(lib, "pob_emit_begin_group_packed"):
        lib.pob_emit_begin_group_packed.argtypes = [vp, ctypes.c_uint32, ctypes.c_uint64, vp, ctypes.c_uint64, ctypes.c_uint64, ctypes.POINTER(ctypes.c_uint64)]
        lib.pob_emit_next_group_packed.argtypes = [vp, ctypes.POINTER(ctypes.c_void_p), ctypes.POINTER(ctypes.c_uint64), ctypes.POINTER(ctypes.c_uint64), ctypes.POINTER(ctypes.c_uint64)]
        lib.pob_write_wtns_group.argtypes = [vp, ctypes.c_uint32, ctypes.c_uint64, vp, ctypes.c_uint64, ctypes.POINTER(ctypes.c_char_p)]
        lib.pob_emit_measure_group.argtypes = [vp, ctypes.c_uint32, ctypes.c_uint32, ctypes.c_uint64, ctypes.c_uint64, vp, ctypes.c_uint64, vp, ctypes.c_uint64, ctypes.c_int,
                                               ctypes.POINTER(ctypes.c_double), ctypes.POINTER(ctypes.c_double), ctypes.POINTER(ctypes.c_uint64)]
    if hasattr(lib, "pob_emit_group_selfcheck"):
        lib.pob_emit_group_selfcheck.argtypes = [vp, ctypes.c_int]
        lib.pob_emit_group_selfcheck_result.argtypes = [vp, ctypes.POINTER(ctypes.c_uint64), ctypes.POINTER(ctypes.c_uint64), ctypes.POINTER(ctypes.c_uint64), ctypes.POINTER(ctypes.c_uint32)]
        lib.pob_debug_selfcheck_sites.argtypes = [vp, ctypes.c_int, vp, ctypes.c_uint64, ctypes.POINTER(ctypes.c_uint64)]
        lib.pob_debug_group_emit_xor.argtypes = [vp, ctypes.c_uint32, ctypes.c_uint32, ctypes.c_uint32, ctypes.c_uint8]
    lib.pob_time_kernel.argtypes = [vp, ctypes.c_int, ctypes.c_int, vp, ctypes.POINTER(ctypes.c_float)]
    lib.pob_probe_check_kernel.argtypes = [vp, ctypes.c_int, ctypes.POINTER(ctypes.c_float)]
    lib.pob_debug_xor_bits.argtypes = [vp, ctypes.c_uint32, ctypes.c_uint64, ctypes.c_uint64]
    lib.pob_debug_store_fault.argtypes = [vp, ctypes.c_int, ctypes.c_uint32, ctypes.c_uint64, ctypes.c_uint64, ctypes.POINTER(ctypes.c_uint32)]
# ... 840 lines not shown
```

Measured before the change: 1.253 million.

## Align Keccak BIT slabs to 16-word boundaries with padded group stride

```diff
diff --git a/include/pob_hip.h b/include/pob_hip.h
--- a/include/pob_hip.h
+++ b/include/pob_hip.h
@@ -21,6 +21,7 @@
     uint64_t n_alias;
     uint32_t kchk_rounds;
     uint32_t kgc_rounds;
+    uint64_t bit_stride;
 } pob_info_t;
 
 int pob_open(int device, int circuit, const uint64_t* params, int nparams, uint32_t max_batch, pob_handle* out);
diff --git a/proof_of_burn_amd/csrc/circuits.hpp b/proof_of_burn_amd/csrc/circuits.hpp
--- a/proof_of_burn_amd/csrc/circuits.hpp
+++ b/proof_of_burn_amd/csrc/circuits.hpp
@@ -120,6 +120,8 @@
 
 #define SC_RANGE_POS 32
 #define MAX_KB 72
+static_assert(BIT_PAD_MAX >= 2 * MAX_KB + 1, "two padding runs per KeccakBytes instance and the slab's end");
+static_assert(ABSORB_BITS % BIT_ALIGN == 0 && AB_DIRECT % BIT_ALIGN == 0 && KR_BITS % BIT_ALIGN == 0 && 1600u % BIT_ALIGN == 0 && 1088u % BIT_ALIGN == 0, "every offset inside a sponge keeps the line alignment of its first word");
 #define MAX_SC 64
 struct CircuitLayout {
     int circuit;
@@ -161,16 +163,18 @@
 }
 
 #define NO_RANK 0xFFFFFFFFu
+#define KB_HEAD_TAIL_BITS 251u
 template <class P> HD BitRef dbits(P& p, uint32_t n) { BitRef r = {p.dvs(n), NO_RANK}; return r; }
 template <class P> GD void kb_head(P& p, int mb, S inLen, KBRefs& r) {
     const uint32_t m = 136 * mb;
     r.mb = mb;
     r.out = p.sms(32); r.in = p.sms(m); r.inLen = p.sms(1); r.padded_w = p.dvs(m); r.numBlocks = p.sms(1);
-    r.inBitsArray = dbits(p, 8 * m); r.inBits = dbits(p, 8 * m); r.inBlocks = p.bits(8 * m); r.outBits = dbits(p, 256); r.outBytes = dbits(p, 256);
+    r.inBitsArray = dbits(p, 8 * m); r.inBits = dbits(p, 8 * m); p.align_bits(); r.inBlocks = p.bits(8 * m); r.outBits = dbits(p, 256); r.outBytes = dbits(p, 256);
     inLen = p.put(r.inLen, inLen);
     gAssertLessThanS(p, 16, inLen, (S)m);
     r.pad_o_w = p.dvs(m); r.pad_nb = p.sms(1); r.pad_in_w = p.dvs(m); r.pad_il = p.sms(1); r.pad_dv = p.sms(1); r.pad_rm = p.sms(1);
     r.pad_flt = p.bits(m + 1); r.pad_isEq = p.bits(m); r.pad_isLast = p.bits(m);
+    p.align_bits(KB_HEAD_TAIL_BITS);
     inLen = p.put(r.pad_il, inLen);
     S q, rem;
     r.c_div = p.cur;
@@ -264,6 +268,7 @@
     const uint32_t n = r.mb;
     r.k_out = dbits(p, 256); r.k_in = dbits(p, n * 1088); r.k_blocks = p.sms(1); r.k_finalState = dbits(p, 1600);
     r.f_out = dbits(p, 1600); r.f_in = dbits(p, n * 1088); r.f_blocks = p.sms(1); r.f_s = dbits(p, (n + 1) * 1600);
+    p.align_bits();
     r.abs_w = p.cur.w; r.abs_b = p.cur.b;
     p.skip_alias(n * ABSORB_WIRES, n * ABSORB_BITS);
     r.sel_out = dbits(p, 1600); r.sel_arrays = dbits(p, (n + 1) * 1600); r.sel_select = p.sms(1); r.sel_T = dbits(p, 1600 * (n + 1));
@@ -967,6 +972,8 @@
     std::vector<UnitDesc> units;
     std::vector<SpongeDesc> sponges;
     Cur total;
+    uint32_t bit_stride;
+    PadLog pads;
     uint32_t nfr_in, nsm_in, max_stage;
     enum { TRACK_STRIDE = 32, MAX_TRACKS = 7 };
     uint32_t ntracks, track_fork[MAX_TRACKS], track_join[MAX_TRACKS];
@@ -1033,6 +1040,7 @@
     void keccak_tail(uint32_t kb, uint32_t range_stage, SmRef dst, bool has_dst) {
         KBRefs& r = L.kbs[kb];
         r.index = kb;
+        if (p.cur.b % BIT_ALIGN) throw std::runtime_error("layout planner: KB_HEAD_TAIL_BITS is not the BIT footprint between kb_head's padding step and the sponge");
         kb_declare_keccak(p, r);
         SpongeDesc s; s.n = r.mb; s.stage = range_stage + 1; s.src_b = r.inBlocks.i; s.src_w = r.inBlocks.w;
         s.kin_w = r.k_in.w; s.fin_w = r.f_in.w; s.fs_w = r.f_s.w; s.abs_b = r.abs_b; s.abs_w = r.abs_w;
@@ -1120,8 +1128,18 @@
             CountP q; const UnitDesc dd = d; unit_run_all(q, dd, L); d.cost = q.nput * (unit_is_heavy(d.kind) ? 4 : 1);
         }
     }
+    void begin() { memset(&pads, 0, sizeof pads); p.pads = &pads; }
+    void finish() {
+        p.align_bits();
+        p.pads = nullptr;
+        if (pads.n > BIT_PAD_MAX) throw std::runtime_error("layout planner: more padding runs than BIT_PAD_MAX");
+        bit_stride = p.cur.b;
+        total = p.cur; total.b -= pads.words;
+        estimate_costs();
+    }
     void plan_pob(const PobParams& prm) {
         memset(&L, 0, sizeof L);
+        begin();
         L.circuit = 0; L.pob = prm; L.nkb = 0; max_stage = 0; L.decl_order = p.decl_order;
         L.fp_n2be32 = n2be_footprint(32); L.fp_n2beN = n2be_footprint(prm.amountBytes);
         const uint32_t TB = TRACK_STRIDE, TR = 2 * TRACK_STRIDE, TC = 3 * TRACK_STRIDE, TN = 4 * TRACK_STRIDE;
@@ -1227,11 +1245,11 @@
         }
         proof_of_work_checker(TB + 2);
         unit(U_POB_FINAL, 10);
-        total = p.cur;
-        estimate_costs();
+        finish();
     }
     const char* plan_gadget(uint32_t tid, const int* prm, int nprm) {
         memset(&L, 0, sizeof L);
+        begin();
         L.circuit = 2; L.nkb = 0; max_stage = 0; ntracks = 1; L.decl_order = p.decl_order;
         L.pob = PobParams{1, 1, 1, 0, 31, 0, fr_zero(), fr_zero()};
         L.fp_n2be32 = n2be_footprint(32); L.fp_n2beN = n2be_footprint(31);
@@ -1295,12 +1313,12 @@
             L.gm.nfr_in = 3; L.gm.nsm_in = 1; L.gm.nout = 0;
         } else unit(U_GM, 1, tid, (uint32_t)a, (uint32_t)b, (uint32_t)c, (uint32_t)d);
         nfr_in = L.gm.nfr_in; nsm_in = L.gm.nsm_in;
-        total = p.cur;
-        estimate_costs();
+        finish();
         return nullptr;
     }
     void plan_spend(const SpendParams& prm) {
         memset(&L, 0, sizeof L);
+        begin();
         L.circuit = 1; L.spend = prm; L.nkb = 0; max_stage = 0; ntracks = 1; L.decl_order = p.decl_order;
         L.fp_n2be32 = n2be_footprint(32); L.fp_n2beN = n2be_footprint(prm.maxAmountBytes);
         L.pob = PobParams{1, 1, 1, 0, prm.maxAmountBytes, 0, fr_zero(), fr_zero()};
@@ -1313,7 +1331,6 @@
         unit(U_SP_INPUT, 0);
         unit(U_SP_HEAD, 2);
         public_commitment(4, 3);
-        total = p.cur;
-        estimate_costs();
+        finish();
     }
 };
diff --git a/proof_of_burn_amd/csrc/pob_emit.hip b/proof_of_burn_amd/csrc/pob_emit.hip
--- a/proof_of_burn_amd/csrc/pob_emit.hip
+++ b/proof_of_burn_amd/csrc/pob_emit.hip
@@ -86,7 +86,7 @@
     A.emit_out = E.d_win[slot]; A.emit_sel = idx % 64; A.emit_group = idx / 64; A.emit_w0 = (uint32_t)w0; A.emit_wn = (uint32_t)wn;
     if (E.red) { A.emit_rbits = E.d_rbits; A.emit_rpre = E.d_rpre; }
     emit_units(h, A, k, launch_g_emit);
-    const u64* Gp = (const u64*)h->d_bits + (uint64_t)(idx / 64) * h->plan.total.b;
+    const u64* Gp = (const u64*)h->d_bits + (uint64_t)(idx / 64) * h->plan.bit_stride;
     for_each_run_piece(E, w0, wn, [&](const EmitState::Run& r, uint64_t lo, uint64_t hi) {
         if (!E.red) {
             if (r.absorb) launch_k_emit_absorb(Gp, E.d_win[slot] + (lo - w0) * 32, AbsorbRef{r.b, r.prev, r.src}, r.o + (uint32_t)(lo - r.w), (uint32_t)(hi - lo), idx % 64, h->d_ktab, st);
@@ -480,7 +480,7 @@
     const uint32_t nblk = (uint32_t)((wn + 63) / 64);
     hipStream_t st = own_stream(h);
     HIPC(hipStreamWaitEvent(st, Gr.ev_free[ps], 0));
-    const u64* Gp = (const u64*)h->d_bits + (uint64_t)Gr.group * h->plan.total.b;
+    const u64* Gp = (const u64*)h->d_bits + (uint64_t)Gr.group * h->plan.bit_stride;
     const GroupWin GW{Gr.d_win, Gr.plane, Gr.lanes, (uint32_t)w0, (uint32_t)wn, E.red ? E.d_rbits : nullptr, E.red ? E.d_rpre : nullptr};
     struct Piece { const EmitState::Run* r; uint64_t lo, hi; };
     std::vector<Piece> canon;
diff --git a/proof_of_burn_amd/csrc/pob_host.hip b/proof_of_burn_amd/csrc/pob_host.hip
--- a/proof_of_burn_amd/csrc/pob_host.hip
+++ b/proof_of_burn_amd/csrc/pob_host.hip
@@ -296,7 +296,7 @@
     GArgs A; memset(&A, 0, sizeof A);
     A.units = h->d_units; A.order = h->d_order; A.L = h->d_L;
     A.bits = h->d_bits; A.sm = h->d_sm; A.fr = h->d_fr;
-    A.bits_stride = h->plan.total.b; A.sm_stride = (uint64_t)h->plan.total.s * 64; A.fr_stride = (uint64_t)h->plan.total.f * 512;
+    A.bits_stride = h->plan.bit_stride; A.sm_stride = (uint64_t)h->plan.total.s * 64; A.fr_stride = (uint64_t)h->plan.total.f * 512;
     A.pos_tab = h->d_pos; A.inv_lut = h->d_inv; A.pow256 = h->d_pow256; A.npow256 = h->npow256; A.in_fr = h->d_in_fr[h->in_cur]; A.in_sm = h->d_in_sm[h->in_cur];
     A.nfr_in = h->plan.nfr_in; A.nsm_in = h->plan.nsm_in;
     A.status = h->d_status_raw; A.chk_status = h->d_chk; A.bad_wire = h->d_bad; A.emit_counters = h->d_emit_ctr;
@@ -305,7 +305,7 @@
 }
 static KArgs kargs(pob_ctx* h) {
     KArgs K; memset(&K, 0, sizeof K);
-    K.bits = (u64*)h->d_bits; K.group_stride = h->plan.total.b; K.sponges = h->d_sponges;
+    K.bits = (u64*)h->d_bits; K.group_stride = h->plan.bit_stride; K.sponges = h->d_sponges;
     K.perm_sponge = h->d_perm_sponge; K.perm_block = h->d_perm_block; K.bad_wire = h->d_bad;
     return K;
 }
@@ -349,19 +349,20 @@
         if (why) { err = std::string("gadget main: ") + why; return POB_E_ARG; }
     } else { err = "unknown circuit"; return POB_E_ARG; }
     const Cur t = plan.total;
-    if (t.b >= (1u << 29) || t.s >= (1u << 24) || t.f >= (1u << 21) || t.q >= (1u << 30)) {
+    if (plan.bit_stride >= (1u << 29) || t.s >= (1u << 24) || t.f >= (1u << 21) || t.q >= (1u << 30)) {
         err = "instantiation exceeds the layout's offset limits (BIT < 2^29, SM < 2^24, FR < 2^21 wires)"; return POB_E_ARG;
     }
     return POB_OK;
 }
 static void fill_info(const Plan& pl, uint32_t nperms, uint32_t max_batch, pob_info_t* info) {
     info->n_witness = pl.total.w; info->n_bit = pl.total.b; info->n_sm = pl.total.s; info->n_fr = pl.total.f;
+    info->bit_stride = pl.bit_stride;
     info->n_fr_inputs = pl.nfr_in; info->n_sm_inputs = pl.nsm_in; info->n_outputs = pl.L.circuit == 2 ? pl.L.gm.nout : 1;
     info->n_units = (uint32_t)pl.units.size(); info->n_sponges = (uint32_t)pl.sponges.size(); info->n_perms = nperms;
     { std::vector<char> used(pl.max_stage + 1, 0); for (const UnitDesc& u : pl.units) if (u.flags & UNIT_GEN) used[u.stage] = 1; for (const SpongeDesc& s : pl.sponges) used[s.stage] = 1;
       info->n_stages = 0; for (char c : used) info->n_stages += c; }
     info->max_batch = max_batch;
-    info->group_bytes = (uint64_t)pl.total.b * 8 + (uint64_t)pl.total.s * 256 + (uint64_t)pl.total.f * 2048;
+    info->group_bytes = (uint64_t)pl.bit_stride * 8 + (uint64_t)pl.total.s * 256 + (uint64_t)pl.total.f * 2048;
     info->n_derived = pl.total.q;
     info->n_alias = (uint64_t)nperms * ABSORB_ALIAS;
     info->kchk_rounds = (uint32_t)pob_kchk_rounds(); info->kgc_rounds = (uint32_t)pob_kgc_rounds();
@@ -559,7 +560,7 @@
     }
     h->stream3 = p_track1;
     const uint64_t G = h->groups, npad = G * 64;
-    HIPC(hipMalloc(&h->d_bits, G * (uint64_t)std::max(pl.total.b, 1u) * 8));
+    HIPC(hipMalloc(&h->d_bits, G * (uint64_t)std::max(pl.bit_stride, 1u) * 8));
     HIPC(hipMalloc(&h->d_sm, G * (uint64_t)std::max(pl.total.s, 1u) * 256));
     HIPC(hipMalloc(&h->d_fr, G * (uint64_t)std::max(pl.total.f, 1u) * 2048));
     HIPC(hipMalloc(&h->d_units, pl.units.size() * sizeof(UnitDesc)));
@@ -1128,7 +1129,7 @@
     if (!h->inorder || !h->gc) { h->err = "pob_debug_store_fault: the calculator's generation carries no evaluation (pob_set_inorder bit 2)"; return POB_E_STATE; }
     bool found = false;
     if (cls == POB_CLASS_BIT) {
-        if (index >= h->plan.total.b) return POB_E_ARG;
+        if (index >= h->plan.bit_stride) return POB_E_ARG;
         for (const SpongeDesc& sp : h->plan.sponges) {
             if (index < sp.abs_b || index >= sp.abs_b + (uint64_t)sp.n * ABSORB_BITS) continue;
             const uint32_t b = (uint32_t)((index - sp.abs_b) / ABSORB_BITS), o = (uint32_t)((index - sp.abs_b) % ABSORB_BITS);
@@ -1143,7 +1144,7 @@
     h->fault_g = !found;
     if (!found) {
         const Cur t = h->plan.total;
-        if (!(h->circuit == POB_CIRCUIT_PROOF_OF_BURN || h->circuit == POB_CIRCUIT_SPEND) || (cls == POB_CLASS_BIT ? index >= t.b : cls == POB_CLASS_SM ? index >= t.s : cls == POB_CLASS_FR ? index >= t.f : true)) {
+        if (!(h->circuit == POB_CIRCUIT_PROOF_OF_BURN || h->circuit == POB_CIRCUIT_SPEND) || (cls == POB_CLASS_BIT ? index >= h->plan.bit_stride : cls == POB_CLASS_SM ? index >= t.s : cls == POB_CLASS_FR ? index >= t.f : true)) {
             h->err = "pob_debug_store_fault: not a stored word whose evaluation rides with its generation"; return POB_E_ARG;
         }
         if (wire) *wire = 0xFFFFFFFFu;
@@ -1156,7 +1157,7 @@
     if (!h || group >= h->groups) return POB_E_ARG;
     if (!h->inorder || !h->gc) { h->err = "pob_debug_value_fault: the calculator's generation carries no evaluation (pob_set_inorder bit 2)"; return POB_E_STATE; }
     const Cur t = h->plan.total;
-    if (!(cls == POB_CLASS_BIT ? index < t.b : cls == POB_CLASS_SM ? index < t.s : cls == POB_CLASS_FR ? index < t.f : false)) { h->err = "pob_debug_value_fault: no such word"; return POB_E_ARG; }
+    if (!(cls == POB_CLASS_BIT ? index < h->plan.bit_stride : cls == POB_CLASS_SM ? index < t.s : cls == POB_CLASS_FR ? index < t.f : false)) { h->err = "pob_debug_value_fault: no such word"; return POB_E_ARG; }
     auto refuse = [&](const char* why) { h->err = std::string("pob_debug_value_fault: not covered: ") + why; return POB_E_ARG; };
     if (!(h->circuit == POB_CIRCUIT_PROOF_OF_BURN || h->circuit == POB_CIRCUIT_SPEND)) return refuse("the G units of a gadget-level main do not ride");
     if (cls == POB_CLASS_BIT) return refuse("BIT words (round blocks, sponge chains, the G units' bit runs)");
@@ -1189,10 +1190,10 @@
 }
 
 int pob_debug_xor_bits(pob_handle h, uint32_t group, uint64_t bit_index, uint64_t mask) {
-    if (!h || group >= h->groups || bit_index >= h->plan.total.b) return POB_E_ARG;
+    if (!h || group >= h->groups || bit_index >= h->plan.bit_stride) return POB_E_ARG;
     HIPC(hipSetDevice(h->device));
     h->rode = false;
-    hipLaunchKernelGGL(k_xor_word, dim3(1), dim3(1), 0, own_stream(h), h->d_bits + (uint64_t)group * h->plan.total.b + bit_index, mask);
+    hipLaunchKernelGGL(k_xor_word, dim3(1), dim3(1), 0, own_stream(h), h->d_bits + (uint64_t)group * h->plan.bit_stride + bit_index, mask);
     HIPC(hipStreamSynchronize(own_stream(h)));
     return POB_OK;
 }
@@ -1203,8 +1204,8 @@
     h->rode = false;
     const Cur t = h->plan.total;
     if (cls == POB_CLASS_BIT) {
-        if (index >= t.b) return POB_E_ARG;
-        hipLaunchKernelGGL(k_xor_word, dim3(1), dim3(1), 0, own_stream(h), h->d_bits + (uint64_t)group * t.b + index, (uint64_t)(xor_mask & 1u) << lane);
+        if (index >= h->plan.bit_stride) return POB_E_ARG;
+        hipLaunchKernelGGL(k_xor_word, dim3(1), dim3(1), 0, own_stream(h), h->d_bits + (uint64_t)group * h->plan.bit_stride + index, (uint64_t)(xor_mask & 1u) << lane);
     } else if (cls == POB_CLASS_SM) {
         if (index >= t.s) return POB_E_ARG;
         hipLaunchKernelGGL(k_xor_u32, dim3(1), dim3(1), 0, own_stream(h), (uint32_t*)h->d_sm + ((uint64_t)group * t.s + index) * 64 + lane, xor_mask);
@@ -1265,6 +1266,10 @@
         if (k >= L.nkb) return POB_E_ARG;
         const KBRefs& r = L.kbs[k];
         return n == "kb.inBlocks" ? set(POB_CLASS_BIT, r.inBlocks.i, r.inBlocks.w) : set(POB_CLASS_BIT, r.abs_b + AB_MID, r.abs_w);
+    }
+    if (n == "bit.pad") {
+        if (k >= pl.pads.n) return POB_E_ARG;
+        return set(POB_CLASS_BIT, pl.pads.at[k], pl.pads.len[k]);
     }
     if (n == "pad.div.out" || n == "pad.div.rem") {
         if (k >= L.nkb) return POB_E_ARG;
diff --git a/proof_of_burn_amd/csrc/policy.hpp b/proof_of_burn_amd/csrc/policy.hpp
--- a/proof_of_burn_amd/csrc/policy.hpp
+++ b/proof_of_burn_amd/csrc/policy.hpp
@@ -25,6 +25,7 @@
 static inline uint32_t pob_decl_order_env() { static const uint32_t v = (getenv("POB_DECL_ORDER") && getenv("POB_DECL_ORDER")[0] == '1') ? 1u : 0u; return v; }
 #define POB_DECL_ORDER_DEFAULT pob_decl_order_env()
 #endif
+#define BIT_ALIGN 16u
 struct PolBase {
     Cur cur;
     uint32_t decl_order = POB_DECL_ORDER_DEFAULT;
@@ -33,17 +34,26 @@
     HD uint32_t dvs(uint32_t n) { const uint32_t w = cur.w; cur.w += n; cur.q += n; return w; }
     HD FrRef frs(uint32_t n) { FrRef r = {cur.w, cur.f}; cur.w += n; cur.f += n; return r; }
     HD void skip_alias(uint32_t nw, uint32_t nb) { cur.w += nw; cur.b += nb; }
+    HD uint32_t align_bits(uint32_t ahead = 0) { const uint32_t pad = (0u - (cur.b + ahead)) & (BIT_ALIGN - 1u); cur.b += pad; return pad; }
 };
 
 enum : uint32_t { NOTE_POSEIDON = 1, NOTE_N2BE = 2, NOTE_SHIFTRIGHT = 3, NOTE_SHIFTLEFT = 4 };
 struct PlanNote { uint32_t what, n; Cur cur; uint32_t a[7]; };
 #define PLAN_MAX_NOTES 8
+#define BIT_PAD_MAX 160
+struct PadLog { uint32_t n, words, at[BIT_PAD_MAX], len[BIT_PAD_MAX]; };
 struct CountP : PolBase {
     static constexpr bool is_gen = false, is_check = false, is_emit = false, is_count = true, ride = false;
     uint32_t nput = 0;
     uint32_t nb = 0, ns = 0, nf = 0;
     PlanNote notes[PLAN_MAX_NOTES]; uint32_t nnotes = 0;
     bool notes_overflow = false;
+    PadLog* pads = nullptr;
+    HD uint32_t align_bits(uint32_t ahead = 0) {
+        const uint32_t at = cur.b, n = PolBase::align_bits(ahead);
+        if (pads && n) { if (pads->n < BIT_PAD_MAX) { pads->at[pads->n] = at; pads->len[pads->n] = n; } pads->n++; pads->words += n; }
+        return n;
+    }
     HD void note(uint32_t what, uint32_t n, Cur c, uint32_t a0 = 0, uint32_t a1 = 0, uint32_t a2 = 0, uint32_t a3 = 0, uint32_t a4 = 0, uint32_t a5 = 0, uint32_t a6 = 0) {
         if (nnotes >= PLAN_MAX_NOTES) { notes_overflow = true; return; }
         PlanNote& x = notes[nnotes++]; x.what = what; x.n = n; x.cur = c;
diff --git a/proof_of_burn_amd/witness.py b/proof_of_burn_amd/witness.py
--- a/proof_of_burn_amd/witness.py
+++ b/proof_of_burn_amd/witness.py
@@ -97,7 +97,8 @@
                 ("n_units", ctypes.c_uint32), ("n_sponges", ctypes.c_uint32), ("n_perms", ctypes.c_uint32),
                 ("n_stages", ctypes.c_uint32), ("max_batch", ctypes.c_uint32),
                 ("group_bytes", ctypes.c_uint64), ("keccak_bit_wires", ctypes.c_uint64), ("n_derived", ctypes.c_uint64), ("n_alias", ctypes.c_uint64),
-                ("kchk_rounds", ctypes.c_uint32), ("kgc_rounds", ctypes.c_uint32)]
+                ("kchk_rounds", ctypes.c_uint32), ("kgc_rounds", ctypes.c_uint32),
+                ("bit_stride", ctypes.c_uint64)]
 
 
 RECORD_DTYPE = np.dtype([("status", "<u4"), ("check_status", "<u4"), ("bad_wire", "<u4"), ("commitment", "u1", (32,))])
```

Measured after the change: 1.355 million (median of 6 runs). 8.2% higher.
